# ut-vision/Rot-MVGaze

Measured on AMD Instinct MI355X. Metric: multi-view samples/sec (fwd+bwd), BxVx3x224x224, higher is better.
Workload: dtype f32; 1 GPU; C3: ResNet-50, V=4, B=128 per GPU, 3x224x224, fwd+loss+bwd; backbone=ResNet-50, views=4, batch_per_gpu=128, global_batch=128, image=3x224x224, parallelism=dp1, weights=random init, seed 0 (kaiming-normal convs, default Linear), rccl_ranks=1, step_launch=eager: every kernel queued from Python

## Files before the change

### include/rotmvgaze.h

```cpp
#ifndef ROTMVGAZE_H
#define ROTMVGAZE_H

#include <stddef.h>
#include <stdint.h>

#ifdef __cplusplus
extern "C" {
#endif

#define MVG_ABI_VERSION 11

int mvg_abi_version(void);
const char *mvg_last_error(void);
int mvg_device_cus(void);
int mvg_set_scratch(void *ptr, size_t bytes, void *stream);
size_t mvg_scratch_bytes(void);
void *mvg_stream_create_low_priority(void);
int mvg_set_reserved_cus(int n);

enum {
  MVG_K_CONV_FPROP = 0, MVG_K_CONV_DGRAD = 1, MVG_K_CONV_WGRAD = 2, MVG_K_WGRAD_REDUCE = 3,
  MVG_K_BN_FINALIZE = 4, MVG_K_BN_APPLY = 5, MVG_K_BN_BWD_REDUCE = 6, MVG_K_BN_BWD_APPLY = 7,
  MVG_K_POOL = 8, MVG_K_LAYOUT = 9, MVG_K_LINEAR_FPROP = 10, MVG_K_LINEAR_DGRAD = 11,
  MVG_K_LINEAR_WGRAD = 12, MVG_K_ROTCAT = 13, MVG_K_COLSUM = 14, MVG_K_LOSS = 15,
// ... 38 lines not shown
                    int nvec, int fout, int img_rows, int feat_rows, float *workspace, size_t ws_floats, void *stream);
int mvg_fuser_wgrad(const float *img_feat, const float *feat, const float *rel, const int32_t *row_img,
                    const int32_t *row_src, const float *dy, float *dw, float *db, int rows, int cf, int nvec, int fout,
                    int img_rows, int feat_rows, float *workspace, int splits, int accumulate, void *stream);

int mvg_linear_wgrad(const float *x, const float *dy, float *dw, float *db, int rows, int fin, int fout,
                     float *workspace, int splits, int accumulate, void *stream);

size_t mvg_linear_workspace_floats(int rows, int fin, int fout);
int mvg_linear_fprop(const float *x, const float *w, const float *bias, int relu, float *y, int rows,
                     int fin, int fout, float *workspace, size_t ws_floats, void *stream);
int mvg_linear_dgrad(const float *dy, const float *w, const float *mask, const float *addend, float *dx,
                     int rows, int fin, int fout, float *workspace, size_t ws_floats, void *stream);


int mvg_bn_finalize(const float *stats, int groups, int partials, int rows_per_partial,
                    int64_t rows_per_group, int c, const float *gamma, const float *beta,
                    float *running_mean, float *running_var, float momentum, float eps,
                    float *mean, float *invstd, float *scale, float *shift, void *stream);
int mvg_bn_eval_affine(int groups, int c, const float *gamma, const float *beta,
                       const float *running_mean, const float *running_var, float eps,
                       float *scale, float *shift, void *stream);
int mvg_bn_eval_affine_batch(const void *items_dev, int n, int max_c, float eps, void *stream);
int mvg_bn_apply(const float *y, const float *scale, const float *shift, const float *residual,
                 const float *res_scale, const float *res_shift, int relu, float *out, int groups,
                 int64_t rows_per_group, int c, void *stream);
int mvg_bn_apply_bits(const float *y, const float *scale, const float *shift, const float *residual,
                      const float *res_scale, const float *res_shift, float *out, uint8_t *relu_bits, int groups,
                      int64_t rows_per_group, int c, void *stream);
int mvg_bn_bwd_reduce_bits(const float *g, const uint8_t *relu_bits, const float *y, const float *mean,
                           const float *invstd, int groups, int64_t rows_per_group, int c, float *s1, float *s2,
                           float *dgamma, float *dbeta, int accumulate, float *workspace, float *dz_out, void *stream);
int mvg_bn_apply_bits_bf16(const uint16_t *y, const float *scale, const float *shift, const uint16_t *residual,
                           const float *res_scale, const float *res_shift, uint16_t *out, uint8_t *relu_bits,
                           int groups, int64_t rows_per_group, int c, void *stream);
int mvg_bn_bwd_reduce_bits_bf16(const uint16_t *g, const uint8_t *relu_bits, const uint16_t *y, const float *mean,
                                const float *invstd, int groups, int64_t rows_per_group, int c, float *s1,
                                float *s2, float *dgamma, float *dbeta, int accumulate, float *workspace,
                                uint16_t *dz_out, void *stream);
int mvg_bn_bwd_reduce(const float *g, const float *act, const float *y, const float *mean,
                      const float *invstd, const float *relu_scale, const float *relu_shift,
                      int groups, int64_t rows_per_group, int c, float *s1, float *s2, float *dgamma,
                      float *dbeta, int accumulate, float *workspace, float *dz_out, void *stream);
size_t mvg_bn_bwd_workspace_floats(int groups, int64_t rows_per_group, int c);
int mvg_bn_bwd_apply(const float *g, const float *act, const float *y, const float *mean,
                     const float *invstd, const float *gamma, const float *s1, const float *s2,
                     const float *relu_scale, const float *relu_shift, int groups,
                     int64_t rows_per_group, int c, float *dy, float *dz_out, void *stream);
int mvg_bn_eval_bwd(const float *g, const float *act, const uint8_t *relu_bits, const float *y, const float *relu_scale,
                    const float *relu_shift, const float *gamma, const float *running_mean, const float *running_var,
                    float eps, int groups, int64_t rows_per_group, int c, float *dy, float *dz_out, float *dgamma,
                    float *dbeta, int accumulate, float *workspace, void *stream);
size_t mvg_bn_eval_bwd_workspace_floats(int groups, int64_t rows_per_group, int c);

int mvg_maxpool3x3s2_fwd(const float *x, float *y, uint8_t *argmax, int n, int h, int w, int c,
                         int ho, int wo, void *stream);
int mvg_maxpool3x3s2_bwd(const float *dy, const uint8_t *argmax, float *dx, int n, int h, int w,
                         int c, int ho, int wo, void *stream);
int mvg_bn_relu_maxpool_fwd(const float *y, const float *scale, const float *shift, float *pooled,
                            uint8_t *argmax, int groups, int n_per_group, int h, int w, int c,
                            int ho, int wo, void *stream);
int mvg_bn_relu_maxpool_bwd_reduce(const float *g_pooled, const uint8_t *argmax, const float *y,
                                   const float *mean, const float *invstd, const float *scale,
                                   const float *shift, int groups, int n_per_group, int h, int w,
                                   int c, int ho, int wo, float *s1, float *s2, float *dgamma,
                                   float *dbeta, int accumulate, float *workspace, void *stream);
int mvg_bn_relu_maxpool_bwd_apply(const float *g_pooled, const uint8_t *argmax, const float *y,
                                  const float *mean, const float *invstd, const float *gamma,
                                  const float *scale, const float *shift, const float *s1,
                                  const float *s2, int groups, int n_per_group, int h, int w, int c,
                                  int ho, int wo, float *dy, void *stream);
int mvg_bn_relu_maxpool_eval_bwd(const float *g_pooled, const uint8_t *argmax, const float *y, const float *scale,
                                 const float *shift, const float *gamma, const float *running_mean,
                                 const float *running_var, float eps, int groups, int n_per_group, int h, int w,
                                 int c, int ho, int wo, float *dy, float *dgamma, float *dbeta, int accumulate,
                                 float *workspace, void *stream);
int mvg_avgpool_fwd(const float *x, float *y, int n, int hw, int c, void *stream);
int mvg_avgpool_bwd(const float *dy, float *dx, int n, int hw, int c, void *stream);
int mvg_nchw_to_nhwc4(const float *src, float *dst, int n, int c, int h, int w, void *stream);
int mvg_nhwc4_to_nchw(const float *src, float *dst, int n, int c, int h, int w, void *stream);
int mvg_preprocess_u8hwc(const uint8_t *src, float *dst, int n, int h, int w, float mean0, float mean1,
                         float mean2, float std0, float std1, float std2, int swap_rb, void *stream);
int mvg_preprocess_u8hwc_resize(const uint8_t *src, float *dst, int n, int h, int w, int oh, int ow, float mean0,
                                float mean1, float mean2, float std0, float std1, float std2, int swap_rb,
                                void *stream);
int mvg_multi_erase_nchw(float *img, const float *masks, const int32_t *grid, int gmax, int n, int c,
                         int h, int w, void *stream);

int mvg_rotation_matrix_2d(const float *pitch_yaw , float *rot , int n,
                           int inverse, void *stream);
int mvg_relative_rotation(const float *rot, const int32_t *vi, const int32_t *vj, float *rel,
                          int batch, int views, int dirs, void *stream);

int mvg_rotcat_fwd(const float *img_feat , const float *feat ,
                   const float *rel , const int32_t *view_of,
                   const int32_t *src_of, float *x , int batch, int dirs,
                   int cf, int nvec, void *stream);
int mvg_rotcat_bwd(const float *dx, const float *rel, const int32_t *src_of, float *dfeat, int batch,
                   int dirs, int cf, int nvec, void *stream);
int mvg_rotcat_ext_fwd(const float *img_feat, const float *feat, const float *rel_apply,
                       const float *rel_append, const int32_t *view_of, const int32_t *src_of,
                       float *x, int ld, int batch, int dirs, int cf, int nvec, void *stream);
int mvg_rotcat_ext_bwd(const float *dx, int ld, const float *rel, const int32_t *src_of, float *dfeat,
                       int batch, int dirs, int cf, int nvec, void *stream);
int mvg_ibn_scales(const float *a , const float *feat ,
                   const int32_t *view_of, const int32_t *src_of, float *running_mean, int training,
                   float momentum, float eps, float *scales, int batch, int dirs, int nvec,
                   void *stream);
int mvg_paircat_fwd(const float *a, const float *feat, const float *rel, const float *scales,
                    const int32_t *view_of, const int32_t *src_of, float *x, int batch, int dirs,
                    int nvec, void *stream);
int mvg_paircat_bwd(const float *dx, const float *rel, const float *scales, const int32_t *src_of,
                    float *da_dir, float *dfeat, int batch, int dirs, int nvec, void *stream);
int mvg_segment_sum(const float *x, int64_t row_stride, int width, const int32_t *seg_of, float *out,
                    int batch, int dirs, int segments, int accumulate, void *stream);

int mvg_axpby(const float *x, float *y, float a, float b, int64_t n, void *stream);
int mvg_scale_by(const float *x, const float *scale, float *out, int64_t n, void *stream);

int mvg_linear_skinny_fwd(const float *x, const float *w, const float *bias, float *y, int rows, int k,
                          int nout, void *stream);
int mvg_linear_skinny_bwd(const float *dy, const float *x, const float *w, const float *mask, float *dx,
                          float *dw, float *db, int rows, int k, int nout, int accumulate, float *dx_absmax, void *stream);

int mvg_adam_step(float *param, const float *grad, float *exp_avg, float *exp_avg_sq, int64_t n, float lr,
                  float beta1, float beta2, float eps, float weight_decay, int step, void *stream);
int mvg_adam_step_dev(float *param, const float *grad, float *exp_avg, float *exp_avg_sq, int64_t n, const float *lr_dev,
                      float *state3, float beta1, float beta2, float eps, float weight_decay, void *stream);

int mvg_gaze_angular_loss(const float *pred, const float *gt, int n, float row_weight,
                          float *loss, int accumulate, float *dpred, float *theta_out, void *stream);

int mvg_gaze_lp_loss(const float *pred, const float *label, int n, int p, float *loss, float *dpred, void *stream);
int mvg_gaze_angular_loss_multi(const float *pred, const float *gt, int iters, int dirs, int batch, const float *host_weights,
                                float *loss, float *dpred, void *stream);

int mvg_mt19937_seed(uint32_t *host_state , uint64_t seed);
int64_t mvg_pair_index_build(uint32_t *host_state, const int64_t *host_file_rows, int n_files,
                             int camera_tag, int64_t *host_out , int64_t capacity);


int mvg_cast_weights_bf16(const mvg_conv_desc *d, const float *w, int cin_src, void *w_krsc, void *w_crsk,
                          void *stream);
int mvg_conv_fprop_bf16(const mvg_conv_desc *d, const void *x, const void *wgt, void *y, const float *bias,
                        int relu, float *stats, void *stream);
int mvg_conv_stats_partials_bf16(const mvg_conv_desc *d, int32_t *out_rows_per_partial);
int mvg_conv_fprop_bf16_affine(const mvg_conv_desc *d, const void *x, const void *wgt, void *out, const float *scale,
                               const float *shift, const void *residual, int relu, void *stream);
int mvg_conv_dgrad_bf16(const mvg_conv_desc *d, const void *dy, const void *wgt_crsk, void *dx,
                        const void *mask, const void *addend, void *stream);
int mvg_conv_dgrad_bn_partials_bf16(const mvg_conv_desc *d);
int mvg_conv_dgrad_bf16_bnreduce(const mvg_conv_desc *d, const void *dy, const void *wgt_crsk, void *dx, const void *addend,
                                 const void *bn_y, const uint8_t *bn_bits, const float *bn_mean, const float *bn_invstd,
                                 const float *relu_scale, const float *relu_shift, float *partials, float *s1, float *s2,
                                 float *dgamma, float *dbeta, int accumulate, void *stream);
int mvg_stem_rowwindow_bf16(const float *x_nchw, void *xw, int64_t images, int h, int w, void *stream);
int mvg_stem_fprop_bf16(const mvg_conv_desc *d, const void *xw, const void *w_fold, void *y, float *stats, void *stream);
int mvg_stem_wgrad_splits_bf16(const mvg_conv_desc *d);
int mvg_stem_wgrad_bf16(const mvg_conv_desc *d, const void *xw, const void *dy, float *dw_fold, float *workspace, int splits,
                        int accumulate, void *stream);
int mvg_conv_wgrad_bf16(const mvg_conv_desc *d, const void *x, const void *dy, float *dw, float *workspace,
                        int splits, int accumulate, void *stream);
int mvg_conv_wgrad_splits_bf16(const mvg_conv_desc *d);
int mvg_conv_wgrad_bf16_slabs(const mvg_conv_desc *d, const void *x, const void *dy, float *workspace, int splits, void *stream);
int mvg_linear_fprop_mixed(const float *x, const void *w_bf16, const float *bias, int relu, float *y, int rows, int fin,
                           int fout, void *stream);
int mvg_linear_dgrad_mixed(const float *dy, const void *wt_bf16, const float *mask, const float *addend, float *dx,
                           int rows, int fin, int fout, void *stream);
int mvg_linear_wgrad_mixed(const float *x, const float *dy, float *dw, float *db, int rows, int fin, int fout,
                           float *workspace, int splits, int accumulate, void *stream);
int mvg_bn_apply_bf16(const uint16_t *y, const float *scale, const float *shift, const uint16_t *residual,
                      const float *res_scale, const float *res_shift, int relu, uint16_t *out, int groups,
                      int64_t rows_per_group, int c, void *stream);
int mvg_bn_bwd_reduce_bf16(const uint16_t *g, const uint16_t *act, const uint16_t *y, const float *mean,
                           const float *invstd, const float *relu_scale, const float *relu_shift, int groups,
                           int64_t rows_per_group, int c, float *s1, float *s2, float *dgamma, float *dbeta,
                           int accumulate, float *workspace, uint16_t *dz_out, void *stream);
int mvg_bn_bwd_apply_bf16(const uint16_t *g, const uint16_t *act, const uint16_t *y, const float *mean,
                          const float *invstd, const float *gamma, const float *s1, const float *s2,
                          const float *relu_scale, const float *relu_shift, int groups, int64_t rows_per_group,
                          int c, uint16_t *dy, uint16_t *dz_out, void *stream);
int mvg_bn_relu_maxpool_fwd_bf16(const uint16_t *y, const float *scale, const float *shift, uint16_t *pooled,
                                 uint8_t *argmax, int groups, int n_per_group, int h, int w, int c, int ho,
                                 int wo, void *stream);
int mvg_bn_relu_maxpool_bwd_reduce_bf16(const uint16_t *g_pooled, const uint8_t *argmax, const uint16_t *y,
                                        const float *mean, const float *invstd, const float *scale,
                                        const float *shift, int groups, int n_per_group, int h, int w, int c,
                                        int ho, int wo, float *s1, float *s2, float *dgamma, float *dbeta,
                                        int accumulate, float *workspace, void *stream);
int mvg_bn_relu_maxpool_bwd_apply_bf16(const uint16_t *g_pooled, const uint8_t *argmax, const uint16_t *y,
                                       const float *mean, const float *invstd, const float *gamma,
                                       const float *scale, const float *shift, const float *s1,
                                       const float *s2, int groups, int n_per_group, int h, int w, int c,
                                       int ho, int wo, uint16_t *dy, void *stream);
int mvg_avgpool_fwd_bf16(const uint16_t *x, float *y, int n, int hw, int c, void *stream);
int mvg_avgpool_bwd_bf16(const float *dy, uint16_t *dx, int n, int hw, int c, void *stream);
int mvg_nchw_to_nhwc8_bf16(const float *src, uint16_t *dst, int n, int c, int h, int w, void *stream);
int mvg_preprocess_u8hwc_resize_bf16(const uint8_t *src, uint16_t *dst, int n, int h, int w, int oh, int ow, float mean0,
                                     float mean1, float mean2, float std0, float std1, float std2, int swap_rb,
                                     void *stream);

int mvg_split_f32(const float *x, void *out_sp, int64_t n, float scale, void *stream);
int mvg_merge_sp(const void *x_sp, float *out, int64_t n, float inv_scale, void *stream);
int mvg_split_weights(const mvg_conv_desc *d, const float *w, void *w_krsc_sp, void *w_crsk_sp, float *stat2, void *items_dev,
                      void *stream);
int mvg_weights_prep_batch(const void *items_dev, int n, int mode, int blocks_per_item , void *stream);
int mvg_conv_stats_partials_split(const mvg_conv_desc *d, int32_t *rows_per_partial);
int mvg_conv_fprop_split(const mvg_conv_desc *d, const void *x_sp, const float *x_sinv, const void *w_sp, const float *w_sinv,
                         float *y, float *stats, void *stream);
int mvg_conv_fprop_split_affine(const mvg_conv_desc *d, const void *x_sp, const float *x_sinv, const void *w_sp, const float *w_sinv,
                                void *out, int out_sp, const float *scale, const float *shift, const void *residual,
                                int residual_sp, int relu, void *stream);
int mvg_conv_fprop_split_affine_ranged(const mvg_conv_desc *d, const void *x_sp, const float *x_sinv, const void *w_sp,
                                       const float *w_sinv, void *out, int out_sp, const float *scale, const float *shift,
                                       const void *residual, int residual_sp, int relu, uint32_t *range_word, void *stream);
int mvg_split_f32_ranged(const float *x, void *out_sp, int64_t n, float scale, uint32_t *range_word, void *stream);
int mvg_conv_dgrad_split(const mvg_conv_desc *d, const void *dy_sp, const float *dy_sinv, const void *w_crsk_sp,
                         const float *w_sinv, float *dx, const float *addend, const void *relu_mask_sp, void *stream);
int mvg_bn_apply_split(const float *y, const float *scale, const float *shift, const void *residual, int residual_sp,
                       const float *res_scale, const float *res_shift, int relu, void *out_sp, uint8_t *relu_bits,
                       int groups, int64_t rows_per_group, int c, void *stream);
int mvg_bn_bwd_reduce_split(const float *g, const uint8_t *relu_bits, const float *y, const float *mean, const float *invstd,
                            const float *relu_scale, const float *relu_shift, int groups, int64_t rows_per_group, int c,
                            float *s1, float *s2, float *dgamma, float *dbeta, int accumulate, float *workspace,
                            float *dz_out, float *mx, const float *gamma, float *dy_sinv, void *stream);
int mvg_bn_bwd_apply_split(const float *g, const float *y, const float *mean, const float *invstd, const float *gamma,
                           const float *s1, const float *s2, const float *relu_scale, const float *relu_shift,
                           int groups, int64_t rows_per_group, int c, void *dy_sp, const float *mx, float *dy_sinv,
                           int dy_sinv_ready, void *stream);
int mvg_bn_relu_maxpool_fwd_split(const float *y, const float *scale, const float *shift, void *pooled_sp,
                                  uint8_t *argmax, int groups, int n_per_group, int h, int w, int c, int ho, int wo,
                                  void *stream);
int mvg_avgpool_fwd_split(const void *x_sp, float *y, int n, int hw, int c, void *stream);
int mvg_act_scales(const void *items_dev, int n, float *slots, int n_slots, void *stream);
int mvg_bn_apply_split_scaled(const float *y, const float *scale, const float *shift, const void *residual, int residual_sp,
                              const float *res_scale, const float *res_shift, const float *res_sinv, int relu, void *out_sp,
                              const float *out_sinv, uint8_t *relu_bits, int groups, int64_t rows_per_group, int c,
                              void *stream);
int mvg_bn_relu_maxpool_fwd_split_scaled(const float *y, const float *scale, const float *shift, void *pooled_sp,
                                         const float *pooled_sinv, uint8_t *argmax, int groups, int n_per_group, int h, int w,
                                         int c, int ho, int wo, void *stream);
int mvg_avgpool_fwd_split_scaled(const void *x_sp, const float *x_sinv, float *y, int n, int hw, int c, void *stream);
int mvg_conv_dgrad_bn_partials_split(const mvg_conv_desc *d);
int mvg_conv_dgrad_split_bnreduce(const mvg_conv_desc *d, const void *dy_sp, const float *dy_sinv, const void *w_crsk_sp,
                                  const float *w_sinv, float *dx, const float *addend, const float *bn_y, const uint8_t *bn_bits,
                                  const float *bn_mean, const float *bn_invstd, const float *relu_scale, const float *relu_shift,
                                  float *partials, float *s1, float *s2, float *dgamma, float *dbeta, int accumulate,
                                  float *mx, const float *bn_gamma, float *dx_dy_sinv, void *stream);
int mvg_conv_dgrad_split_bnapply_bnreduce(const mvg_conv_desc *d, void *dy_sp, const float *dy_sinv, const float *dz, const float *y,
                                          const float *mean, const float *invstd, const float *gamma, const float *un_s1,
                                          const float *un_s2, int64_t rows_per_group, const void *w_crsk_sp, const float *w_sinv,
                                          float *dx, const float *addend, const float *bn_y, const uint8_t *bn_bits,
                                          const float *bn_mean, const float *bn_invstd, const float *relu_scale,
                                          const float *relu_shift, float *partials, float *s1, float *s2, float *dgamma, float *dbeta,
                                          int accumulate, float *mx, const float *bn_gamma, float *dx_dy_sinv, void *stream);
int mvg_conv_fprop_split_stages(const mvg_conv_desc *d);
int mvg_conv_dgrad_split_stages(const mvg_conv_desc *d, int fused_reduce);
int mvg_conv_fprop_split_bnapply(const mvg_conv_desc *d, void *out_sp, const float *out_sinv, const float *bn_y, const float *scale,
                                 const float *shift, const void *residual, int residual_sp, const float *res_scale,
                                 const float *res_shift, const float *res_sinv, uint8_t *relu_bits, const void *w_sp,
                                 const float *w_sinv, float *y, float *stats, void *stream);
int mvg_stem_rowwindow_split(const float *x_nhwc4, void *xw_sp, int64_t images, int h, int w, void *stream);
int mvg_stem_rowwindow_split_nchw(const float *x_nchw, void *xw_sp, int64_t images, int h, int w, void *stream);
int mvg_stem_fprop_split(const mvg_conv_desc *d, const void *xw_sp, const void *w_sp, const float *w_sinv, float *y, float *stats,
                         void *stream);
int mvg_stem_wgrad_splits_split(const mvg_conv_desc *d);
int mvg_stem_wgrad_split(const mvg_conv_desc *d, const void *xw_sp, const void *dy_sp, const float *dy_sinv, float *dw_rw,
                         float *workspace, int splits, int accumulate, void *stream);
int mvg_bn_relu_maxpool_bwd_reduce_split(const float *g_pooled, const uint8_t *argmax, const float *y, const float *mean,
                                         const float *invstd, const float *scale, const float *shift, int groups,
                                         int n_per_group, int h, int w, int c, int ho, int wo, float *s1, float *s2,
                                         float *dgamma, float *dbeta, int accumulate, float *workspace, float *mx, const float *gamma,
                                         float *dy_sinv, void *stream);
int mvg_bn_relu_maxpool_bwd_apply_split(const float *g_pooled, const uint8_t *argmax, const float *y, const float *mean,
                                        const float *invstd, const float *gamma, const float *scale, const float *shift,
                                        const float *s1, const float *s2, int groups, int n_per_group, int h, int w, int c,
                                        int ho, int wo, void *dy_sp, const float *mx, float *dy_sinv, int dy_sinv_ready, void *stream);
int mvg_conv_wgrad_splits_split(const mvg_conv_desc *d);
int mvg_conv_wgrad_split_tile(const mvg_conv_desc *d, int32_t *bm, int32_t *bn, int32_t *incremental);
int mvg_conv_wgrad_split(const mvg_conv_desc *d, const void *x_sp, const void *dy_sp, const float *dy_sinv, float *dw,
                         float *workspace, int splits, int accumulate, void *stream);
int mvg_conv_wgrad_split_slabs(const mvg_conv_desc *d, const void *x_sp, const void *dy_sp, const float *dy_sinv, float *workspace,
                               int splits, void *stream);
int mvg_conv_wgrad_split_xs(const mvg_conv_desc *d, const void *x_sp, const float *x_sinv, const void *dy_sp, const float *dy_sinv,
                            float *dw, float *workspace, int splits, int accumulate, void *stream);
int mvg_conv_wgrad_split_slabs_xs(const mvg_conv_desc *d, const void *x_sp, const float *x_sinv, const void *dy_sp,
                                  const float *dy_sinv, float *workspace, int splits, void *stream);
int mvg_wgrad_reduce_batch(const float *const *host_slabs, float *const *host_dw, const int64_t *host_n, const int32_t *host_splits,
                           const int32_t *host_accumulate, int n, void *stream);

int mvg_absmax_multi(const float *const *host_ptrs, const int64_t *host_counts, float *const *host_out_slots, int n, void *stream);
int mvg_fuse_build_split(const float *img_feat, const float *feat, const float *rel, const int32_t *row_img, const int32_t *row_src_f,
                         const int32_t *row_src_h, void *xf_sp, void *xh_sp, const float *am_img, const float *am_feat,
                         float *xf_sinv, float *xh_sinv, int rows, int cf, int nvec, void *stream);
int mvg_fuse_unbuild(const float *dxh, const float *dxn, const float *rel, const int32_t *seg, const int32_t *vi, float *dfeat, float *da,
                     int da_accumulate, int segments, int views, int dirs, int batch, int cf, int nvec, float *absmax, void *stream);
int mvg_linear_fprop_split(int rows, int fin, int fout, const void *x_sp, const float *x_sinv, const void *w_sp, const float *w_sinv,
                           const float *bias, int relu, void *out, int out_sp, float *out_sinv, const float *bias_absmax,
                           float *out_absmax, void *stream);
int mvg_linear_dgrad_split(int rows, int fin, int fout, const void *dy_sp, const float *dy_sinv, const void *wt_sp, const float *w_sinv,
                           float *dx, const float *addend, const void *relu_mask_sp, float *out_absmax, void *stream);
int mvg_linear_wgrad_split(int rows, int fin, int fout, const void *x_sp, const float *x_sinv, const void *dy_sp, const float *dy_sinv,
                           float *dw, float *workspace, int splits, int accumulate, void *stream);
int mvg_split_colsum(const float *g, int rows, int cols, const float *absmax, void *out_sp, float *out_sinv, float *db, int accumulate,
                     void *stream);

typedef struct mvg_session mvg_session;
typedef struct {
  int32_t depth;
  int32_t num_iter;
  int32_t views, batch;
  int32_t height, width;
  int32_t share_weights, ignore_rotmat;
  int32_t split;
  int32_t raw_u8;
  int32_t in_h, in_w, input_bgr;
} mvg_session_cfg;

int mvg_session_create(const mvg_session_cfg *cfg, mvg_session **out);
#define MVG_SESSION_FP32 0
#define MVG_SESSION_BF16 1
int mvg_session_create_ex(const mvg_session_cfg *cfg, int32_t compute, mvg_session **out);
int mvg_session_compute(const mvg_session *s);
void mvg_session_destroy(mvg_session *s);
int mvg_session_num_tensors(const mvg_session *s);
const char *mvg_session_tensor_name(const mvg_session *s, int i);
int64_t mvg_session_tensor_numel(const mvg_session *s, int i);
size_t mvg_session_workspace_bytes(const mvg_session *s);
int mvg_session_launches(const mvg_session *s);
int mvg_session_num_steps(const mvg_session *s);
const char *mvg_session_step_name(const mvg_session *s, int i);
int mvg_session_bind(mvg_session *s, const void *const *host_tensor_ptrs, void *workspace, size_t bytes, void *stream);
int mvg_session_forward(mvg_session *s, const void *const *host_view_ptrs, const float *rot, float *img_feat, float *lifted,
                        float *feats, float *preds, void *stream);
int mvg_session_num_range_units(const mvg_session *s);
const char *mvg_session_range_unit_name(const mvg_session *s, int i);
int mvg_session_set_range_record(mvg_session *s, uint32_t *record_dev);

#ifdef __cplusplus
}
#endif
#endif
```

### rot-mvgaze_amd/_lib.py

```python
from __future__ import annotations

import ctypes as C
import os

_HERE = os.path.dirname(os.path.abspath(__file__))
LIB_PATH = os.path.join(_HERE, "csrc", "librotmvgaze_hip.so")

K_FAMILIES = 18
ABI_VERSION = 11
SESSION_FP32, SESSION_BF16 = 0, 1


class ConvDesc(C.Structure):
    _fields_ = [(n, C.c_int32) for n in
                ("groups", "n", "h", "w", "cin", "cout", "r", "s", "stride", "pad", "ho", "wo")]

    @classmethod
    def make(cls, groups, n, h, w, cin, cout, k, stride, pad):
        ho = (h + 2 * pad - k) // stride + 1
        wo = (w + 2 * pad - k) // stride + 1
        return cls(groups, n, h, w, cin, cout, k, k, stride, pad, ho, wo)

    @classmethod
    def linear(cls, rows, fin, fout):
        return cls(1, rows, 1, 1, fin, fout, 1, 1, 1, 0, 1, 1)


class ProfEntry(C.Structure):
    _fields_ = [("launches", C.c_int64), ("ms", C.c_double), ("flops", C.c_double), ("bytes", C.c_double)]


class SessionCfg(C.Structure):
    _fields_ = [(n, C.c_int32) for n in
                ("depth", "num_iter", "views", "batch", "height", "width", "share_weights", "ignore_rotmat", "split", "raw_u8",
                 "in_h", "in_w", "input_bgr")]


_P = C.c_void_p
_I = C.c_int
_I64 = C.c_int64
_F = C.c_float
_D = C.POINTER(ConvDesc)

SIGNATURES = {
    "mvg_abi_version": (_I, []),
    "mvg_last_error": (C.c_char_p, []),
    "mvg_device_cus": (_I, []),
    "mvg_set_scratch": (_I, [_P, C.c_size_t, _P]),
    "mvg_scratch_bytes": (C.c_size_t, []),
    "mvg_set_reserved_cus": (_I, [_I]),
    "mvg_stream_create_low_priority": (_P, []),
    "mvg_prof_enable": (_I, [_I]),
    "mvg_prof_reset": (_I, []),
    "mvg_prof_collect": (_I, [C.POINTER(ProfEntry)]),
    "mvg_prof_family_name": (C.c_char_p, [_I]),
    "mvg_conv_fprop": (_I, [_D, _P, _P, _P, _P, _I, _P, _P]),
    "mvg_conv_fprop_affine": (_I, [_D, _P, _P, _P, _P, _P, _P, _I, _P]),
    "mvg_conv_stats_partials": (_I, [_D, C.POINTER(C.c_int32)]),
    "mvg_conv_dgrad": (_I, [_D, _P, _P, _P, _P, _P, _P]),
    "mvg_conv_wgrad": (_I, [_D, _P, _P, _P, _P, _I, _I, _P]),
    "mvg_conv_wgrad_splits": (_I, [_D]),
    "mvg_linear_wgrad": (_I, [_P, _P, _P, _P, _I, _I, _I, _P, _I, _I, _P]),
    "mvg_fuser_fprop": (_I, [_P, _P, _P, _P, _P, _P, _P, _I, _P, _I, _I, _I, _I, _I, _I, _P, C.c_size_t, _P]),
    "mvg_fuser_wgrad": (_I, [_P, _P, _P, _P, _P, _P, _P, _P, _I, _I, _I, _I, _I, _I, _P, _I, _I, _P]),
    "mvg_linear_workspace_floats": (C.c_size_t, [_I, _I, _I]),
    "mvg_linear_fprop": (_I, [_P, _P, _P, _I, _P, _I, _I, _I, _P, C.c_size_t, _P]),
    "mvg_linear_dgrad": (_I, [_P, _P, _P, _P, _P, _I, _I, _I, _P, C.c_size_t, _P]),
    "mvg_bn_finalize": (_I, [_P, _I, _I, _I, _I64, _I, _P, _P, _P, _P, _F, _F, _P, _P, _P, _P, _P]),
    "mvg_bn_eval_affine": (_I, [_I, _I, _P, _P, _P, _P, _F, _P, _P, _P]),
    "mvg_bn_eval_affine_batch": (_I, [_P, _I, _I, _F, _P]),
    "mvg_bn_apply": (_I, [_P, _P, _P, _P, _P, _P, _I, _P, _I, _I64, _I, _P]),
    "mvg_bn_bwd_reduce": (_I, [_P, _P, _P, _P, _P, _P, _P, _I, _I64, _I, _P, _P, _P, _P, _I, _P, _P, _P]),
    "mvg_split_f32": (_I, [_P, _P, _I64, _F, _P]),
    "mvg_merge_sp": (_I, [_P, _P, _I64, _F, _P]),
    "mvg_split_weights": (_I, [_D, _P, _P, _P, _P, _P, _P]),
    "mvg_weights_prep_batch": (_I, [_P, _I, _I, _I, _P]),
    "mvg_conv_stats_partials_split": (_I, [_D, C.POINTER(C.c_int32)]),
    "mvg_conv_fprop_split": (_I, [_D, _P, _P, _P, _P, _P, _P, _P]),
    "mvg_conv_fprop_split_affine": (_I, [_D, _P, _P, _P, _P, _P, _I, _P, _P, _P, _I, _I, _P]),
    "mvg_conv_dgrad_split": (_I, [_D, _P, _P, _P, _P, _P, _P, _P, _P]),
    "mvg_bn_apply_split": (_I, [_P, _P, _P, _P, _I, _P, _P, _I, _P, _P, _I, _I64, _I, _P]),
    "mvg_bn_bwd_apply_split": (_I, [_P, _P, _P, _P, _P, _P, _P, _P, _P, _I, _I64, _I, _P, _P, _P, _I, _P]),
    "mvg_bn_bwd_reduce_split": (_I, [_P, _P, _P, _P, _P, _P, _P, _I, _I64, _I, _P, _P, _P, _P, _I, _P, _P, _P, _P, _P, _P]),
    "mvg_bn_relu_maxpool_fwd_split": (_I, [_P, _P, _P, _P, _P, _I, _I, _I, _I, _I, _I, _I, _P]),
    "mvg_avgpool_fwd_split": (_I, [_P, _P, _I, _I, _I, _P]),
    "mvg_act_scales": (_I, [_P, _I, _P, _I, _P]),
    "mvg_bn_apply_split_scaled": (_I, [_P, _P, _P, _P, _I, _P, _P, _P, _I, _P, _P, _P, _I, _I64, _I, _P]),
    "mvg_bn_relu_maxpool_fwd_split_scaled": (_I, [_P, _P, _P, _P, _P, _P, _I, _I, _I, _I, _I, _I, _I, _P]),
    "mvg_avgpool_fwd_split_scaled": (_I, [_P, _P, _P, _I, _I, _I, _P]),
    "mvg_conv_wgrad_split_xs": (_I, [_D, _P, _P, _P, _P, _P, _P, _I, _I, _P]),
    "mvg_conv_wgrad_split_slabs_xs": (_I, [_D, _P, _P, _P, _P, _P, _I, _P]),
    "mvg_stem_rowwindow_split": (_I, [_P, _P, _I64, _I, _I, _P]),
    "mvg_stem_rowwindow_split_nchw": (_I, [_P, _P, _I64, _I, _I, _P]),
    "mvg_stem_fprop_split": (_I, [_D, _P, _P, _P, _P, _P, _P]),
    "mvg_stem_wgrad_splits_split": (_I, [_D]),
    "mvg_stem_wgrad_split": (_I, [_D, _P, _P, _P, _P, _P, _I, _I, _P]),
    "mvg_bn_relu_maxpool_bwd_reduce_split": (_I, [_P, _P, _P, _P, _P, _P, _P, _I, _I, _I, _I, _I, _I, _I, _P, _P, _P, _P, _I, _P, _P, _P, _P, _P]),
    "mvg_bn_relu_maxpool_bwd_apply_split": (_I, [_P, _P, _P, _P, _P, _P, _P, _P, _P, _P, _I, _I, _I, _I, _I, _I, _I, _P, _P, _P, _I, _P]),
    "mvg_conv_dgrad_bn_partials_split": (_I, [_D]),
    "mvg_conv_dgrad_split_bnreduce": (_I, [_D, _P, _P, _P, _P, _P, _P, _P, _P, _P, _P, _P, _P, _P, _P, _P, _P, _P, _I, _P, _P, _P, _P]),
    "mvg_conv_dgrad_split_bnapply_bnreduce": (_I, [_D] + [_P] * 9 + [_I64] + [_P] * 15 + [_I, _P, _P, _P, _P]),
    "mvg_conv_fprop_split_stages": (_I, [_D]),
    "mvg_conv_dgrad_split_stages": (_I, [_D, _I]),
    "mvg_conv_fprop_split_bnapply": (_I, [_D] + [_P] * 6 + [_I] + [_P] * 9),
    "mvg_conv_wgrad_splits_split": (_I, [_D]),
    "mvg_conv_wgrad_split_tile": (_I, [_D, C.POINTER(C.c_int32), C.POINTER(C.c_int32), C.POINTER(C.c_int32)]),
    "mvg_conv_wgrad_split": (_I, [_D, _P, _P, _P, _P, _P, _I, _I, _P]),
    "mvg_conv_wgrad_split_slabs": (_I, [_D, _P, _P, _P, _P, _I, _P]),
    "mvg_wgrad_reduce_batch": (_I, [C.POINTER(C.c_void_p), C.POINTER(C.c_void_p), C.POINTER(C.c_int64), C.POINTER(C.c_int32),
                                    C.POINTER(C.c_int32), _I, _P]),
    "mvg_bn_apply_bits": (_I, [_P, _P, _P, _P, _P, _P, _P, _P, _I, _I64, _I, _P]),
    "mvg_bn_bwd_reduce_bits": (_I, [_P, _P, _P, _P, _P, _I, _I64, _I, _P, _P, _P, _P, _I, _P, _P, _P]),
    "mvg_bn_apply_bits_bf16": (_I, [_P, _P, _P, _P, _P, _P, _P, _P, _I, _I64, _I, _P]),
    "mvg_bn_bwd_reduce_bits_bf16": (_I, [_P, _P, _P, _P, _P, _I, _I64, _I, _P, _P, _P, _P, _I, _P, _P, _P]),
    "mvg_bn_bwd_workspace_floats": (C.c_size_t, [_I, _I64, _I]),
    "mvg_bn_bwd_apply": (_I, [_P, _P, _P, _P, _P, _P, _P, _P, _P, _P, _I, _I64, _I, _P, _P, _P]),
    "mvg_maxpool3x3s2_fwd": (_I, [_P, _P, _P, _I, _I, _I, _I, _I, _I, _P]),
    "mvg_maxpool3x3s2_bwd": (_I, [_P, _P, _P, _I, _I, _I, _I, _I, _I, _P]),
    "mvg_bn_relu_maxpool_fwd": (_I, [_P, _P, _P, _P, _P, _I, _I, _I, _I, _I, _I, _I, _P]),
    "mvg_bn_relu_maxpool_bwd_reduce": (_I, [_P, _P, _P, _P, _P, _P, _P, _I, _I, _I, _I, _I, _I, _I, _P, _P, _P, _P, _I, _P,
                                            _P]),
    "mvg_bn_relu_maxpool_bwd_apply": (_I, [_P, _P, _P, _P, _P, _P, _P, _P, _P, _P, _I, _I, _I, _I, _I, _I, _I, _P, _P]),
    "mvg_bn_eval_bwd": (_I, [_P, _P, _P, _P, _P, _P, _P, _P, _P, _F, _I, _I64, _I, _P, _P, _P, _P, _I, _P, _P]),
    "mvg_bn_eval_bwd_workspace_floats": (C.c_size_t, [_I, _I64, _I]),
    "mvg_bn_relu_maxpool_eval_bwd": (_I, [_P, _P, _P, _P, _P, _P, _P, _P, _F, _I, _I, _I, _I, _I, _I, _I, _P, _P, _P, _I, _P,
                                          _P]),
    "mvg_avgpool_fwd": (_I, [_P, _P, _I, _I, _I, _P]),
    "mvg_avgpool_bwd": (_I, [_P, _P, _I, _I, _I, _P]),
    "mvg_nchw_to_nhwc4": (_I, [_P, _P, _I, _I, _I, _I, _P]),
    "mvg_nhwc4_to_nchw": (_I, [_P, _P, _I, _I, _I, _I, _P]),
    "mvg_preprocess_u8hwc": (_I, [_P, _P, _I, _I, _I, _F, _F, _F, _F, _F, _F, _I, _P]),
    "mvg_gaze_lp_loss": (_I, [_P, _P, _I, _I, _P, _P, _P]),
    "mvg_preprocess_u8hwc_resize": (_I, [_P, _P, _I, _I, _I, _I, _I, _F, _F, _F, _F, _F, _F, _I, _P]),
    "mvg_multi_erase_nchw": (_I, [_P, _P, _P, _I, _I, _I, _I, _I, _P]),
    "mvg_rotation_matrix_2d": (_I, [_P, _P, _I, _I, _P]),
    "mvg_relative_rotation": (_I, [_P, _P, _P, _P, _I, _I, _I, _P]),
    "mvg_rotcat_fwd": (_I, [_P, _P, _P, _P, _P, _P, _I, _I, _I, _I, _P]),
    "mvg_rotcat_bwd": (_I, [_P, _P, _P, _P, _I, _I, _I, _I, _P]),
    "mvg_rotcat_ext_fwd": (_I, [_P, _P, _P, _P, _P, _P, _P, _I, _I, _I, _I, _I, _P]),
    "mvg_rotcat_ext_bwd": (_I, [_P, _I, _P, _P, _P, _I, _I, _I, _I, _P]),
    "mvg_ibn_scales": (_I, [_P, _P, _P, _P, _P, _I, _F, _F, _P, _I, _I, _I, _P]),
    "mvg_paircat_fwd": (_I, [_P, _P, _P, _P, _P, _P, _P, _I, _I, _I, _P]),
    "mvg_paircat_bwd": (_I, [_P, _P, _P, _P, _P, _P, _I, _I, _I, _P]),
    "mvg_segment_sum": (_I, [_P, _I64, _I, _P, _P, _I, _I, _I, _I, _P]),
    "mvg_axpby": (_I, [_P, _P, _F, _F, _I64, _P]),
    "mvg_scale_by": (_I, [_P, _P, _P, _I64, _P]),
    "mvg_linear_skinny_fwd": (_I, [_P, _P, _P, _P, _I, _I, _I, _P]),
    "mvg_linear_skinny_bwd": (_I, [_P, _P, _P, _P, _P, _P, _P, _I, _I, _I, _I, _P, _P]),
    "mvg_adam_step": (_I, [_P, _P, _P, _P, _I64, _F, _F, _F, _F, _F, _I, _P]),
    "mvg_gaze_angular_loss": (_I, [_P, _P, _I, _F, _P, _I, _P, _P, _P]),
    "mvg_gaze_angular_loss_multi": (_I, [_P, _P, _I, _I, _I, C.POINTER(C.c_float), _P, _P, _P]),
    "mvg_adam_step_dev": (_I, [_P, _P, _P, _P, _I64, _P, _P, _F, _F, _F, _F, _P]),
    "mvg_absmax_multi": (_I, [C.POINTER(C.c_void_p), C.POINTER(C.c_int64), C.POINTER(C.c_void_p), _I, _P]),
    "mvg_fuse_build_split": (_I, [_P, _P, _P, _P, _P, _P, _P, _P, _P, _P, _P, _P, _I, _I, _I, _P]),
    "mvg_fuse_unbuild": (_I, [_P, _P, _P, _P, _P, _P, _P, _I, _I, _I, _I, _I, _I, _I, _P, _P]),
    "mvg_linear_fprop_split": (_I, [_I, _I, _I, _P, _P, _P, _P, _P, _I, _P, _I, _P, _P, _P, _P]),
    "mvg_linear_dgrad_split": (_I, [_I, _I, _I, _P, _P, _P, _P, _P, _P, _P, _P, _P]),
    "mvg_linear_wgrad_split": (_I, [_I, _I, _I, _P, _P, _P, _P, _P, _P, _I, _I, _P]),
    "mvg_split_colsum": (_I, [_P, _I, _I, _P, _P, _P, _P, _I, _P]),
    "mvg_cast_weights_bf16": (_I, [_D, _P, _I, _P, _P, _P]),
    "mvg_conv_fprop_bf16": (_I, [_D, _P, _P, _P, _P, _I, _P, _P]),
    "mvg_conv_stats_partials_bf16": (_I, [_D, C.POINTER(C.c_int32)]),
    "mvg_conv_fprop_bf16_affine": (_I, [_D, _P, _P, _P, _P, _P, _P, _I, _P]),
    "mvg_conv_dgrad_bf16": (_I, [_D, _P, _P, _P, _P, _P, _P]),
    "mvg_conv_dgrad_bn_partials_bf16": (_I, [_D]),
    "mvg_conv_dgrad_bf16_bnreduce": (_I, [_D, _P, _P, _P, _P, _P, _P, _P, _P, _P, _P, _P, _P, _P, _P, _P, _I, _P]),
    "mvg_conv_wgrad_bf16": (_I, [_D, _P, _P, _P, _P, _I, _I, _P]),
    "mvg_stem_rowwindow_bf16": (_I, [_P, _P, _I64, _I, _I, _P]),
    "mvg_stem_fprop_bf16": (_I, [_D, _P, _P, _P, _P, _P]),
    "mvg_stem_wgrad_splits_bf16": (_I, [_D]),
    "mvg_stem_wgrad_bf16": (_I, [_D, _P, _P, _P, _P, _I, _I, _P]),
    "mvg_conv_wgrad_splits_bf16": (_I, [_D]),
    "mvg_conv_wgrad_bf16_slabs": (_I, [_D, _P, _P, _P, _I, _P]),
    "mvg_linear_fprop_mixed": (_I, [_P, _P, _P, _I, _P, _I, _I, _I, _P]),
    "mvg_linear_dgrad_mixed": (_I, [_P, _P, _P, _P, _P, _I, _I, _I, _P]),
    "mvg_linear_wgrad_mixed": (_I, [_P, _P, _P, _P, _I, _I, _I, _P, _I, _I, _P]),
    "mvg_bn_apply_bf16": (_I, [_P, _P, _P, _P, _P, _P, _I, _P, _I, _I64, _I, _P]),
    "mvg_bn_bwd_reduce_bf16": (_I, [_P, _P, _P, _P, _P, _P, _P, _I, _I64, _I, _P, _P, _P, _P, _I, _P, _P, _P]),
    "mvg_bn_bwd_apply_bf16": (_I, [_P, _P, _P, _P, _P, _P, _P, _P, _P, _P, _I, _I64, _I, _P, _P, _P]),
    "mvg_bn_relu_maxpool_fwd_bf16": (_I, [_P, _P, _P, _P, _P, _I, _I, _I, _I, _I, _I, _I, _P]),
    "mvg_bn_relu_maxpool_bwd_reduce_bf16": (_I, [_P, _P, _P, _P, _P, _P, _P, _I, _I, _I, _I, _I, _I, _I, _P, _P, _P, _P, _I,
                                                 _P, _P]),
    "mvg_bn_relu_maxpool_bwd_apply_bf16": (_I, [_P, _P, _P, _P, _P, _P, _P, _P, _P, _P, _I, _I, _I, _I, _I, _I, _I, _P, _P]),
    "mvg_avgpool_fwd_bf16": (_I, [_P, _P, _I, _I, _I, _P]),
    "mvg_avgpool_bwd_bf16": (_I, [_P, _P, _I, _I, _I, _P]),
    "mvg_nchw_to_nhwc8_bf16": (_I, [_P, _P, _I, _I, _I, _I, _P]),
    "mvg_preprocess_u8hwc_resize_bf16": (_I, [_P, _P, _I, _I, _I, _I, _I, _F, _F, _F, _F, _F, _F, _I, _P]),
    "mvg_mt19937_seed": (_I, [_P, C.c_uint64]),
    "mvg_pair_index_build": (_I64, [_P, _P, _I, _I, _P, _I64]),
    "mvg_session_create": (_I, [C.POINTER(SessionCfg), C.POINTER(_P)]),
    "mvg_session_destroy": (None, [_P]),
    "mvg_session_num_tensors": (_I, [_P]),
    "mvg_session_tensor_name": (C.c_char_p, [_P, _I]),
    "mvg_session_tensor_numel": (_I64, [_P, _I]),
    "mvg_session_workspace_bytes": (C.c_size_t, [_P]),
    "mvg_session_launches": (_I, [_P]),
    "mvg_session_bind": (_I, [_P, C.POINTER(_P), _P, C.c_size_t, _P]),
    "mvg_session_forward": (_I, [_P, C.POINTER(_P), _P, _P, _P, _P, _P, _P]),
    "mvg_conv_fprop_split_affine_ranged": (_I, [_D, _P, _P, _P, _P, _P, _I, _P, _P, _P, _I, _I, _P, _P]),
    "mvg_split_f32_ranged": (_I, [_P, _P, _I64, _F, _P, _P]),
    "mvg_session_num_range_units": (_I, [_P]),
    "mvg_session_range_unit_name": (C.c_char_p, [_P, _I]),
    "mvg_session_set_range_record": (_I, [_P, _P]),
    "mvg_session_create_ex": (_I, [C.POINTER(SessionCfg), C.c_int32, C.POINTER(_P)]),
    "mvg_session_compute": (_I, [_P]),
    "mvg_session_num_steps": (_I, [_P]),
    "mvg_session_step_name": (C.c_char_p, [_P, _I]),
}

_lib = None


def lib() -> C.CDLL:
    global _lib
    if _lib is not None:
        return _lib
    if not os.path.exists(LIB_PATH):
        raise RuntimeError(
            f"{LIB_PATH} not found: the HIP extension is required (python rot-mvgaze_amd/csrc/build.py); "
            "this package has no CPU fallback")
    try:
        l = C.CDLL(LIB_PATH, mode=C.RTLD_GLOBAL)
    except OSError as e:
        raise RuntimeError(f"failed to load {LIB_PATH}: {e}") from e
    for name, (res, args) in SIGNATURES.items():
        fn = getattr(l, name)
        fn.restype = res
        fn.argtypes = args
    if l.mvg_abi_version() != ABI_VERSION:
        raise RuntimeError(f"librotmvgaze_hip.so ABI {l.mvg_abi_version()} != binding ABI {ABI_VERSION}")
    _lib = l
    return l


def check(rc: int, what: str = "") -> None:
    if rc != 0:
        msg = lib().mvg_last_error()
        raise RuntimeError(f"librotmvgaze_hip {what} failed (rc={rc}): {msg.decode() if msg else '?'}")
```

### rot-mvgaze_amd/csrc/conv_split.hip

```cpp
#include "bf16_tile.h"
#include "elem.h"

namespace mvg {

typedef _Float16 f16x8 __attribute__((ext_vector_type(8)));

#define SPLIT_ONE(PA, PB, av, bv, acc)                                                                         \
  _Pragma("unroll") for (int i = 0; i < TM; ++i) _Pragma("unroll") for (int j = 0; j < TN; ++j)                \
      acc[i][j] = __builtin_amdgcn_mfma_f32_32x32x16_f16(av[PA][i], bv[PB][j], acc[i][j], 0, 0, 0);
#define SPLIT_PRODUCTS(av, bv, acc) SPLIT_ONE(0, 1, av, bv, acc) SPLIT_ONE(1, 0, av, bv, acc) SPLIT_ONE(0, 0, av, bv, acc)

constexpr int SP_BM = 128, SP_BK = 32;

__global__ __launch_bounds__(256) void split_f32_kernel(const float4 *__restrict__ x, uint4 *__restrict__ out, long long n8, float scale) {
  const long long stride = (long long)gridDim.x * 256;
  for (long long i = (long long)blockIdx.x * 256 + threadIdx.x; i < n8; i += stride) {
    const float4 lo = x[2 * i], hi = x[2 * i + 1];
    const float v[8] = {lo.x * scale, lo.y * scale, lo.z * scale, lo.w * scale, hi.x * scale, hi.y * scale, hi.z * scale, hi.w * scale};
    uint4 q1, q2;
    split2_chunk(v, q1, q2);
    out[2 * i] = q1;
    out[2 * i + 1] = q2;
  }
}
// ... 27 lines not shown
}

__global__ __launch_bounds__(256) void split_colsum_kernel(const float *__restrict__ g, int rows, int cols, const unsigned *__restrict__ absmax,
                                                           uint4 *__restrict__ out, float *__restrict__ out_sinv, float *__restrict__ db,
                                                           int accumulate) {
  __shared__ float sh[64][33];
  const float scale = sp_scale_for(__uint_as_float(*absmax));
  if (blockIdx.x == 0 && threadIdx.x == 0) *out_sinv = 1.f / scale;
  const int cl = threadIdx.x & 3, rl = threadIdx.x >> 2;
  const int c8 = blockIdx.x * 4 + cl, c8n = cols >> 3;
  float sum[8] = {0.f, 0.f, 0.f, 0.f, 0.f, 0.f, 0.f, 0.f};
  for (int r = rl; r < rows; r += 64) {
    const float4 *src = reinterpret_cast<const float4 *>(g + (long long)r * cols + c8 * 8);
    const float4 lo = src[0], hi = src[1];
    const float v[8] = {lo.x, lo.y, lo.z, lo.w, hi.x, hi.y, hi.z, hi.w};
    float w[8];
#pragma unroll
    for (int k = 0; k < 8; ++k) {
      sum[k] += v[k];
      w[k] = v[k] * scale;
    }
    uint4 q1, q2;
    split2_chunk(w, q1, q2);
    uint4 *dst = out + SP_NP * ((long long)r * c8n + c8);
    dst[0] = q1;
    dst[1] = q2;
  }
  if (db == nullptr) return;
#pragma unroll
  for (int k = 0; k < 8; ++k) sh[rl][cl * 8 + k] = sum[k];
  __syncthreads();
  if (threadIdx.x < 32) {
    const int col = blockIdx.x * 32 + threadIdx.x;
    float t = accumulate ? db[col] : 0.f;
    for (int r = 0; r < 64; ++r) t += sh[r][threadIdx.x];
    db[col] = t;
  }
}

struct WPrepItem {
  const float *w;
  void *wk, *wt;
  int cout, rs, cin, cin_pad;
  float *stat;
};

__global__ void wprep_stage_item_kernel(WPrepItem it, WPrepItem *__restrict__ dst) {
  if (threadIdx.x == 0) *dst = it;
  if (threadIdx.x < 2) it.stat[threadIdx.x] = 0.f;
}

__global__ __launch_bounds__(256) void weights_absmax_kernel(const WPrepItem *__restrict__ items) {
  const WPrepItem it = items[blockIdx.y];
  const long long n4 = (long long)it.cout * it.rs * it.cin / 4;
  float m = 0.f;
  for (long long i = (long long)blockIdx.x * 256 + threadIdx.x; i < n4; i += (long long)gridDim.x * 256) {
    const float4 v = reinterpret_cast<const float4 *>(it.w)[i];
    m = fmaxf(fmaxf(m, fmaxf(fabsf(v.x), fabsf(v.y))), fmaxf(fabsf(v.z), fabsf(v.w)));
  }
#pragma unroll
  for (int o = 32; o > 0; o >>= 1) m = fmaxf(m, __shfl_xor(m, o, 64));
  if ((threadIdx.x & 63) == 0 && m > 0.f) atomicMax(reinterpret_cast<unsigned *>(it.stat), __float_as_uint(m));
}

__global__ __launch_bounds__(256) void weights_prep_batch_kernel(const WPrepItem *__restrict__ items, int mode) {
  __shared__ float tile[64][65];
  const WPrepItem it = items[blockIdx.y];
  const float *__restrict__ w = it.w;
  const int cout = it.cout, rs = it.rs, cin = it.cin;
  if (mode == 1) {
    const float scale = sp_scale_for(__uint_as_float(*reinterpret_cast<const unsigned *>(it.stat)));
    if (blockIdx.x == 0 && threadIdx.x == 0) it.stat[1] = 1.f / scale;
    uint4 *wk = reinterpret_cast<uint4 *>(it.wk), *wt = reinterpret_cast<uint4 *>(it.wt);
    const int c8n = cin / 8, o8n = cout / 8;
    const bool tiled = wt != nullptr && rs == 1 && (cin % 64) == 0 && (cout % 64) == 0;
    const long long nk = (long long)cout * rs * c8n, nt = (wt && !tiled) ? (long long)cin * rs * o8n : 0;
    for (long long i = (long long)blockIdx.x * 256 + threadIdx.x; i < nk + nt; i += (long long)gridDim.x * 256) {
      float v[8];
      uint4 *dst;
      if (i < nk) {
        const float4 *src = reinterpret_cast<const float4 *>(w + i * 8);
        const float4 lo = src[0], hi = src[1];
        v[0] = lo.x; v[1] = lo.y; v[2] = lo.z; v[3] = lo.w; v[4] = hi.x; v[5] = hi.y; v[6] = hi.z; v[7] = hi.w;
        dst = wk + SP_NP * i;
      } else {
        const long long j = i - nk;
        const int o8 = (int)(j % o8n);
        const long long t = j / o8n;
        const int tap = (int)(t % rs), c = (int)(t / rs);
#pragma unroll
        for (int k = 0; k < 8; ++k) v[k] = w[((long long)(o8 * 8 + k) * rs + tap) * cin + c];
        dst = wt + SP_NP * j;
      }
#pragma unroll
      for (int k = 0; k < 8; ++k) v[k] *= scale;
      uint4 q1, q2;
      split2_chunk(v, q1, q2);
      dst[0] = q1;
      dst[1] = q2;
    }
    if (tiled) {
      const int tc = cin / 64, ntiles = (cout / 64) * tc;
      for (int t = blockIdx.x; t < ntiles; t += gridDim.x) {
        const int o0 = (t / tc) * 64, c0 = (t % tc) * 64;
        __syncthreads();
#pragma unroll
        for (int ps = 0; ps < 4; ++ps) {
          const int r = (threadIdx.x >> 4) + 16 * ps, cq = threadIdx.x & 15;
          const float4 x = *reinterpret_cast<const float4 *>(w + (long long)(o0 + r) * cin + c0 + 4 * cq);
          tile[r][4 * cq] = x.x;
          tile[r][4 * cq + 1] = x.y;
          tile[r][4 * cq + 2] = x.z;
          tile[r][4 * cq + 3] = x.w;
        }
        __syncthreads();
#pragma unroll
        for (int q = 0; q < 2; ++q) {
          const int idx = threadIdx.x + 256 * q, cl = idx >> 3, o8 = idx & 7;
          float v[8];
#pragma unroll
          for (int k = 0; k < 8; ++k) v[k] = tile[o8 * 8 + k][cl] * scale;
          uint4 q1, q2;
          split2_chunk(v, q1, q2);
          uint4 *dst = wt + SP_NP * ((long long)(c0 + cl) * o8n + (o0 >> 3) + o8);
          dst[0] = q1;
          dst[1] = q2;
        }
      }
    }
    return;
  }
  unsigned short *wk = reinterpret_cast<unsigned short *>(it.wk), *wt = reinterpret_cast<unsigned short *>(it.wt);
  const int cin_pad = it.cin_pad;
  const long long total = (long long)cout * rs * cin_pad;
  if (rs == 1 && cin == cin_pad && (cin % 64) == 0 && (cout % 64) == 0) {
    uint4 *wk4 = reinterpret_cast<uint4 *>(wk);
    for (long long i = (long long)blockIdx.x * 256 + threadIdx.x; i < total / 8; i += (long long)gridDim.x * 256) {
      const float4 lo = reinterpret_cast<const float4 *>(w + i * 8)[0], hi = reinterpret_cast<const float4 *>(w + i * 8)[1];
      wk4[i] = make_uint4(bf16_pack2(lo.x, lo.y), bf16_pack2(lo.z, lo.w), bf16_pack2(hi.x, hi.y), bf16_pack2(hi.z, hi.w));
    }
    if (wt) {
      const int tc = cin / 64, ntiles = (cout / 64) * tc;
      for (int t = blockIdx.x; t < ntiles; t += gridDim.x) {
        const int o0 = (t / tc) * 64, c0 = (t % tc) * 64;
        __syncthreads();
#pragma unroll
        for (int ps = 0; ps < 4; ++ps) {
          const int r = (threadIdx.x >> 4) + 16 * ps, cq = threadIdx.x & 15;
          const float4 x = *reinterpret_cast<const float4 *>(w + (long long)(o0 + r) * cin + c0 + 4 * cq);
          tile[r][4 * cq] = x.x;
          tile[r][4 * cq + 1] = x.y;
          tile[r][4 * cq + 2] = x.z;
          tile[r][4 * cq + 3] = x.w;
        }
        __syncthreads();
#pragma unroll
        for (int q = 0; q < 2; ++q) {
          const int idx = threadIdx.x + 256 * q, cl = idx >> 3, o8 = idx & 7;
          float v[8];
#pragma unroll
          for (int k = 0; k < 8; ++k) v[k] = tile[o8 * 8 + k][cl];
          *reinterpret_cast<uint4 *>(wt + (long long)(c0 + cl) * cout + o0 + o8 * 8) =
              make_uint4(bf16_pack2(v[0], v[1]), bf16_pack2(v[2], v[3]), bf16_pack2(v[4], v[5]), bf16_pack2(v[6], v[7]));
        }
      }
    }
    return;
  }
  for (long long i = (long long)blockIdx.x * 256 + threadIdx.x; i < total; i += (long long)gridDim.x * 256) {
    const int c = (int)(i % cin_pad);
    const long long t = i / cin_pad;
    const int tap = (int)(t % rs), o = (int)(t / rs);
    const float v = c < cin ? w[((long long)o * rs + tap) * cin + c] : 0.f;
    const __bf16 b = (__bf16)v;
    const unsigned short u = __builtin_bit_cast(unsigned short, b);
    wk[i] = u;
    if (wt) wt[((long long)c * rs + tap) * cout + o] = u;
  }
}

typedef float f32x4 __attribute__((ext_vector_type(4)));

#define SPLIT16_ONE(PA, PB)                                                                       \
  _Pragma("unroll") for (int i = 0; i < TM; ++i) _Pragma("unroll") for (int j = 0; j < TN; ++j)   \
      acc[i][j] = __builtin_amdgcn_mfma_f32_16x16x32_f16(av[PA][i], bv[PB][j], acc[i][j], 0, 0, 0);

__device__ __forceinline__ int sp_row_swz(int R) { return ((R >> 1) & 1) | (((R >> 2) & 1) << 2); }

enum AForm : int { A_DMA = 0, A_DY = 1, A_OUT_SP = 2, A_OUT_AFFINE = 3 };
constexpr int BNA_MAX_C = 512;

__device__ __forceinline__ void unpack8(const float4 (&v)[2], float (&o)[8]) {
  o[0] = v[0].x; o[1] = v[0].y; o[2] = v[0].z; o[3] = v[0].w; o[4] = v[1].x; o[5] = v[1].y; o[6] = v[1].z; o[7] = v[1].w;
}

struct DyFormer {
  static constexpr int TABLES = 5;
  __amdgpu_buffer_rsrc_t rs_dz, rs_y;
  float inv_rows, dsc;
  float4 dzv[2][2], yv[2][2];
  float mu[8], is[8], ga[8], sa[8], sb[8];
  static __device__ __forceinline__ void stage(float *t, const IgemmParams &p, int g, int C, int tid) {
    for (int i = tid; i < C; i += 256) {
      const long long gc = (long long)g * C + i;
      t[i] = p.bna_mean[gc];
      t[C + i] = p.bna_invstd[gc];
      t[2 * C + i] = p.bna_gamma[i];
      t[3 * C + i] = p.bna_s1[gc];
      t[4 * C + i] = p.bna_s2[gc];
    }
  }
  __device__ __forceinline__ DyFormer(const IgemmParams &p, long long grow0, long long rows_per_group, int C)
      : rs_dz(make_rsrc(p.bna_dz + grow0 * C, 4ll * rows_per_group * C)), rs_y(make_rsrc(p.bna_y + grow0 * C, 4ll * rows_per_group * C)),
        inv_rows(p.bna_inv_rows), dsc(1.f / *p.a_sinv) {}
  __device__ __forceinline__ void load(int i, unsigned off) {
    dzv[i][0] = buf_ld16(rs_dz, off);
    dzv[i][1] = buf_ld16(rs_dz, off + 16u);
    yv[i][0] = buf_ld16(rs_y, off);
    yv[i][1] = buf_ld16(rs_y, off + 16u);
  }
  __device__ __forceinline__ void consts(const float *kc, int C) {
    ld8(kc, mu);
    ld8(kc + C, is);
    ld8(kc + 2 * C, ga);
    ld8(kc + 3 * C, sa);
    ld8(kc + 4 * C, sb);
  }
  __device__ __forceinline__ void form(int i, bool ok, float (&o)[8]) {
    float d[8], v[8];
    unpack8(dzv[i], d);
    unpack8(yv[i], v);
    bn_dy_chunk(d, v, mu, is, ga, sa, sb, inv_rows, dsc, o, false, mu, mu);
#pragma unroll
    for (int k = 0; k < 8; ++k) o[k] = ok ? o[k] : 0.f;
  }
  __device__ __forceinline__ void store_extra(int, unsigned) {}
};

template <bool AFFINE>
struct OutFormer {
  static constexpr int TABLES = AFFINE ? 4 : 2;
  __amdgpu_buffer_rsrc_t rs_y, rs_r;
  float osc, rsi;
  unsigned short *bits_out;
  float4 yv[2][2], rv[2][2];
  float sc[8], sh[8], rs[8], rh[8];
  unsigned mb[2];
  static __device__ __forceinline__ void stage(float *t, const IgemmParams &p, int g, int C, int tid) {
    for (int i = tid; i < C; i += 256) {
      const long long gc = (long long)g * C + i;
      t[i] = p.fap_scale[gc];
      t[C + i] = p.fap_shift[gc];
      if constexpr (AFFINE) {
        t[2 * C + i] = p.fap_res_scale[gc];
        t[3 * C + i] = p.fap_res_shift[gc];
      }
    }
  }
  __device__ __forceinline__ OutFormer(const IgemmParams &p, long long grow0, long long rows_per_group, int C)
      : rs_y(make_rsrc(p.fap_y + grow0 * C, 4ll * rows_per_group * C)),
        rs_r(make_rsrc(reinterpret_cast<const float *>(p.fap_res) + grow0 * C, 4ll * rows_per_group * C)),
        osc(__uint_as_float(__builtin_amdgcn_readfirstlane(__float_as_uint(p.a_sinv ? 1.f / *p.a_sinv : 1.f)))),
        rsi(__uint_as_float(__builtin_amdgcn_readfirstlane(__float_as_uint((!AFFINE && p.fap_res_sinv) ? *p.fap_res_sinv : 1.f)))),
        bits_out(p.fap_bits ? p.fap_bits + grow0 * (C >> 3) : nullptr) {}
  __device__ __forceinline__ void load(int i, unsigned off) {
    yv[i][0] = buf_ld16(rs_y, off);
    yv[i][1] = buf_ld16(rs_y, off + 16u);
    rv[i][0] = buf_ld16(rs_r, off);
    rv[i][1] = buf_ld16(rs_r, off + 16u);
  }
  __device__ __forceinline__ void consts(const float *kc, int C) {
    ld8(kc, sc);
    ld8(kc + C, sh);
    if constexpr (AFFINE) {
      ld8(kc + 2 * C, rs);
      ld8(kc + 3 * C, rh);
    }
  }
  __device__ __forceinline__ void form(int i, bool ok, float (&o)[8]) {
    float v[8], r[8];
    unpack8(yv[i], v);
    if constexpr (AFFINE) {
      unpack8(rv[i], r);
    } else {
      const uint4 r1 = make_uint4(__float_as_uint(rv[i][0].x), __float_as_uint(rv[i][0].y), __float_as_uint(rv[i][0].z), __float_as_uint(rv[i][0].w));
      const uint4 r2 = make_uint4(__float_as_uint(rv[i][1].x), __float_as_uint(rv[i][1].y), __float_as_uint(rv[i][1].z), __float_as_uint(rv[i][1].w));
      merge2_chunk(r1, r2, r);
    }
    mb[i] = bn_apply_chunk(v, sc, sh, true, r, AFFINE, rs, rh, !AFFINE, rsi, true, osc, o);
#pragma unroll
    for (int k = 0; k < 8; ++k) o[k] = ok ? o[k] : 0.f;
  }
  __device__ __forceinline__ void store_extra(int i, unsigned off) {
    if (bits_out) bits_out[off >> 5] = (unsigned short)mb[i];
  }
};

#define MVG_SPLIT_RNG 0
#include "conv_split_igemm.inc"
#undef MVG_SPLIT_RNG
#define MVG_SPLIT_RNG 1
#include "conv_split_igemm.inc"
#undef MVG_SPLIT_RNG

template <int BM, int BN, bool INCR>
__global__ __launch_bounds__(256, BN >= 256 ? 2 : 3) void wgrad_split_kernel(WgradParams p) {
  constexpr int BK = 16, WGM = 2, WGN = 2;
  constexpr int WTM = BM / WGM, WTN = BN / WGN;
  constexpr int TM = WTM / 32, TN = WTN / 32;
  constexpr int LDA = BM + 32, LDB = BN + 32;
  constexpr int MV = BM / 8, NVB = BN / 8;
  constexpr int A_TPR = 256 / BK;
  constexpr int A_CPT = MV / A_TPR > 0 ? MV / A_TPR : 1;
  constexpr int B_CPT = (NVB + A_TPR - 1) / A_TPR;
  constexpr int A_ELEMS = BK * LDA, B_ELEMS = BK * LDB;
  constexpr int STAGE = SP_NP * (A_ELEMS + B_ELEMS);
  __shared__ __attribute__((aligned(16))) unsigned short smem[2 * STAGE];

  const int tid = threadIdx.x;
  const int lane = tid & 63, wave = tid >> 6;
  const int wm = wave / WGN, wn = wave % WGN;
  const int li = lane & 31, lh = lane >> 5;
  const int tiles = p.mtiles * p.ntiles;
  const int logical = xcd_remap(blockIdx.x, gridDim.x);
  const int split = logical / tiles;
  const int tile = logical - split * tiles;
  const int ntile = tile % p.ntiles, mtile = tile / p.ntiles;
  const long long m_begin = (long long)split * p.pixels_per_split;
  long long m_end = m_begin + p.pixels_per_split;
  if (m_end > p.pixels) m_end = p.pixels;
  const int m_count = m_end > m_begin ? (int)(m_end - m_begin) : 0;
  const int ohw = p.ho * p.wo;
  const long long img0 = m_begin / ohw;
  const unsigned rem0 = (unsigned)(m_begin - img0 * ohw);

  const char *dy = reinterpret_cast<const char *>(p.dy);
  const char *x = reinterpret_cast<const char *>(p.x);
  const __amdgpu_buffer_rsrc_t rs_a = make_rsrc(dy + m_begin * p.cout * SP_BYTES, (long long)SP_BYTES * m_count * p.cout);
  const long long x_img_elems = (long long)p.h * p.w * p.cin;
  const __amdgpu_buffer_rsrc_t rs_b = make_rsrc(x + img0 * x_img_elems * SP_BYTES, p.x_bytes - (long long)SP_BYTES * img0 * x_img_elems);
  const int i_row = tid / A_TPR, i_v0 = tid % A_TPR;
  unsigned a_off[A_CPT];
  bool a_on[A_CPT];
#pragma unroll
  for (int j = 0; j < A_CPT; ++j) {
    const int cv = i_v0 + j * A_TPR;
    const int col = mtile * BM + cv * 8;
    a_on[j] = cv < MV;
    a_off[j] = (a_on[j] && col < p.cout) ? (unsigned)(i_row * p.cout + col) * (unsigned)SP_BYTES : 0x80000000u;
  }
  int i_dy[B_CPT], i_dx[B_CPT];
  unsigned i_tconst[B_CPT];
  bool i_cok[B_CPT], b_on[B_CPT];
#pragma unroll
  for (int j = 0; j < B_CPT; ++j) {
    const int cv = i_v0 + j * A_TPR;
    const int col = ntile * BN + cv * 8;
    b_on[j] = cv < NVB;
    i_cok[j] = b_on[j] && col < p.ncols;
    const int tap = (int)fdiv((unsigned)(i_cok[j] ? col : 0), p.cin_div);
    const int cc = (i_cok[j] ? col : 0) - tap * p.cin;
    const int fr = (int)fdiv((unsigned)tap, p.s_div), fs = tap - fr * p.s;
    i_dy[j] = fr - p.pad;
    i_dx[j] = fs - p.pad_w;
    i_tconst[j] = (unsigned)((i_dy[j] * p.w + i_dx[j]) * p.cin + cc) * (unsigned)SP_BYTES;
  }
  const unsigned row_bytes = (unsigned)(p.stride * p.w * p.cin) * (unsigned)SP_BYTES, col_bytes = (unsigned)(p.stride_w * p.cin) * (unsigned)SP_BYTES;
  const unsigned img_bytes = (unsigned)x_img_elems * (unsigned)SP_BYTES;
  int s_oy = 0, s_ox = 0;
  unsigned s_imgoff = 0;
  if (INCR) {
    const unsigned pix = rem0 + (unsigned)i_row;
    const unsigned img = fdiv(pix, p.ohw_div);
    const unsigned rem = pix - img * (unsigned)ohw;
    const unsigned oy = fdiv(rem, p.wo_div);
    s_oy = (int)oy;
    s_ox = (int)(rem - oy * (unsigned)p.wo);
    s_imgoff = img * img_bytes;
  }
  u32x4 a_reg[A_CPT][SP_NP], b_reg[B_CPT][SP_NP];
  auto load_tiles = [&](int kt) {
#pragma unroll
    for (int j = 0; j < A_CPT; ++j) {
#pragma unroll
      for (int pc = 0; pc < SP_NP; ++pc)
        a_reg[j][pc] = __builtin_amdgcn_raw_buffer_load_b128(rs_a, a_off[j] + 16u * pc, 0, 0);
      a_off[j] += (unsigned)(BK * p.cout) * (unsigned)SP_BYTES;
    }
    const bool mok = kt * BK + i_row < m_count;
    int oy, ox;
    unsigned imgoff;
    if constexpr (INCR) {
      oy = s_oy;
      ox = s_ox;
      imgoff = s_imgoff;
    } else {
      const unsigned pix = rem0 + (unsigned)(kt * BK + i_row);
      const unsigned img = fdiv(pix, p.ohw_div);
      const unsigned rem = pix - img * (unsigned)ohw;
      const unsigned uy = fdiv(rem, p.wo_div);
      oy = (int)uy;
      ox = (int)(rem - uy * (unsigned)p.wo);
      imgoff = img * img_bytes;
    }
    const int iy0 = oy * p.stride, ix0 = ox * p.stride_w;
    const unsigned pixoff = imgoff + (unsigned)oy * row_bytes + (unsigned)ox * col_bytes;
#pragma unroll
    for (int j = 0; j < B_CPT; ++j) {
      const bool ok = mok & i_cok[j] & ((unsigned)(iy0 + i_dy[j]) < (unsigned)p.h) & ((unsigned)(ix0 + i_dx[j]) < (unsigned)p.w);
#pragma unroll
      for (int pc = 0; pc < SP_NP; ++pc)
        b_reg[j][pc] = __builtin_amdgcn_raw_buffer_load_b128(rs_b, pred_off(pixoff + i_tconst[j] + 16u * pc, ok), 0, 0);
    }
    if constexpr (INCR) {
      unsigned nx = (unsigned)s_ox + BK;
      const unsigned q = fdiv(nx, p.wo_div);
      nx -= q * (unsigned)p.wo;
      s_ox = (int)nx;
      const int noy = s_oy + (int)q;
      const bool wrap = noy >= p.ho;
      s_oy = wrap ? noy - p.ho : noy;
      s_imgoff += wrap ? img_bytes : 0u;
    }
  };
  auto store_tiles = [&](int buf) {
    unsigned short *As = smem + buf * STAGE;
    unsigned short *Bs = As + SP_NP * A_ELEMS;
#pragma unroll
    for (int j = 0; j < A_CPT; ++j)
      if (a_on[j]) {
#pragma unroll
        for (int pc = 0; pc < SP_NP; ++pc)
          *reinterpret_cast<u32x4 *>(As + pc * A_ELEMS + i_row * LDA + (i_v0 + j * A_TPR) * 8) = a_reg[j][pc];
      }
#pragma unroll
    for (int j = 0; j < B_CPT; ++j)
      if (b_on[j]) {
#pragma unroll
        for (int pc = 0; pc < SP_NP; ++pc)
          *reinterpret_cast<u32x4 *>(Bs + pc * B_ELEMS + i_row * LDB + (i_v0 + j * A_TPR) * 8) = b_reg[j][pc];
      }
  };

  f32x16 acc[TM][TN];
#pragma unroll
  for (int i = 0; i < TM; ++i)
#pragma unroll
    for (int j = 0; j < TN; ++j)
#pragma unroll
      for (int e = 0; e < 16; ++e) acc[i][j][e] = 0.f;

  const int KT = (m_count + BK - 1) / BK;
  load_tiles(0);
  store_tiles(0);
  load_tiles(1);
  __syncthreads();
  for (int kt = 0; kt < KT; ++kt) {
    const int cur = kt & 1;
    store_tiles(cur ^ 1);
    load_tiles(kt + 2);
    const unsigned short *As = smem + cur * STAGE;
    const unsigned short *Bs = As + SP_NP * A_ELEMS;
    f16x8 av[SP_NP][TM], bv[SP_NP][TN];
#pragma unroll
    for (int pc = 0; pc < SP_NP; ++pc) {
#pragma unroll
      for (int i = 0; i < TM; ++i) av[pc][i] = __builtin_bit_cast(f16x8, tr_frag(As + pc * A_ELEMS, LDA, 0, wm * WTM + i * 32, lane));
#pragma unroll
      for (int j = 0; j < TN; ++j) bv[pc][j] = __builtin_bit_cast(f16x8, tr_frag(Bs + pc * B_ELEMS, LDB, 0, wn * WTN + j * 32, lane));
    }
    SPLIT_PRODUCTS(av, bv, acc)
    __syncthreads();
  }

  float *out = p.out + (long long)split * p.cout * p.ncols;
  const float osc = (p.dy_sinv ? *p.dy_sinv : 1.f) * (p.x_sinv ? *p.x_sinv : 1.f);
#pragma unroll
  for (int i = 0; i < TM; ++i)
#pragma unroll
    for (int j = 0; j < TN; ++j) {
      const int col = ntile * BN + wn * WTN + j * 32 + li;
#pragma unroll
      for (int e = 0; e < 16; ++e) {
        const int row = mtile * BM + wm * WTM + i * 32 + (e & 3) + 8 * (e >> 2) + 4 * lh;
        if (row < p.cout && col < p.ncols) {
          const long long off = (long long)row * p.ncols + col;
          float v = acc[i][j][e] * osc;
          if (p.accumulate) v += out[off];
          out[off] = v;
        }
      }
    }
}

struct ReduceItem {
  const float *slabs;
  float *dw;
  long long n4;
  int splits, accumulate, lanes, block0;
};
struct ReduceBatch {
  ReduceItem it[8];
  int n;
};
__global__ __launch_bounds__(256) void wgrad_reduce_batch_kernel(ReduceBatch b) {
  __shared__ float4 sh[256];
  int k = 0;
  for (int i = 1; i < b.n; ++i) k += (int)blockIdx.x >= b.it[i].block0;
  const ReduceItem &r = b.it[k];
  const int cols = 256 / r.lanes;
  const int c = threadIdx.x % cols, l = threadIdx.x / cols;
  const long long i = (long long)(blockIdx.x - r.block0) * cols + c;
  float4 s = make_float4(0.f, 0.f, 0.f, 0.f);
  if (i < r.n4)
    for (int q = l; q < r.splits; q += r.lanes) {
      const float4 v = reinterpret_cast<const float4 *>(r.slabs)[(long long)q * r.n4 + i];
      s.x += v.x;
      s.y += v.y;
      s.z += v.z;
      s.w += v.w;
    }
  sh[threadIdx.x] = s;
  __syncthreads();
  if (l == 0 && i < r.n4) {
    float4 t = r.accumulate ? reinterpret_cast<const float4 *>(r.dw)[i] : make_float4(0.f, 0.f, 0.f, 0.f);
    for (int q = 0; q < r.lanes; ++q) {
      const float4 v = sh[q * cols + c];
      t.x += v.x;
      t.y += v.y;
      t.z += v.z;
      t.w += v.w;
    }
    reinterpret_cast<float4 *>(r.dw)[i] = t;
  }
}

__global__ __launch_bounds__(256) void stem_rowwindow_kernel(const float4 *__restrict__ x, uint4 *__restrict__ xw, long long n, int h, int w) {
  const int wo = w >> 1;
  for (long long i = (long long)blockIdx.x * 256 + threadIdx.x; i < n; i += (long long)gridDim.x * 256) {
    const int q = (int)(i & 3);
    const long long t = i >> 2;
    const int ox = (int)(t % wo);
    const long long row = t / wo;
    const int c0 = 2 * ox - 4 + 2 * q;
    float v[8] = {0.f, 0.f, 0.f, 0.f, 0.f, 0.f, 0.f, 0.f};
    if (c0 >= 0 && c0 < w) {
      const float4 a = x[row * w + c0], b = x[row * w + c0 + 1];
      v[0] = a.x; v[1] = a.y; v[2] = a.z; v[3] = a.w; v[4] = b.x; v[5] = b.y; v[6] = b.z; v[7] = b.w;
    }
    uint4 q1, q2;
    split2_chunk(v, q1, q2);
    xw[SP_NP * i] = q1;
    xw[SP_NP * i + 1] = q2;
  }
}

__global__ __launch_bounds__(256) void stem_rowwindow_nchw_kernel(const float *__restrict__ x, uint4 *__restrict__ xw, long long n, int h, int w) {
  const int wo = w >> 1;
  const long long plane = (long long)h * w;
  for (long long i = (long long)blockIdx.x * 256 + threadIdx.x; i < n; i += (long long)gridDim.x * 256) {
    const int q = (int)(i & 3);
    const long long t = i >> 2;
    const int ox = (int)(t % wo);
    const long long row = t / wo;
    const long long img = row / h;
    const int yy = (int)(row - img * h);
    const int c0 = 2 * ox - 4 + 2 * q;
    float v[8] = {0.f, 0.f, 0.f, 0.f, 0.f, 0.f, 0.f, 0.f};
    if (c0 >= 0 && c0 < w) {
      const float *src = x + img * 3 * plane + (long long)yy * w + c0;
      const float2 r = *reinterpret_cast<const float2 *>(src), g = *reinterpret_cast<const float2 *>(src + plane),
                   b = *reinterpret_cast<const float2 *>(src + 2 * plane);
      v[0] = r.x; v[1] = g.x; v[2] = b.x; v[4] = r.y; v[5] = g.y; v[6] = b.y;
    }
    uint4 q1, q2;
    split2_chunk(v, q1, q2);
    xw[SP_NP * i] = q1;
    xw[SP_NP * i + 1] = q2;
  }
}

static int validate_split(const mvg_conv_desc *d) {
  if (validate(d)) return 2;
  MVG_REQUIRE(d->cin % 32 == 0 && d->cout % 32 == 0, "split conv: cin and cout must be multiples of 32 (got %d, %d)", d->cin,
              d->cout);
  MVG_REQUIRE(d->r * d->s <= 32, "split conv: at most 32 filter taps");
  return 0;
}

static int split_tile_rows(int ncols, int taps, long long rows) { return (ncols < 128 && taps > 1 && rows >= 65536) ? 256 : SP_BM; }

struct SplitPlan { int bm, bn, kt_max; long long tiles; bool pipelined; };
static int split_conv_stages(const SplitPlan &pl) { return (pl.pipelined && pl.bn == 128 && pl.bm == SP_BM) ? 2 : 1; }
static SplitPlan split_plan(int ncols, int taps, long long rows, int groups, bool lin, IgemmClass *cls, int ncls) {
  SplitPlan pl;
  pl.bm = lin ? SP_BM : split_tile_rows(ncols, taps, rows);
  pl.bn = ncols >= 128 ? 128 : 64;
  if (lin && pl.bn == 128 && ncls == 1) {
    const long long t128 = (long long)groups * ceil_div(cls[0].rows_per_group, pl.bm) * ceil_div(ncols, 128);
    if (2 * t128 <= compute_cus()) pl.bn = 64;
  }
  pl.tiles = 0, pl.kt_max = 0;
  for (int i = 0; i < ncls; ++i) {
    IgemmClass &c = cls[i];
    c.mtiles_per_group = ceil_div(c.rows_per_group, pl.bm);
    c.KT = ceil_div(c.ktotal, SP_BK);
    c.tile0 = (int)pl.tiles;
    pl.tiles += (long long)groups * c.mtiles_per_group * ceil_div(ncols, pl.bn);
    pl.kt_max = c.KT > pl.kt_max ? c.KT : pl.kt_max;
  }
  pl.pipelined = pl.tiles <= 2LL * compute_cus() || (pl.tiles <= 4LL * compute_cus() && pl.kt_max >= 48);
  return pl;
}

template <bool DGRAD>
static int launch_igemm_split(IgemmParams &p, hipStream_t st, bool lin, int taps, long long rows, AForm af = A_DMA, bool ranged = false) {
  const SplitPlan pl = split_plan(p.ncols, taps, rows, p.groups, lin, p.cls, p.ncls);
  const int bm = pl.bm, bn = pl.bn;
  const bool pipelined = pl.pipelined;
  p.ntiles = ceil_div(p.ncols, bn);
  p.splits = 1;
  p.sk_tiles = 0;
  p.bn_parts = 0;
  for (int i = 0; i < p.ncls; ++i) {
    IgemmClass &c = p.cls[i];
    c.korder = c.ntaps > 1 ? 1 : 0;
    c.per_div = make_fastdiv((unsigned)(c.ntaps > 0 ? c.ntaps : 1));
    c.unit0 = 0;
    c.part0 = p.bn_parts;
    p.bn_parts += c.mtiles_per_group;
    MVG_REQUIRE((c.ntaps >= 1 || (DGRAD && p.bn_part)) && c.ntaps <= 32 && c.ktotal % SP_BK == 0, "split conv: class shape not covered");
  }
  MVG_REQUIRE(pl.tiles < (1LL << 31), "split conv: grid too large");
  if (pl.tiles <= 0) return 0;
  p.nt_out = (!lin && !(DGRAD && p.cls_step == 2)) ? 1 : 0;
  dim3 grid((unsigned)pl.tiles), block(256);
  if (af != A_DMA) {
    MVG_REQUIRE(!lin && bm == SP_BM && p.ntiles == 1 && p.ncls == 1 && DGRAD == (af == A_DY), "split conv: the operand-forming loaders take one column tile");
    if constexpr (DGRAD) {
      if (bn == 128) hipLaunchKernelGGL((igemm_split16_kernel<128, true, false, 2, 1, A_DY>), grid, block, 0, st, p);
      else hipLaunchKernelGGL((igemm_split16_kernel<64, true, false, 2, 1, A_DY>), grid, block, 0, st, p);
      return check_launch("conv_dgrad_split_bnapply");
    } else {
      if (bn == 128 && af == A_OUT_AFFINE) hipLaunchKernelGGL((igemm_split16_kernel<128, false, false, 2, 1, A_OUT_AFFINE>), grid, block, 0, st, p);
      else if (bn == 128) hipLaunchKernelGGL((igemm_split16_kernel<128, false, false, 2, 1, A_OUT_SP>), grid, block, 0, st, p);
      else if (af == A_OUT_AFFINE) hipLaunchKernelGGL((igemm_split16_kernel<64, false, false, 2, 1, A_OUT_AFFINE>), grid, block, 0, st, p);
      else hipLaunchKernelGGL((igemm_split16_kernel<64, false, false, 2, 1, A_OUT_SP>), grid, block, 0, st, p);
      return check_launch("conv_fprop_split_bnapply");
    }
  }
  if (ranged) {
    MVG_REQUIRE(!DGRAD && !lin && p.out_sp && p.out_absmax, "split conv: the range record goes with a forward that stores sp");
    if constexpr (!DGRAD) {
      if (bm == 256) hipLaunchKernelGGL((igemm_split16_ranged_kernel<64, 4>), grid, block, 0, st, p);
      else if (split_conv_stages(pl) == 2) hipLaunchKernelGGL((igemm_split16_ranged_kernel<128, 2, 2>), grid, block, 0, st, p);
      else if (bn == 128) hipLaunchKernelGGL((igemm_split16_ranged_kernel<128>), grid, block, 0, st, p);
      else hipLaunchKernelGGL((igemm_split16_ranged_kernel<64>), grid, block, 0, st, p);
    }
    return check_launch("conv_fprop_split_ranged");
  }
  if (lin) {
    if (bn == 128 && pipelined) hipLaunchKernelGGL((igemm_split16_kernel<128, DGRAD, true, 2, 2>), grid, block, 0, st, p);
    else if (bn == 128) hipLaunchKernelGGL((igemm_split16_kernel<128, DGRAD, true>), grid, block, 0, st, p);
    else if (pipelined) hipLaunchKernelGGL((igemm_split16_kernel<64, DGRAD, true, 2, 2>), grid, block, 0, st, p);
    else hipLaunchKernelGGL((igemm_split16_kernel<64, DGRAD, true>), grid, block, 0, st, p);
  } else if (bm == 256) hipLaunchKernelGGL((igemm_split16_kernel<64, DGRAD, false, 4>), grid, block, 0, st, p);
  else if (split_conv_stages(pl) == 2) hipLaunchKernelGGL((igemm_split16_kernel<128, DGRAD, false, 2, 2>), grid, block, 0, st, p);
  else if (bn == 128) hipLaunchKernelGGL((igemm_split16_kernel<128, DGRAD>), grid, block, 0, st, p);
  else hipLaunchKernelGGL((igemm_split16_kernel<64, DGRAD>), grid, block, 0, st, p);
  return check_launch(DGRAD ? "conv_dgrad_split" : "conv_fprop_split");
}

}

using namespace mvg;

extern "C" {

int mvg_split_f32(const float *x, void *out_sp, int64_t n, float scale, void *stream) {
  MVG_REQUIRE(x && out_sp && n >= 0 && n % 8 == 0, "split_f32: null argument or n %% 8 != 0");
  MVG_REQUIRE(scale > 0.f, "split_f32: scale must be positive (a power of two keeps the round trip exact)");
  if (n == 0) return 0;
  hipStream_t st = (hipStream_t)stream;
  ProfScope ps(MVG_K_LAYOUT, st, 0.0, (4.0 + SP_BYTES) * (double)n);
  long long blocks = (n / 8 + 255) / 256;
  if (blocks > 8192) blocks = 8192;
  hipLaunchKernelGGL(split_f32_kernel, dim3((unsigned)blocks), dim3(256), 0, st, (const float4 *)x, (uint4 *)out_sp, (long long)(n / 8), scale);
  return check_launch("split_f32");
}

int mvg_split_f32_ranged(const float *x, void *out_sp, int64_t n, float scale, uint32_t *range_word, void *stream) {
  MVG_REQUIRE(x && out_sp && range_word && n >= 0 && n % 8 == 0, "split_f32_ranged: null argument or n %% 8 != 0");
  MVG_REQUIRE(scale > 0.f, "split_f32_ranged: scale must be positive (a power of two keeps the round trip exact)");
  if (n == 0) return 0;
  hipStream_t st = (hipStream_t)stream;
  ProfScope ps(MVG_K_LAYOUT, st, 0.0, (4.0 + SP_BYTES) * (double)n);
  long long blocks = (n / 8 + 255) / 256;
  if (blocks > 8192) blocks = 8192;
  hipLaunchKernelGGL(split_f32_ranged_kernel, dim3((unsigned)blocks), dim3(256), 0, st, (const float4 *)x, (uint4 *)out_sp, (long long)(n / 8), scale,
                     (unsigned *)range_word);
  return check_launch("split_f32_ranged");
}

int mvg_merge_sp(const void *x_sp, float *out, int64_t n, float inv_scale, void *stream) {
  MVG_REQUIRE(x_sp && out && n >= 0 && n % 8 == 0, "merge_sp: null argument or n %% 8 != 0");
  if (n == 0) return 0;
  hipStream_t st = (hipStream_t)stream;
  ProfScope ps(MVG_K_LAYOUT, st, 0.0, (4.0 + SP_BYTES) * (double)n);
  long long blocks = (n / 8 + 255) / 256;
  if (blocks > 8192) blocks = 8192;
  hipLaunchKernelGGL(merge_sp_kernel, dim3((unsigned)blocks), dim3(256), 0, st, (const uint4 *)x_sp, (float4 *)out, (long long)(n / 8), inv_scale);
  return check_launch("merge_sp");
}

int mvg_split_weights(const mvg_conv_desc *d, const float *w, void *w_krsc_sp, void *w_crsk_sp, float *stat2, void *items_dev,
                      void *stream) {
  MVG_REQUIRE(d && w && w_krsc_sp && stat2 && items_dev, "split_weights: null argument");
  if (validate_split(d)) return 2;
  hipStream_t st = (hipStream_t)stream;
  WPrepItem it;
  memset(&it, 0, sizeof(it));
  it.w = w;
  it.wk = w_krsc_sp;
  it.wt = w_crsk_sp;
  it.cout = d->cout;
  it.rs = d->r * d->s;
  it.cin = d->cin;
  it.cin_pad = d->cin;
  it.stat = stat2;
  static_assert(sizeof(WPrepItem) <= 64, "WPrepItem grew: update the callers' table record size");
  hipLaunchKernelGGL(wprep_stage_item_kernel, dim3(1), dim3(64), 0, st, it, (WPrepItem *)items_dev);
  if (check_launch("split_weights: staging the table record")) return 1;
  const long long n8 = (long long)d->cout * it.rs * d->cin / 8;
  long long blocks = (n8 + 256 * 8 - 1) / (256 * 8);
  return mvg_weights_prep_batch(items_dev, 1, 1, (int)(blocks < 16 ? 16 : (blocks > 2048 ? 2048 : blocks)), stream);
}

int mvg_weights_prep_batch(const void *items_dev, int n, int mode, int blocks_per_item, void *stream) {
  MVG_REQUIRE(items_dev != nullptr && n > 0 && (mode == 0 || mode == 1) && blocks_per_item >= 0 && blocks_per_item <= 4096,
              "weights_prep_batch: bad arguments");
  hipStream_t st = (hipStream_t)stream;
  ProfScope ps(MVG_K_LAYOUT, st, 0.0, 0.0);
  const unsigned bx = blocks_per_item > 0 ? (unsigned)blocks_per_item : 64u;
  if (mode == 1) {
    hipLaunchKernelGGL(weights_absmax_kernel, dim3(bx > 64 ? bx / 2 : 16, (unsigned)n), dim3(256), 0, st, (const WPrepItem *)items_dev);
    if (check_launch("weights_absmax")) return 1;
  }
  hipLaunchKernelGGL(weights_prep_batch_kernel, dim3(bx, (unsigned)n), dim3(256), 0, st, (const WPrepItem *)items_dev, mode);
  return check_launch("weights_prep_batch");
}

int mvg_conv_stats_partials_split(const mvg_conv_desc *d, int32_t *rows_per_partial) {
  if (validate_split(d)) return -1;
  const long long rows = (long long)d->n * d->ho * d->wo;
  if (rows_per_partial) *rows_per_partial = 64;
  return ceil_div(rows, SP_BM) * 2;
}

struct SplitAffine {
  const float *scale, *shift;
  const void *residual;
  int residual_sp, relu, out_sp;
  int lin;
  float *out_absmax, *out_sinv;
  const float *bias_absmax;
  uint32_t *range_word;
};

struct SplitFwdApply {
  const float *y, *scale, *shift, *res_scale, *res_shift, *res_sinv;
  const void *res;
  uint8_t *bits;
};

static int fprop_split_impl(const mvg_conv_desc *d, const void *x_sp, const float *x_sinv, const void *w_sp, const float *w_sinv,
                            void *y, float *stats, void *stream, const SplitAffine *aff, int stride_w = -1, int pad_w = -1,
                            const SplitFwdApply *fap = nullptr) {
  if (stride_w < 0 && validate_split(d)) return 2;
  IgemmParams p;
  memset(&p, 0, sizeof(p));
  p.a = (const float *)x_sp;
  p.b = (const float *)w_sp;
  p.a_sinv = x_sinv;
  p.b_sinv = w_sinv;
  p.out = (float *)y;
  p.stats = stats;
  if (aff) {
    p.scale = aff->scale;
    p.bias = aff->shift;
    p.addend = (const float *)aff->residual;
    p.addend_sp = aff->residual_sp;
    p.relu = aff->relu;
    p.out_sp = aff->out_sp;
    p.out_absmax = aff->range_word ? (unsigned *)aff->range_word : (unsigned *)aff->out_absmax;
    p.out_sinv = aff->out_sinv;
    p.bias_absmax = aff->bias_absmax;
  }
  if (fap) {
    p.fap_y = fap->y;
    p.fap_scale = fap->scale;
    p.fap_shift = fap->shift;
    p.fap_res = fap->res;
    p.fap_res_scale = fap->res_scale;
    p.fap_res_shift = fap->res_shift;
    p.fap_res_sinv = fap->res_sinv;
    p.fap_bits = (unsigned short *)fap->bits;
  }
  if (fprop_geometry(p, d, SP_BYTES, SP_BYTES, "split conv", stride_w, pad_w)) return 2;
  MVG_REQUIRE(p.rows_per_group * (long long)d->cout < (1ll << 31), "split conv: a group of the output exceeds 2^31 elements");
  const double flops = 2.0 * d->groups * (double)p.rows_per_group * d->cout * d->r * d->s * d->cin * (stride_w >= 0 ? 147.0 / 224.0 : 1.0);
  const double bytes = (double)SP_BYTES * (d->groups * (double)d->n * d->h * d->w * d->cin + (double)d->cout * d->r * d->s * d->cin) +
                       4.0 * d->groups * (double)p.rows_per_group * d->cout +
                       (fap ? 8.0 + 1.0 / 4.0 : 0.0) * d->groups * (double)d->n * d->h * d->w * d->cin;
  const bool lin = d->r == 1 && d->s == 1 && d->h == 1 && d->w == 1;
  ProfScope ps(lin ? MVG_K_LINEAR_FPROP : MVG_K_CONV_FPROP, (hipStream_t)stream, flops, bytes);
  p.stats_partials = ceil_div(p.rows_per_group, SP_BM) * 2;
  return launch_igemm_split<false>(p, (hipStream_t)stream, aff && aff->lin, d->r * d->s, p.rows_per_group,
                                   fap ? (fap->res_scale ? A_OUT_AFFINE : A_OUT_SP) : A_DMA, aff && aff->range_word);
}

int mvg_conv_fprop_split(const mvg_conv_desc *d, const void *x_sp, const float *x_sinv, const void *w_sp, const float *w_sinv, float *y,
                         float *stats, void *stream) {
  return fprop_split_impl(d, x_sp, x_sinv, w_sp, w_sinv, y, stats, stream, nullptr);
}

int mvg_conv_fprop_split_stages(const mvg_conv_desc *d) {
  if (validate_split(d)) return -1;
  IgemmClass c;
  memset(&c, 0, sizeof(c));
  c.rows_per_group = (long long)d->n * d->ho * d->wo;
  c.ktotal = d->r * d->s * d->cin;
  const SplitPlan pl = split_plan(d->cout, d->r * d->s, c.rows_per_group, d->groups, false, &c, 1);
  return split_conv_stages(pl);
}

int mvg_conv_fprop_split_bnapply(const mvg_conv_desc *d, void *out_sp, const float *out_sinv, const float *bn_y, const float *scale,
                                 const float *shift, const void *residual, int residual_sp, const float *res_scale,
                                 const float *res_shift, const float *res_sinv, uint8_t *relu_bits, const void *w_sp,
                                 const float *w_sinv, float *y, float *stats, void *stream) {
  MVG_REQUIRE(d && out_sp && bn_y && scale && shift && residual && w_sp && y, "fprop_split_bnapply: null argument");
  MVG_REQUIRE(d->r == 1 && d->s == 1 && d->stride == 1 && d->pad == 0, "fprop_split_bnapply: 1x1, stride 1, pad 0 only");
  MVG_REQUIRE(d->cout == 64 || d->cout == 128, "fprop_split_bnapply: cout must be 64 or 128 (one column tile; got %d)", d->cout);
  MVG_REQUIRE(d->cin % 32 == 0 && d->cin <= BNA_MAX_C, "fprop_split_bnapply: cin must be a multiple of 32, at most %d (got %d)", BNA_MAX_C,
              d->cin);
  MVG_REQUIRE(residual_sp ? (!res_scale && !res_shift) : (res_scale && res_shift && !res_sinv),
              "fprop_split_bnapply: the residual is an sp identity (no res_scale / res_shift) or fp32 with res_scale and res_shift");
  MVG_REQUIRE((long long)d->n * d->h * d->w * d->cin < (1ll << 29), "fprop_split_bnapply: a group of the input exceeds 2 GiB");
  const SplitFwdApply a = {bn_y, scale, shift, res_scale, res_shift, res_sinv, residual, relu_bits};
  return fprop_split_impl(d, out_sp, out_sinv, w_sp, w_sinv, y, stats, stream, nullptr, -1, -1, &a);
}

int mvg_conv_fprop_split_affine(const mvg_conv_desc *d, const void *x_sp, const float *x_sinv, const void *w_sp, const float *w_sinv,
                                void *out, int out_sp, const float *scale, const float *shift, const void *residual, int residual_sp,
                                int relu, void *stream) {
  MVG_REQUIRE(scale && shift && out, "fprop_split_affine: scale, shift and out are required");
  const SplitAffine a = {scale, shift, residual, residual_sp, relu, out_sp, 0, nullptr, nullptr, nullptr, nullptr};
  return fprop_split_impl(d, x_sp, x_sinv, w_sp, w_sinv, out, nullptr, stream, &a);
}

int mvg_conv_fprop_split_affine_ranged(const mvg_conv_desc *d, const void *x_sp, const float *x_sinv, const void *w_sp, const float *w_sinv,
                                       void *out, int out_sp, const float *scale, const float *shift, const void *residual,
                                       int residual_sp, int relu, uint32_t *range_word, void *stream) {
  MVG_REQUIRE(scale && shift && out, "fprop_split_affine_ranged: scale, shift and out are required");
  MVG_REQUIRE(range_word && out_sp, "fprop_split_affine_ranged: range_word is required and the output must be sp (out_sp != 0)");
  const SplitAffine a = {scale, shift, residual, residual_sp, relu, out_sp, 0, nullptr, nullptr, nullptr, range_word};
  return fprop_split_impl(d, x_sp, x_sinv, w_sp, w_sinv, out, nullptr, stream, &a);
}

struct SplitBnFuse {
  const float *y;
  const uint8_t *bits;
  const float *mean, *invstd, *rscale, *rshift;
  float *part;
  int part_rows;
};

struct SplitBnApply {
  const float *dz, *y, *mean, *invstd, *gamma, *s1, *s2;
  long long rows_per_group;
};

static int dgrad_split_impl(const mvg_conv_desc *d, const void *dy_sp, const float *dy_sinv, const void *w_crsk_sp, const float *w_sinv,
                            float *dx, const float *addend, void *stream, const SplitBnFuse *bnf, const void *relu_mask_sp = nullptr,
                            bool lin_kernel = false, float *out_absmax = nullptr, const SplitBnApply *bna = nullptr) {
  if (validate_split(d)) return 2;
  IgemmParams p;
  memset(&p, 0, sizeof(p));
  p.a = (const float *)dy_sp;
  p.b = (const float *)w_crsk_sp;
  p.a_sinv = dy_sinv;
  p.b_sinv = w_sinv;
  p.out = dx;
  p.addend = addend;
  p.mask = (const float *)relu_mask_sp;
  p.mask_sp = relu_mask_sp != nullptr;
  p.out_absmax = (unsigned *)out_absmax;
  if (bnf) {
    p.bn_y = bnf->y;
    p.bn_bits = bnf->bits;
    p.bn_mean = bnf->mean;
    p.bn_invstd = bnf->invstd;
    p.bn_rscale = bnf->rscale;
    p.bn_rshift = bnf->rshift;
    p.bn_part = bnf->part;
    p.bn_part_rows = bnf->part_rows;
  }
  if (bna) {
    p.bna_dz = bna->dz;
    p.bna_y = bna->y;
    p.bna_mean = bna->mean;
    p.bna_invstd = bna->invstd;
    p.bna_gamma = bna->gamma;
    p.bna_s1 = bna->s1;
    p.bna_s2 = bna->s2;
    p.bna_inv_rows = 1.0f / (float)bna->rows_per_group;
  }
  if (dgrad_geometry(p, d, SP_BYTES, SP_BYTES, "split conv")) return 2;
  MVG_REQUIRE((long long)d->n * d->h * d->w * d->cin < (1ll << 31), "split conv: a group of dx exceeds 2^31 elements");
  const double flops = 2.0 * d->groups * (double)d->n * d->ho * d->wo * d->cout * d->r * d->s * d->cin;
  const double bytes = (double)SP_BYTES * (d->groups * (double)d->n * d->ho * d->wo * d->cout + (double)d->cout * d->r * d->s * d->cin) +
                       (bnf ? 8.25 : 4.0) * d->groups * (double)d->n * d->h * d->w * d->cin +
                       (bna ? 8.0 : 0.0) * d->groups * (double)d->n * d->ho * d->wo * d->cout;
  const bool lin = d->r == 1 && d->s == 1 && d->h == 1 && d->w == 1;
  ProfScope ps(lin ? MVG_K_LINEAR_DGRAD : MVG_K_CONV_DGRAD, (hipStream_t)stream, flops, bytes);
  if (int e = dgrad_classes(p, d, bnf != nullptr, 4, dx, addend, (hipStream_t)stream)) return e;
  if (p.ncls == 0) return 0;
  return launch_igemm_split<true>(p, (hipStream_t)stream, lin_kernel, d->r * d->s, (long long)d->n * d->h * d->w, bna ? A_DY : A_DMA);
}

int mvg_conv_dgrad_split(const mvg_conv_desc *d, const void *dy_sp, const float *dy_sinv, const void *w_crsk_sp, const float *w_sinv,
                         float *dx, const float *addend, const void *relu_mask_sp, void *stream) {
  MVG_REQUIRE(!relu_mask_sp || d->stride == 1, "dgrad_split: the sp ReLU mask is for stride-1 launches (Linear layers)");
  return dgrad_split_impl(d, dy_sp, dy_sinv, w_crsk_sp, w_sinv, dx, addend, stream, nullptr, relu_mask_sp);
}

int mvg_conv_dgrad_split_stages(const mvg_conv_desc *d, int fused_reduce) {
  if (validate_split(d)) return -1;
  IgemmParams p;
  memset(&p, 0, sizeof(p));
  if (dgrad_geometry(p, d, SP_BYTES, SP_BYTES, "split conv")) return -1;
  DgradDropped dropped;
  dgrad_plan_classes(p, d, fused_reduce != 0, dropped);
  return split_conv_stages(split_plan(p.ncols, d->r * d->s, (long long)d->n * d->h * d->w, p.groups, false, p.cls, p.ncls));
}

int mvg_conv_dgrad_bn_partials_split(const mvg_conv_desc *d) {
  if (validate_split(d)) return -1;
  return dgrad_bn_partials(d, split_tile_rows(d->cin, d->r * d->s, (long long)d->n * d->h * d->w));
}

static int dgrad_split_bnreduce_impl(const char *who, const mvg_conv_desc *d, const void *dy_sp, const float *dy_sinv, const void *w_crsk_sp,
                                     const float *w_sinv, float *dx, const float *addend, const float *bn_y, const uint8_t *bn_bits,
                                     const float *bn_mean, const float *bn_invstd, const float *relu_scale, const float *relu_shift,
                                     float *partials, float *s1, float *s2, float *dgamma, float *dbeta, int accumulate, float *mx,
                                     const float *bn_gamma, float *dx_dy_sinv, void *stream, const SplitBnApply *bna) {
  MVG_REQUIRE(bn_y && bn_mean && bn_invstd && partials && s1 && s2, "%s: null argument", who);
  MVG_REQUIRE((bn_gamma == nullptr) == (dx_dy_sinv == nullptr) && (!dx_dy_sinv || mx), "%s: bn_gamma, dx_dy_sinv (and mx) go together", who);
  MVG_REQUIRE(!(bn_bits && relu_scale) && ((relu_scale == nullptr) == (relu_shift == nullptr)),
              "%s: give the ReLU mask either as bits or as (relu_scale, relu_shift)", who);
  const int P = mvg_conv_dgrad_bn_partials_split(d);
  MVG_REQUIRE(P > 0, "%s: bad descriptor", who);
  const SplitBnFuse f = {bn_y, bn_bits, bn_mean, bn_invstd, relu_scale, relu_shift, partials, mx ? 3 : 2};
  if (dgrad_split_impl(d, dy_sp, dy_sinv, w_crsk_sp, w_sinv, dx, addend, stream, &f, nullptr, false, nullptr, bna)) return 1;
  ProfScope ps(MVG_K_BN_BWD_REDUCE, (hipStream_t)stream, 0.0, 8.0 * d->groups * (double)P * d->cin);
  return bn_bwd_finalize_launch(partials, d->groups, P, d->cin, s1, s2, dgamma, dbeta, accumulate, (hipStream_t)stream, mx, nullptr, nullptr,
                                bn_gamma, bn_invstd, (long long)d->n * d->h * d->w, dx_dy_sinv);
}

int mvg_conv_dgrad_split_bnreduce(const mvg_conv_desc *d, const void *dy_sp, const float *dy_sinv, const void *w_crsk_sp,
                                  const float *w_sinv, float *dx, const float *addend, const float *bn_y, const uint8_t *bn_bits,
                                  const float *bn_mean, const float *bn_invstd, const float *relu_scale, const float *relu_shift,
                                  float *partials, float *s1, float *s2, float *dgamma, float *dbeta, int accumulate,
                                  float *mx, const float *bn_gamma, float *dx_dy_sinv, void *stream) {
  return dgrad_split_bnreduce_impl("dgrad_split_bnreduce", d, dy_sp, dy_sinv, w_crsk_sp, w_sinv, dx, addend, bn_y, bn_bits, bn_mean, bn_invstd,
                                   relu_scale, relu_shift, partials, s1, s2, dgamma, dbeta, accumulate, mx, bn_gamma, dx_dy_sinv, stream, nullptr);
}

int mvg_conv_dgrad_split_bnapply_bnreduce(const mvg_conv_desc *d, void *dy_sp, const float *dy_sinv, const float *dz, const float *y,
                                          const float *mean, const float *invstd, const float *gamma, const float *un_s1,
                                          const float *un_s2, int64_t rows_per_group, const void *w_crsk_sp, const float *w_sinv,
                                          float *dx, const float *addend, const float *bn_y, const uint8_t *bn_bits,
                                          const float *bn_mean, const float *bn_invstd, const float *relu_scale,
                                          const float *relu_shift, float *partials, float *s1, float *s2, float *dgamma, float *dbeta,
                                          int accumulate, float *mx, const float *bn_gamma, float *dx_dy_sinv, void *stream) {
  MVG_REQUIRE(d && dy_sp && dz && y && mean && invstd && gamma && un_s1 && un_s2 && w_crsk_sp && dx,
              "dgrad_split_bnapply_bnreduce: null argument");
  MVG_REQUIRE(dy_sinv, "dgrad_split_bnapply_bnreduce: dy_sinv (the 2^-k the reduce pass left for this unit's dy) is required");
  MVG_REQUIRE(d->r == 1 && d->s == 1 && d->stride == 1 && d->pad == 0, "dgrad_split_bnapply_bnreduce: 1x1, stride 1, pad 0 only");
  MVG_REQUIRE(d->cin == 64 || d->cin == 128, "dgrad_split_bnapply_bnreduce: cin must be 64 or 128 (one column tile; got %d)", d->cin);
  MVG_REQUIRE(d->cout % 32 == 0 && d->cout <= BNA_MAX_C, "dgrad_split_bnapply_bnreduce: cout must be a multiple of 32, at most %d (got %d)",
              BNA_MAX_C, d->cout);
  MVG_REQUIRE(rows_per_group == (int64_t)d->n * d->ho * d->wo, "dgrad_split_bnapply_bnreduce: rows_per_group is not n * ho * wo");
  const SplitBnApply a = {dz, y, mean, invstd, gamma, un_s1, un_s2, (long long)rows_per_group};
  return dgrad_split_bnreduce_impl("dgrad_split_bnapply_bnreduce", d, dy_sp, dy_sinv, w_crsk_sp, w_sinv, dx, addend, bn_y, bn_bits, bn_mean,
                                   bn_invstd, relu_scale, relu_shift, partials, s1, s2, dgamma, dbeta, accumulate, mx, bn_gamma, dx_dy_sinv, stream, &a);
}

static void wgrad_split_tile(const mvg_conv_desc *d, int &bm, int &bn, bool &incr) {
  incr = (long long)d->ho * d->wo >= 32;
  const int ncols = d->r * d->s * d->cin;
  bm = d->cout >= 128 ? 128 : 64;
  bn = ncols >= 128 ? 128 : 64;
  if (bm == 128 && ncols >= 256 && ncols % 256 == 0) bn = 256;
  else if (ncols % 192 == 0) bn = 192;
}

int mvg_conv_wgrad_splits_split(const mvg_conv_desc *d) {
  if (validate_split(d)) return -1;
  int bm, bn;
  bool incr;
  wgrad_split_tile(d, bm, bn, incr);
  const long long tiles = (long long)ceil_div(d->cout, bm) * ceil_div(d->r * d->s * d->cin, bn);
  return wgrad_split_count(tiles, (long long)d->groups * d->n * d->ho * d->wo, bn == 256 ? 2 : 3, 256);
}

int mvg_conv_wgrad_split_tile(const mvg_conv_desc *d, int32_t *bm, int32_t *bn, int32_t *incremental) {
  if (validate_split(d)) return -1;
  int tm, tn;
  bool incr;
  wgrad_split_tile(d, tm, tn, incr);
  if (bm) *bm = tm;
  if (bn) *bn = tn;
  if (incremental) *incremental = incr ? 1 : 0;
  return 0;
}

static int wgrad_split_impl(const mvg_conv_desc *d, const void *x_sp, const void *dy_sp, const float *dy_sinv, float *dw, float *workspace,
                            int splits, int accumulate, void *stream, int stride_w = -1, int pad_w = -1, const float *x_sinv = nullptr,
                            bool slabs_only = false) {
  if (stride_w < 0 && validate_split(d)) return 2;
  WgradParams p;
  memset(&p, 0, sizeof(p));
  p.x = (const float *)x_sp;
  p.dy = (const float *)dy_sp;
  p.dy_sinv = dy_sinv;
  p.x_sinv = x_sinv;
  if (wgrad_geometry(p, d, SP_BYTES, 16, dw, nullptr, workspace, splits, accumulate, "wgrad_split", stride_w, pad_w)) return 2;
  int bm, bn;
  bool incr;
  wgrad_split_tile(d, bm, bn, incr);
  p.mtiles = ceil_div(d->cout, bm);
  p.ntiles = ceil_div(p.ncols, bn);
  hipStream_t st = (hipStream_t)stream;
  const bool lin = d->r == 1 && d->s == 1 && d->h == 1 && d->w == 1;
  {
    const double flops = 2.0 * (double)p.pixels * d->cout * d->r * d->s * d->cin * (stride_w >= 0 ? 147.0 / 224.0 : 1.0);
    const double bytes = (double)SP_BYTES * ((double)d->groups * d->n * d->h * d->w * d->cin + (double)p.pixels * d->cout) +
                         4.0 * (double)d->cout * d->r * d->s * d->cin;
    ProfScope ps(lin ? MVG_K_LINEAR_WGRAD : MVG_K_CONV_WGRAD, st, flops, bytes);
    MVG_REQUIRE((long long)p.mtiles * p.ntiles * splits < (1LL << 31), "wgrad_split: grid too large");
    dim3 grid(p.mtiles * p.ntiles * splits), block(256);
#define MVG_WGRAD_SPLIT(BM_, BN_)                                                                  \
  do {                                                                                             \
    if (incr) hipLaunchKernelGGL((wgrad_split_kernel<BM_, BN_, true>), grid, block, 0, st, p);     \
    else hipLaunchKernelGGL((wgrad_split_kernel<BM_, BN_, false>), grid, block, 0, st, p);         \
  } while (0)
    if (bm == 128 && bn == 256) MVG_WGRAD_SPLIT(128, 256);
    else if (bm == 128 && bn == 192) MVG_WGRAD_SPLIT(128, 192);
    else if (bm == 64 && bn == 192) MVG_WGRAD_SPLIT(64, 192);
    else if (bm == 128 && bn == 128) MVG_WGRAD_SPLIT(128, 128);
    else if (bm == 64 && bn == 128) MVG_WGRAD_SPLIT(64, 128);
    else if (bm == 128 && bn == 64) MVG_WGRAD_SPLIT(128, 64);
    else MVG_WGRAD_SPLIT(64, 64);
#undef MVG_WGRAD_SPLIT
    if (check_launch("conv_wgrad_split")) return 1;
  }
  return splits > 1 && !slabs_only ? wgrad_reduce_slabs(p, workspace, dw, nullptr, splits, accumulate, st, "wgrad_split") : 0;
}

int mvg_conv_wgrad_split_xs(const mvg_conv_desc *d, const void *x_sp, const float *x_sinv, const void *dy_sp, const float *dy_sinv,
                            float *dw, float *workspace, int splits, int accumulate, void *stream) {
  MVG_REQUIRE(d && x_sp && dy_sp && dw, "wgrad_split: d, x_sp, dy_sp and dw are required");
  return wgrad_split_impl(d, x_sp, dy_sp, dy_sinv, dw, workspace, splits, accumulate, stream, -1, -1, x_sinv);
}

int mvg_conv_wgrad_split(const mvg_conv_desc *d, const void *x_sp, const void *dy_sp, const float *dy_sinv, float *dw, float *workspace,
                         int splits, int accumulate, void *stream) {
  return wgrad_split_impl(d, x_sp, dy_sp, dy_sinv, dw, workspace, splits, accumulate, stream);
}

int mvg_conv_wgrad_split_slabs_xs(const mvg_conv_desc *d, const void *x_sp, const float *x_sinv, const void *dy_sp, const float *dy_sinv,
                                  float *workspace, int splits, void *stream) {
  MVG_REQUIRE(d && x_sp && dy_sp, "wgrad_split_slabs: d, x_sp and dy_sp are required");
  MVG_REQUIRE(splits > 1 && workspace, "wgrad_split_slabs: splits > 1 and a workspace (the slabs ARE the result)");
  return wgrad_split_impl(d, x_sp, dy_sp, dy_sinv, workspace, workspace, splits, 0, stream, -1, -1, x_sinv, true);
}

int mvg_conv_wgrad_split_slabs(const mvg_conv_desc *d, const void *x_sp, const void *dy_sp, const float *dy_sinv, float *workspace, int splits,
                               void *stream) {
  MVG_REQUIRE(splits > 1 && workspace, "wgrad_split_slabs: splits > 1 and a workspace (the slabs ARE the result)");
  return wgrad_split_impl(d, x_sp, dy_sp, dy_sinv, workspace, workspace, splits, 0, stream, -1, -1, nullptr, true);
}

int mvg_wgrad_reduce_batch(const float *const *host_slabs, float *const *host_dw, const int64_t *host_n, const int32_t *host_splits,
                           const int32_t *host_accumulate, int n, void *stream) {
  MVG_REQUIRE(host_slabs && host_dw && host_n && host_splits && host_accumulate && n >= 1 && n <= 8, "wgrad_reduce_batch: 1..8 items");
  ReduceBatch b;
  memset(&b, 0, sizeof(b));
  b.n = n;
  long long blocks = 0;
  double bytes = 0.0;
  for (int i = 0; i < n; ++i) {
    MVG_REQUIRE(host_slabs[i] && host_dw[i] && host_n[i] > 0 && host_n[i] % 4 == 0 && host_splits[i] > 1, "wgrad_reduce_batch: bad item");
    ReduceItem &r = b.it[i];
    r.slabs = host_slabs[i];
    r.dw = host_dw[i];
    r.n4 = host_n[i] / 4;
    r.splits = host_splits[i];
    r.accumulate = host_accumulate[i];
    r.lanes = r.splits >= 32 ? 16 : (r.splits >= 8 ? 4 : 1);
    r.block0 = (int)blocks;
    blocks += (r.n4 + 256 / r.lanes - 1) / (256 / r.lanes);
    bytes += 4.0 * host_n[i] * (r.splits + 1);
  }
  MVG_REQUIRE(blocks < (1LL << 31), "wgrad_reduce_batch: grid too large");
  hipStream_t st = (hipStream_t)stream;
  ProfScope ps(MVG_K_WGRAD_REDUCE, st, 0.0, bytes);
  hipLaunchKernelGGL(wgrad_reduce_batch_kernel, dim3((unsigned)blocks), dim3(256), 0, st, b);
  return check_launch("wgrad_reduce_batch");
}

static mvg_conv_desc linear_desc(int rows, int fin, int fout) {
  mvg_conv_desc d;
  memset(&d, 0, sizeof(d));
  d.groups = 1; d.n = rows; d.h = d.w = d.ho = d.wo = 1; d.cin = fin; d.cout = fout; d.r = d.s = 1; d.stride = 1; d.pad = 0;
  return d;
}

int mvg_split_colsum(const float *g, int rows, int cols, const float *absmax, void *out_sp, float *out_sinv, float *db, int accumulate,
                     void *stream) {
  MVG_REQUIRE(g && absmax && out_sp && out_sinv && rows > 0 && cols > 0 && cols % 32 == 0, "split_colsum: null argument or cols %% 32 != 0");
  hipStream_t st = (hipStream_t)stream;
  ProfScope ps(MVG_K_COLSUM, st, 0.0, (4.0 + SP_BYTES) * (double)rows * cols);
  hipLaunchKernelGGL(split_colsum_kernel, dim3(cols / 32), dim3(256), 0, st, g, rows, cols, (const unsigned *)absmax, (uint4 *)out_sp, out_sinv,
                     db, accumulate);
  return check_launch("split_colsum");
}

int mvg_linear_fprop_split(int rows, int fin, int fout, const void *x_sp, const float *x_sinv, const void *w_sp, const float *w_sinv,
                           const float *bias, int relu, void *out, int out_sp, float *out_sinv, const float *bias_absmax,
                           float *out_absmax, void *stream) {
  MVG_REQUIRE(bias != nullptr && out != nullptr, "linear_fprop_split: bias and out are required");
  MVG_REQUIRE(!out_sp || out_sinv, "linear_fprop_split: an sp result needs out_sinv (it is stored scaled)");
  MVG_REQUIRE(!(out_sp && out_absmax), "linear_fprop_split: out_absmax is for fp32 results");
  const mvg_conv_desc d = linear_desc(rows, fin, fout);
  const SplitAffine a = {nullptr, bias, nullptr, 0, relu, out_sp, 1, out_absmax, out_sinv, bias_absmax, nullptr};
  return fprop_split_impl(&d, x_sp, x_sinv, w_sp, w_sinv, out, nullptr, stream, &a);
}

int mvg_linear_dgrad_split(int rows, int fin, int fout, const void *dy_sp, const float *dy_sinv, const void *wt_sp, const float *w_sinv,
                           float *dx, const float *addend, const void *relu_mask_sp, float *out_absmax, void *stream) {
  const mvg_conv_desc d = linear_desc(rows, fin, fout);
  return dgrad_split_impl(&d, dy_sp, dy_sinv, wt_sp, w_sinv, dx, addend, stream, nullptr, relu_mask_sp, true, out_absmax);
}

int mvg_linear_wgrad_split(int rows, int fin, int fout, const void *x_sp, const float *x_sinv, const void *dy_sp, const float *dy_sinv,
                           float *dw, float *workspace, int splits, int accumulate, void *stream) {
  const mvg_conv_desc d = linear_desc(rows, fin, fout);
  return wgrad_split_impl(&d, x_sp, dy_sp, dy_sinv, dw, workspace, splits, accumulate, stream, -1, -1, x_sinv);
}

static int stem_desc(const mvg_conv_desc *d, mvg_conv_desc *rw) {
  MVG_REQUIRE(d != nullptr, "stem (row-window): null descriptor");
  MVG_REQUIRE(d->r == 7 && d->s == 7 && d->stride == 2 && d->pad == 3 && d->cin == 4, "stem (row-window): 7x7 stride 2 pad 3, 4 stored channels");
  MVG_REQUIRE(d->w % 2 == 0 && d->ho == (d->h - 1) / 2 + 1 && d->wo == d->w / 2, "stem (row-window): even width; ho, wo inconsistent");
  MVG_REQUIRE(d->cout % 32 == 0 && d->groups > 0 && d->n > 0, "stem (row-window): cout must be a multiple of 32");
  *rw = *d;
  rw->w = d->wo;
  rw->cin = 32;
  rw->s = 1;
  return 0;
}

int mvg_stem_rowwindow_split(const float *x_nhwc4, void *xw_sp, int64_t images, int h, int w, void *stream) {
  MVG_REQUIRE(x_nhwc4 && xw_sp && images > 0 && h > 0 && w > 0 && w % 2 == 0, "stem_rowwindow: bad arguments (even width)");
  hipStream_t st = (hipStream_t)stream;
  const long long n = images * h * (w / 2) * 4;
  ProfScope ps(MVG_K_LAYOUT, st, 0.0, 16.0 * (double)images * h * w + 32.0 * (double)n);
  long long blocks = (n + 255) / 256;
  if (blocks > 16384) blocks = 16384;
  hipLaunchKernelGGL(stem_rowwindow_kernel, dim3((unsigned)blocks), dim3(256), 0, st, (const float4 *)x_nhwc4, (uint4 *)xw_sp, n, h, w);
  return check_launch("stem_rowwindow");
}

int mvg_stem_rowwindow_split_nchw(const float *x_nchw, void *xw_sp, int64_t images, int h, int w, void *stream) {
  MVG_REQUIRE(x_nchw && xw_sp && images > 0 && h > 0 && w > 0 && w % 2 == 0, "stem_rowwindow (NCHW): bad arguments (even width)");
  hipStream_t st = (hipStream_t)stream;
  const long long n = images * h * (w / 2) * 4;
  ProfScope ps(MVG_K_LAYOUT, st, 0.0, 12.0 * (double)images * h * w + 32.0 * (double)n);
  long long blocks = (n + 255) / 256;
  if (blocks > 16384) blocks = 16384;
  hipLaunchKernelGGL(stem_rowwindow_nchw_kernel, dim3((unsigned)blocks), dim3(256), 0, st, x_nchw, (uint4 *)xw_sp, n, h, w);
  return check_launch("stem_rowwindow_nchw");
}

int mvg_stem_fprop_split(const mvg_conv_desc *d, const void *xw_sp, const void *w_sp, const float *w_sinv, float *y, float *stats,
                         void *stream) {
  mvg_conv_desc rw;
  if (stem_desc(d, &rw)) return 2;
  return fprop_split_impl(&rw, xw_sp, nullptr, w_sp, w_sinv, y, stats, stream, nullptr, 1, 0);
}

int mvg_stem_wgrad_splits_split(const mvg_conv_desc *d) {
  mvg_conv_desc rw;
  if (stem_desc(d, &rw)) return -1;
  const long long tiles = (long long)ceil_div(rw.cout, rw.cout >= 128 ? 128 : 64) * ceil_div(7 * 32, 128);
  return wgrad_split_count(tiles, (long long)rw.groups * rw.n * rw.ho * rw.wo, 3, 256);
}

int mvg_stem_wgrad_split(const mvg_conv_desc *d, const void *xw_sp, const void *dy_sp, const float *dy_sinv, float *dw_rw, float *workspace,
                         int splits, int accumulate, void *stream) {
  mvg_conv_desc rw;
  if (stem_desc(d, &rw)) return 2;
  return wgrad_split_impl(&rw, xw_sp, dy_sp, dy_sinv, dw_rw, workspace, splits, accumulate, stream, 1, 0);
}

}
```

### rot-mvgaze_amd/csrc/conv_split_igemm.inc

```
#ifndef MVG_SPLIT_RNG
#error "conv_split_igemm.inc: define MVG_SPLIT_RNG (0 or 1) before including"
#endif

#if MVG_SPLIT_RNG
template <int BN, int WGM = 2, int STAGES = 1>
__global__ __launch_bounds__(256, STAGES == 2 ? 2 : WGM == 4 ? 3 : 4) void igemm_split16_ranged_kernel(IgemmParams p) {
  constexpr bool DGRAD = false, LIN = false;
  constexpr AForm AF = A_DMA;
#else
template <int BN, bool DGRAD, bool LIN = false, int WGM = 2, int STAGES = 1, AForm AF = A_DMA>
__global__ __launch_bounds__(256, STAGES == 2 ? 2 : (DGRAD || WGM == 4 || AF != A_DMA) ? 3 : 4) void igemm_split16_kernel(IgemmParams p) {
#endif
  constexpr int BM = 64 * WGM, WGN = 4 / WGM, NW = 4;
  static_assert(WGM == 2 || (WGM == 4 && BN == 64), "tiles: 128 x BN (2 x 2 waves) or 256 x 64 (4 x 1)");
  static_assert(STAGES == 1 || STAGES == 2, "one LDS stage, or the two-stage pipeline");
  static_assert(AF == A_DMA || (DGRAD == (AF == A_DY) && !LIN && WGM == 2 && STAGES == 1),
                "operand-forming loaders: dy in backward-data, the block output in forward; 128-row tiles, one stage");
  using Former = std::conditional_t<AF == A_DY, DyFormer, OutFormer<AF == A_OUT_AFFINE>>;
  constexpr int WTM = BM / WGM, WTN = BN / WGN;
  constexpr int TM = WTM / 16, TN = WTN / 16;
  constexpr int SLOTS = 4 * SP_NP;
  constexpr int ROWB = 16 * SLOTS, ROWS = BM + BN, STAGE_B = ROWS * ROWB;
  constexpr int NQ = ROWS * SLOTS / 64;
  constexpr int QA = BM * SLOTS / 64;
  constexpr int A_PER = QA / NW, B_PER = (NQ - QA) / NW;
  static_assert(QA % NW == 0 && (NQ - QA) % NW == 0, "whole instructions per wave");
  constexpr int EPI_B = bf16_epilogue_bytes<BM, BN, WGM, DGRAD>();
  constexpr int INFO_OFF = STAGES * STAGE_B > EPI_B ? STAGES * STAGE_B : EPI_B;
  constexpr int BNK_OFF = INFO_OFF + BM * 8;
  constexpr int SMEM_B = BNK_OFF + (AF != A_DMA ? Former::TABLES : 0) * BNA_MAX_C * 4;
  __shared__ __attribute__((aligned(16))) unsigned char smem[SMEM_B];

  const int tid = threadIdx.x;
  const int lane = tid & 63, wave = __builtin_amdgcn_readfirstlane(tid >> 6);
  const int wm = wave / WGN, wn = wave % WGN;
  const int nwg = gridDim.x;
  const int wg_all = p.no_remap ? (int)blockIdx.x : xcd_remap(blockIdx.x, nwg);
  int ci = 0;
  for (int i = 1; i < p.ncls; ++i) ci += wg_all >= p.cls[i].tile0;
  const IgemmClass &c = p.cls[ci];
  const int wg = wg_all - c.tile0;
  const int ntile = wg % p.ntiles;
  const int mt_all = wg / p.ntiles;
  const int g = mt_all / c.mtiles_per_group;
  const int mtile = mt_all - g * c.mtiles_per_group;
  const int KT = c.KT;
  const int ohw = c.out_h * c.out_w;

  uint2 *rowinfo = reinterpret_cast<uint2 *>(smem + INFO_OFF);
  if (tid < BM) {
    const long long m = (long long)mtile * BM + tid;
    const bool ok = m < c.rows_per_group;
    const int mm = ok ? (int)m : 0;
    const int img = (int)fdiv((unsigned)mm, c.ohw_div);
    const int rem = mm - img * ohw;
    const int oy = (int)fdiv((unsigned)rem, c.ow_div), ox = rem - oy * c.out_w;
    const int y0 = DGRAD ? oy + c.cls_cy : oy * p.stride - p.pad;
    const int x0 = DGRAD ? ox + c.cls_cx : ox * p.stride_w - p.pad_w;
    const unsigned base = (unsigned)(img * p.src_img_stride * SP_BYTES) + (unsigned)((y0 * p.src_w + x0) * p.src_c) * (unsigned)SP_BYTES;
    unsigned msk = 0;
    for (int t = 0; t < c.ntaps; ++t) {
      const int fr = (int)fdiv((unsigned)t, c.tap_ns_div), fs = t - fr * c.tap_ns;
      const int iy = DGRAD ? y0 - fr : y0 + fr;
      const int ix = DGRAD ? x0 - fs : x0 + fs;
      msk |= (unsigned)(((unsigned)iy < (unsigned)p.src_h) & ((unsigned)ix < (unsigned)p.src_w)) << t;
    }
    rowinfo[tid] = make_uint2(base, ok ? msk : 0u);
  }
  if constexpr (AF != A_DMA) Former::stage(reinterpret_cast<float *>(smem + BNK_OFF), p, g, p.src_c, tid);
  __syncthreads();
  unsigned a_base[A_PER], a_vmask[A_PER], b_base[B_PER];
#pragma unroll
  for (int i = 0; i < A_PER; ++i) {
    const int sl = (wave + NW * i) * 64 + lane;
    const int row = sl / SLOTS, j = (sl % SLOTS) ^ sp_row_swz(row);
    const uint2 ri = rowinfo[row];
    a_base[i] = ri.x + 16u * (unsigned)j;
    a_vmask[i] = ri.y;
  }
#pragma unroll
  for (int i = 0; i < B_PER; ++i) {
    const int sl = (wave + NW * (A_PER + i)) * 64 + lane - BM * SLOTS;
    const int row = sl / SLOTS, j = (sl % SLOTS) ^ sp_row_swz(row);
    const int n = ntile * BN + row;
    b_base[i] = pred_off(((unsigned)n * (unsigned)p.b_row_len) * (unsigned)SP_BYTES + 16u * (unsigned)j, n < p.ncols);
  }
  const __amdgpu_buffer_rsrc_t rs_a =
      make_rsrc(reinterpret_cast<const char *>(p.a) + (long long)g * p.imgs_per_group * p.src_img_stride * SP_BYTES, p.a_group_bytes);
  const __amdgpu_buffer_rsrc_t rs_b = make_rsrc(p.b, p.b_bytes);
  typedef __attribute__((address_space(3))) void *lds_vp;

  auto issue = [&](int kt, int stage_off) {
    int kstart = kt * SP_BK;
    if (c.korder) {
      const int cblk = (int)fdiv((unsigned)kt, c.per_div), rem = kt - cblk * c.ntaps;
      kstart = (rem << p.src_c_shift) + cblk * SP_BK;
    }
    const int ks = __builtin_amdgcn_readfirstlane(kstart);
    const int tap_u = c.ntaps > 1 ? (ks >> p.src_c_shift) : 0;
    const int chb = ks - (tap_u << p.src_c_shift);
    const int fru = (int)fdiv((unsigned)tap_u, c.tap_ns_div), fsu = tap_u - fru * c.tap_ns;
    const int disp = (fru * p.src_w + fsu) * p.src_c;
    const unsigned sdelta = (unsigned)(((DGRAD ? -disp : disp) + chb) * SP_BYTES);
    unsigned kb = (unsigned)ks * (unsigned)SP_BYTES;
    if (DGRAD) {
      const int btap = (c.tap_r0 + p.tap_step * fru) * p.s + c.tap_s0 + p.tap_step * fsu;
      kb = (unsigned)(btap * p.src_c + chb) * (unsigned)SP_BYTES;
    }
    if constexpr (AF == A_DMA) {
#pragma unroll
      for (int i = 0; i < A_PER; ++i) {
        const bool ok = ((a_vmask[i] >> tap_u) & 1u) != 0u;
        __builtin_amdgcn_raw_ptr_buffer_load_lds(rs_a, (lds_vp)(smem + stage_off + (wave + NW * i) * 1024), 16, (int)pred_off(a_base[i] + sdelta, ok), 0, 0, 0);
      }
    }
#pragma unroll
    for (int i = 0; i < B_PER; ++i)
      __builtin_amdgcn_raw_ptr_buffer_load_lds(rs_b, (lds_vp)(smem + stage_off + (wave + NW * (A_PER + i)) * 1024), 16, (int)(b_base[i] + kb), 0, 0, 0);
  };

  f32x4 acc[TM][TN];
#pragma unroll
  for (int i = 0; i < TM; ++i)
#pragma unroll
    for (int j = 0; j < TN; ++j)
#pragma unroll
      for (int e = 0; e < 4; ++e) acc[i][j][e] = 0.f;

  const int cc_l = lane >> 4;
  int a_off[TM][SP_NP], b_off[TN][SP_NP];
#pragma unroll
  for (int i = 0; i < TM; ++i) {
    const int R = wm * WTM + i * 16 + (lane & 15);
#pragma unroll
    for (int pc = 0; pc < SP_NP; ++pc) a_off[i][pc] = R * ROWB + (((2 * cc_l + pc) ^ sp_row_swz(R)) << 4);
  }
#pragma unroll
  for (int j = 0; j < TN; ++j) {
    const int R = wn * WTN + j * 16 + (lane & 15);
#pragma unroll
    for (int pc = 0; pc < SP_NP; ++pc) b_off[j][pc] = (BM + R) * ROWB + (((2 * cc_l + pc) ^ sp_row_swz(R)) << 4);
  }

  auto load_frags = [&](const unsigned char *stage, f16x8 (&av)[SP_NP][TM], f16x8 (&bv)[SP_NP][TN]) {
#pragma unroll
    for (int pc = 0; pc < SP_NP; ++pc) {
#pragma unroll
      for (int i = 0; i < TM; ++i) av[pc][i] = *reinterpret_cast<const f16x8 *>(stage + a_off[i][pc]);
#pragma unroll
      for (int j = 0; j < TN; ++j) bv[pc][j] = *reinterpret_cast<const f16x8 *>(stage + b_off[j][pc]);
    }
  };
  auto products = [&](const f16x8 (&av)[SP_NP][TM], const f16x8 (&bv)[SP_NP][TN]) { SPLIT16_ONE(0, 1) SPLIT16_ONE(1, 0) SPLIT16_ONE(0, 0) };
  if constexpr (AF != A_DMA) {
    const int C = p.src_c;
    const int a_cc = tid & 3, a_r0 = tid >> 2;
    const long long grow0 = (long long)g * c.rows_per_group;
    Former f(p, grow0, c.rows_per_group, C);
    uint4 *a_out = reinterpret_cast<uint4 *>(const_cast<float *>(p.a)) + grow0 * C / 4;
    bool a_ok[2];
    unsigned a_goff[2];
#pragma unroll
    for (int i = 0; i < 2; ++i) {
      const long long m = (long long)mtile * BM + a_r0 + 64 * i;
      a_ok[i] = m < c.rows_per_group;
      a_goff[i] = pred_off((unsigned)m * (unsigned)C * 4u + 32u * (unsigned)a_cc, a_ok[i]);
    }
    auto a_load = [&](int kt) {
#pragma unroll
      for (int i = 0; i < 2; ++i) f.load(i, a_goff[i] + 128u * (unsigned)kt);
    };
    constexpr bool PREFETCH = BN == 64;
    if (PREFETCH) a_load(0);
    for (int kt = 0; kt < KT; ++kt) {
      issue(kt, 0);
      if (!PREFETCH) a_load(kt);
      uint4 q[2][SP_NP];
      f.consts(reinterpret_cast<const float *>(smem + BNK_OFF) + kt * SP_BK + a_cc * 8, C);
#pragma unroll
      for (int i = 0; i < 2; ++i) {
        float o[8];
        f.form(i, a_ok[i], o);
        split2_chunk(o, q[i][0], q[i][1]);
        const int R = a_r0 + 64 * i;
#pragma unroll
        for (int pc = 0; pc < SP_NP; ++pc)
          *reinterpret_cast<uint4 *>(smem + R * ROWB + (((2 * a_cc + pc) ^ sp_row_swz(R)) << 4)) = q[i][pc];
      }
      asm volatile("s_waitcnt vmcnt(0)" ::: "memory");
      __syncthreads();
#pragma unroll
      for (int i = 0; i < 2; ++i)
        if (a_ok[i]) {
          const unsigned off = a_goff[i] + 128u * (unsigned)kt;
          uint4 *dst = a_out + (off >> 4);
          dst[0] = q[i][0];
          dst[1] = q[i][1];
          f.store_extra(i, off);
        }
      if (PREFETCH && kt + 1 < KT) a_load(kt + 1);
      {
        f16x8 av[SP_NP][TM], bv[SP_NP][TN];
        load_frags(smem, av, bv);
        products(av, bv);
      }
      __syncthreads();
    }
  } else if constexpr (STAGES == 1) {
    for (int kt = 0; kt < KT; ++kt) {
      issue(kt, 0);
      asm volatile("s_waitcnt vmcnt(0)" ::: "memory");
      __syncthreads();
      {
        f16x8 av[SP_NP][TM], bv[SP_NP][TN];
        load_frags(smem, av, bv);
        products(av, bv);
      }
      __syncthreads();
    }
  } else {
    constexpr int G = A_PER + B_PER;
    if (KT > 0) issue(0, 0);
    if (KT > 1) {
      issue(1, STAGE_B);
      asm volatile("s_waitcnt vmcnt(%0)\n\ts_barrier" ::"n"(G) : "memory");
    } else {
      asm volatile("s_waitcnt vmcnt(0)\n\ts_barrier" ::: "memory");
    }
    f16x8 a0[SP_NP][TM], b0[SP_NP][TN], a1[SP_NP][TM], b1[SP_NP][TN];
    load_frags(smem, a0, b0);
    int cur = 0;
    auto step = [&](int kt, const f16x8 (&ca)[SP_NP][TM], const f16x8 (&cb)[SP_NP][TN], f16x8 (&na)[SP_NP][TM], f16x8 (&nb)[SP_NP][TN]) {
      if (kt + 1 < KT) {
        asm volatile("s_waitcnt vmcnt(0) lgkmcnt(0)\n\ts_barrier" ::: "memory");
        if (kt + 2 < KT) issue(kt + 2, cur);
        cur ^= STAGE_B;
        load_frags(smem + cur, na, nb);
      }
      products(ca, cb);
    };
    for (int kt = 0; kt < KT; kt += 2) {
      step(kt, a0, b0, a1, b1);
      if (kt + 1 < KT) step(kt + 1, a1, b1, a0, b0);
    }
    __syncthreads();
  }
#if MVG_SPLIT_RNG
  bf16_epilogue<BM, BN, WGM, DGRAD, true, WGM, true, DGRAD, LIN, WGN, false, true>(p, c, acc, reinterpret_cast<unsigned short *>(smem), tid, g, mtile,
                                                                                     ntile);
#else
  bf16_epilogue<BM, BN, WGM, DGRAD, true, WGM, true, DGRAD, LIN, WGN>(p, c, acc, reinterpret_cast<unsigned short *>(smem), tid, g, mtile, ntile);
#endif
}
```

### rot-mvgaze_amd/heads.py

```python
from __future__ import annotations

from typing import Dict, List, Optional, Tuple

import torch

from . import ops
from ._lib import ConvDesc
from .arch import DEFAULT_VARIANT, NUM_FEAT_VEC, ROT_DIM, Variant
from .backbone import GradSink

Tensor = torch.Tensor
IBN_MOMENTUM, IBN_EPS = 0.05, 1e-4
SPLIT_MIN_ROWS = 1024


def directed_pairs(views: int) -> Tuple[List[int], List[int]]:
    vi, vj = [], []
    for i in range(views):
        for j in range(i + 1, views):
            vi += [i, j]
            vj += [j, i]
    return vi, vj


# ... 82 lines not shown
            rows, dev = x.shape[0], x.device
            assert x.shape[1] == self.fin_p[0], (x.shape, self.fin_p[0])
        hs: List[Tensor] = []
        cur = x
        for l in range(self.n):
            w, b = self._weights(l)
            last = l == self.n - 1
            y = out if (last and out is not None) else torch.empty(rows, self.fout_p[l], dtype=torch.float32, device=dev)
            if self._use_mixed(l):
                assert gen is None
                if self._wbf[l] is None:
                    self._wbf[l] = ops.cast_weights_bf16(ConvDesc.linear(1, self.fin_p[l], self.fout_p[l]), w, self.fin_p[l], True)
                ops.linear_fprop_mixed(cur, self._wbf[l][0], b, not last, y, rows, self.fin_p[l], self.fout_p[l])
            elif l == 0 and gen is not None:
                ops.fuser_fprop(gen.img, gen.feat, gen.rel, gen.row_img, gen.row_src, w, b, not last, y, rows, gen.cf, gen.nvec,
                                self.fout_p[l])
            elif last and self.fout[l] <= 4:
                ops.linear_skinny_fwd(cur, w, b, y, rows, self.fin_p[l], self.fout[l])
            else:
                ops.linear_fprop(cur, w, b, not last, y, rows, self.fin_p[l], self.fout_p[l])
            if not last:
                hs.append(y)
            cur = y
        return hs, cur

    def backward(self, x: Optional[Tensor], hs: List[Tensor], gy: Tensor, sink: GradSink, wr: _Written,
                 dx_addend: Optional[Tensor] = None, dx_out: Optional[Tensor] = None, gen: Optional["_GenInput"] = None) -> Tensor:
        rows, dev = gy.shape[0], gy.device
        g = gy
        for l in range(self.n - 1, -1, -1):
            inp = x if l == 0 else hs[l - 1]
            w, _ = self._weights(l) if self.padded[l] else (self.w[l].detach(), None)
            last = l == self.n - 1
            fin, fout = self.fin_p[l], self.fout_p[l]
            if self.padded[l]:
                accs = (wr.acc(self.w[l]), wr.acc(self.b[l]))

                def padded_grads(inp=inp, g=g, l=l, fin=fin, fout=fout, accs=accs):
                    dwp = torch.empty(fout, fin, dtype=torch.float32, device=dev)
                    dbp = torch.empty(fout, dtype=torch.float32, device=dev)
                    ops.linear_wgrad(inp, g, dwp, dbp, rows, fin, fout, False)
                    for p, src, a in ((self.w[l], dwp[: self.fout[l], : self.fin[l]], accs[0]),
                                      (self.b[l], dbp[: self.fout[l]], accs[1])):
                        if a:
                            sink.view(p).add_(src)
                        else:
                            sink.view(p).copy_(src)
                wr.off_path(padded_grads, inp, g)
            elif last and self.fout[l] <= 4:
                aw, ab = wr.acc(self.w[l]), wr.acc(self.b[l])
                assert aw == ab
                dh = torch.empty(rows, fin, dtype=torch.float32, device=dev)
                ops.linear_skinny_bwd(g, inp, w, inp, dh, sink.view(self.w[l]), sink.view(self.b[l]), rows, fin, self.fout[l], aw)
                g = dh
                continue
            else:
                aw, ab = wr.acc(self.w[l]), wr.acc(self.b[l])

                assert aw == ab

                def grads(inp=inp, g=g, l=l, fin=fin, fout=fout, aw=aw):
                    if self._use_mixed(l):
                        ops.linear_wgrad_mixed(inp, g, sink.view(self.w[l]), sink.view(self.b[l]), rows, fin, fout, aw)
                    elif l == 0 and gen is not None:
                        ops.fuser_wgrad(gen.img, gen.feat, gen.rel, gen.row_img, gen.row_src, g, sink.view(self.w[l]),
                                        sink.view(self.b[l]), rows, gen.cf, gen.nvec, fout, aw)
                    else:
                        ops.linear_wgrad(inp, g, sink.view(self.w[l]), sink.view(self.b[l]), rows, fin, fout, aw)
                if l == 0 and gen is not None:
                    wr.off_path(grads, gen.img, gen.feat, g, *([gen.rel] if gen.rel is not None else []))
                else:
                    wr.off_path(grads, inp, g)
            mixed = self._use_mixed(l)
            if l == 0:
                dx = dx_out if dx_out is not None else torch.empty(rows, fin, dtype=torch.float32, device=dev)
                if mixed:
                    ops.linear_dgrad_mixed(g, self._wbf[l][1], None, dx_addend, dx, rows, fin, fout)
                else:
                    ops.linear_dgrad(g, w, None, dx_addend, dx, rows, fin, fout)
                return dx
            dh = torch.empty(rows, fin, dtype=torch.float32, device=dev)
            if mixed:
                ops.linear_dgrad_mixed(g, self._wbf[l][1], hs[l - 1], None, dh, rows, fin, fout)
            else:
                ops.linear_dgrad(g, w, hs[l - 1], None, dh, rows, fin, fout)
            g = dh
        raise AssertionError("unreachable")


class FusionHead:
    def __init__(self, params: Dict[str, Tensor], fc_dim: int, num_iter: int, variant: Variant = DEFAULT_VARIANT):
        self.cf, self.I, self.v = fc_dim, num_iter, variant
        self.lifter = _Mlp(params, "_lifter._lifter.", 2)
        three = variant.encode_rotmat or variant.share_feature
        self.fusers = [_Mlp(params, f"_img_fusers.{i}._fuser.", 3 if three else 2) for i in range(num_iter)]
        self.heads = [_Mlp(params, f"_gaze_estimators.{i}.", 2) for i in range(num_iter)]
        if variant.share_weights:
            self.fusers = [self.fusers[0]] * num_iter
            self.heads = [self.heads[0]] * num_iter
        self.ibn = [params[f"_img_fusers.{i}._batchnorm.running_mean"] for i in range(num_iter)] \
            if variant.share_feature else None
        self.fused_input = True
        self.mixed = False
        self.split = True
        self.kin = self.fusers[0].in_width
        self.hin = self.heads[0].in_width
        self._idx_cache: Dict[Tuple[int, str], dict] = {}
        self._wprep_state = None
        self._wsp_versions = None
        self.keep_infer_copies = True
        self._wbf_infer_ok = False

    def invalidate_weight_cache(self):
        self._wbf_infer_ok = False

    def _prepare_split_weights(self, rows: int, dev, mixed: bool = False, reuse: bool = False):
        mods = [m for m in self.unique_modules()]
        if mixed:
            mods = [self.lifter] + mods
            layers = [(m, l) for m in mods for l in range(m.n) if m._use_mixed(l)]
        else:
            layers = [(m, l) for m in mods for l in range(m.n) if m._use_split(l, rows)]
        key = (str(dev), mixed, tuple(m.w[l].data_ptr() for m, l in layers))
        if self._wprep_state is None or self._wprep_state[0] != key:
            wstat = torch.zeros(len(layers), 2, dtype=torch.float32, device=dev)
            rows_t, bufs = [], []
            for i, (m, l) in enumerate(layers):
                fin, fout = m.fin[l], m.fout[l]
                if mixed:
                    wk = torch.empty(fout, 1, 1, fin, dtype=torch.bfloat16, device=dev)
                    wt = torch.empty(fin, 1, 1, fout, dtype=torch.bfloat16, device=dev)
                else:
                    wk, wt = ops.sp_empty(fout, fin, device=dev), ops.sp_empty(fin, fout, device=dev)
                    wk.sinv = wt.sinv = wstat[i, 1:2]
                bufs.append((m, l, wk, wt))
                rows_t.append([m.w[l].data_ptr(), wk.data_ptr(), wt.data_ptr(), fout | (1 << 32), fin | (fin << 32), wstat[i].data_ptr()])
            table = torch.tensor(rows_t, dtype=torch.int64).to(dev) if rows_t else None
            self._wprep_state = (key, bufs, table, wstat)
            self._wbf_infer_ok = False
        _, bufs, table, wstat = self._wprep_state
        for m in mods:
            m._wsp = [None] * m.n
            m._wbf = [None] * m.n
        if table is None:
            return
        if mixed and reuse and self._wbf_infer_ok and self._wsp_versions == tuple(m.w[l]._version for m, l, _, _ in bufs):
            for m, l, wk, wt in bufs:
                m._wbf[l] = (wk, wt)
            return
        self._wbf_infer_ok = mixed and reuse
        if not mixed:
            wstat.zero_()
        ops.weights_prep_batch(table, len(bufs), 0 if mixed else 1, 256)
        for m, l, wk, wt in bufs:
            if mixed:
                m._wbf[l] = (wk, wt)
            else:
                m._wsp[l] = (wk, wt)
        self._wsp_versions = tuple(m.w[l]._version for m, l, _, _ in bufs)

    def unique_modules(self) -> List[_Mlp]:
        out, seen = [], set()
        for it in range(self.I - 1, -1, -1):
            for m in (self.heads[it], self.fusers[it]):
                if id(m) not in seen:
                    seen.add(id(m))
                    out.append(m)
        return out

    def _indices(self, views: int, dev) -> dict:
        key = (views, str(dev))
        if key not in self._idx_cache:
            vi, vj = directed_pairs(views)
            D = len(vi)
            mk = lambda a: torch.tensor(a, dtype=torch.int32, device=dev)
            self._idx_cache[key] = {"vi": mk(vi), "vj": mk(vj), "partner": mk([d ^ 1 for d in range(D)]),
                                    "ident": mk(list(range(D))), "D": D}
        return self._idx_cache[key]

    def _row_tables(self, views: int, batch: int, dev) -> dict:
        key = (views, batch, str(dev), "rows")
        if key not in self._idx_cache:
            vi, vj = directed_pairs(views)
            D = len(vi)
            b = torch.arange(batch, dtype=torch.int32)
            tab = lambda idx: (torch.tensor(idx, dtype=torch.int32)[:, None] * batch + b[None, :]).reshape(-1).contiguous().to(dev)
            self._idx_cache[key] = {"img": tab(vi), "view": tab(vj), "partner": tab([d ^ 1 for d in range(D)]),
                                    "ident": tab(list(range(D)))}
        return self._idx_cache[key]

    def _fuser_input(self, a: Tensor, src: Tensor, rel: Tensor, vi, src_idx, B: int, D: int, scales):
        dev, v = a.device, self.v
        X = torch.empty(D * B, self.kin, dtype=torch.float32, device=dev)
        if v.share_feature:
            ops.paircat_fwd(a, src, rel, scales, vi, src_idx, X, B, D, NUM_FEAT_VEC)
        elif v.encode_rotmat:
            ops.rotcat_ext_fwd(a, src, None, rel, vi, src_idx, X, self.kin, B, D, self.cf, NUM_FEAT_VEC)
        else:
            ops.rotcat_fwd(a, src, None if v.ignore_rotmat else rel, vi, src_idx, X, B, D, self.cf, NUM_FEAT_VEC)
        return X

    def _head_input(self, a: Tensor, feat: Tensor, vi, ident, B: int, D: int):
        Xh = torch.empty(D * B, self.hin, dtype=torch.float32, device=a.device)
        if self.v.share_feature:
            ops.paircat_fwd(a, feat, None, None, vi, ident, Xh, B, D, NUM_FEAT_VEC)
        else:
            ops.rotcat_fwd(a, feat, None, vi, ident, Xh, B, D, self.cf, NUM_FEAT_VEC)
        return Xh

    def forward(self, img_feat: Tensor, rot: Tensor, keep_tape: bool, training: bool = True):
        V, B, cf = img_feat.shape
        dev = img_feat.device
        ix = self._indices(V, dev)
        D, I, NV = ix["D"], self.I, NUM_FEAT_VEC
        split_on = self.split and not self.mixed and not (self.v.share_feature or self.v.encode_rotmat) and D * B >= SPLIT_MIN_ROWS
        for m in [self.lifter] + self.fusers + self.heads:
            m.mixed = self.mixed
            m.split = split_on
            m._wbf = [None] * m.n
        self.lifter.split = False
        if split_on:
            return self._forward_split(img_feat, rot, keep_tape, ix)
        if self.mixed:
            self._prepare_split_weights(D * B, dev, mixed=True, reuse=self.keep_infer_copies and not keep_tape and not training)
        hl, lifted = self.lifter.forward(img_feat.reshape(V * B, cf))
        rel = torch.empty(D, B, 3, 3, dtype=torch.float32, device=dev)
        ops.relative_rotation(rot.detach().to(torch.float32).contiguous(), ix["vi"], ix["vj"], rel, B, V, D)
        feats = torch.empty(I, D * B, ROT_DIM, dtype=torch.float32, device=dev)
        preds = torch.empty(I, D * B, 2, dtype=torch.float32, device=dev)
        a = lifted if self.v.share_feature else img_feat
        saved = []
        src, src_idx = lifted, ix["vj"]
        fused_in = self.fused_input and not (self.v.share_feature or self.v.encode_rotmat) and not self.mixed and not split_on
        rt = self._row_tables(V, B, dev) if fused_in else None
        img2d = img_feat.reshape(V * B, cf)
        for it in range(I):
            scales = None
            if fused_in:
                gen_f = _GenInput(img2d, src.reshape(-1, ROT_DIM), None if self.v.ignore_rotmat else rel, rt["img"],
                                  rt["view"] if it == 0 else rt["partner"], cf, NV)
                Hf, Fn = self.fusers[it].forward(None, feats[it], gen=gen_f)
                gen_h = _GenInput(img2d, Fn, None, rt["img"], rt["ident"], cf, NV)
                Hh, _ = self.heads[it].forward(None, preds[it], gen=gen_h)
                if keep_tape:
                    saved.append((gen_f, Hf, gen_h, Hh, None))
                src, src_idx = Fn, ix["partner"]
                continue
            if self.v.share_feature:
                scales = torch.empty(2 * D, NV, dtype=torch.float32, device=dev)
                ops.ibn_scales(a, src, ix["vi"], src_idx, self.ibn[it], training, IBN_MOMENTUM, IBN_EPS, scales, B, D, NV)
            X = self._fuser_input(a, src, rel, ix["vi"], src_idx, B, D, scales)
            Hf, Fn = self.fusers[it].forward(X, feats[it])
            Xh = self._head_input(a, Fn, ix["vi"], ix["ident"], B, D)
            Hh, _ = self.heads[it].forward(Xh, preds[it])
            if keep_tape:
                saved.append((X, Hf, Xh, Hh, scales))
            src, src_idx = Fn, ix["partner"]
        tape = {"img_feat": img_feat, "lifted": lifted, "hl": hl, "rel": rel, "saved": saved, "V": V, "B": B, "mode": "mixed" if self.mixed else "fp32",
                "wbf": {id(m): list(m._wbf) for m in [self.lifter] + self.fusers + self.heads},
                "wsp_versions": self._wsp_versions if self.mixed else None} if keep_tape else None
        return lifted.view(V, B, 3, NV), feats.view(I, D, B, 3, NV), preds.view(I, D, B, 2), tape

    _SLOTS = 64

    def _forward_split(self, img_feat: Tensor, rot: Tensor, keep_tape: bool, ix: dict):
        V, B, cf = img_feat.shape
        dev = img_feat.device
        D, I, NV = ix["D"], self.I, NUM_FEAT_VEC
        rows, kin = D * B, self.kin
        assert 2 + I <= 8 and 11 * I + 2 <= self._SLOTS
        self._prepare_split_weights(rows, dev)
        st = torch.zeros(self._SLOTS, dtype=torch.float32, device=dev)
        names: Dict[str, int] = {}

        def slot(name: str) -> Tensor:
            i = names.setdefault(name, len(names))
            return st[i:i + 1]

        def sp(r: int, c: int, name: str) -> Tensor:
            t = ops.sp_empty(r, c, device=dev)
            t.sinv = slot(name)
            return t
        for m in [self.lifter] + self.fusers + self.heads:
            m.split = False
        hl, lifted = self.lifter.forward(img_feat.reshape(V * B, cf))
        rel = torch.empty(D, B, 3, 3, dtype=torch.float32, device=dev)
        ops.relative_rotation(rot.detach().to(torch.float32).contiguous(), ix["vi"], ix["vj"], rel, B, V, D)
        rel_fuse = None if self.v.ignore_rotmat else rel
        rt = self._row_tables(V, B, dev)
        img2d = img_feat.reshape(V * B, cf)
        ops.absmax_multi([img2d, lifted] + [self.fusers[it].b[0].detach() for it in range(I)],
                         [slot("am_img"), slot("am_lift")] + [slot(f"bam{it}") for it in range(I)])
        feats = torch.empty(I, rows, ROT_DIM, dtype=torch.float32, device=dev)
        preds = torch.empty(I, rows, 2, dtype=torch.float32, device=dev)
        hh = torch.empty(I, rows, self.heads[0].fout[0], dtype=torch.float32, device=dev)
        xf = sp(rows, kin, "xf0")
        ops.fuse_build_split(img2d, lifted, rel_fuse, rt["img"], rt["view"], None, xf, None, slot("am_img"), slot("am_lift"), rows, cf, NV)
        saved = []
        for it in range(I):
            fu, hd = self.fusers[it], self.heads[it]
            wf0, wf1, wh0 = fu._wsp[0], fu._wsp[1], hd._wsp[0]
            hid, hhid = fu.fout[0], hd.fout[0]
            h = sp(rows, hid, f"h{it}")
            ops.linear_fprop_split(xf, wf0[0], fu.b[0].detach(), True, h, rows, kin, hid, bias_absmax=slot(f"bam{it}"))
            ops.linear_fprop_split(h, wf1[0], fu.b[1].detach(), False, feats[it], rows, hid, ROT_DIM, out_absmax=slot(f"amF{it}"))
            xh = sp(rows, kin, f"xh{it}")
            xf_next = sp(rows, kin, f"xf{it + 1}") if it + 1 < I else None
            ops.fuse_build_split(img2d, feats[it], rel_fuse, rt["img"], rt["partner"], rt["ident"], xf_next, xh, slot("am_img"),
                                 slot(f"amF{it}"), rows, cf, NV)
            ops.linear_fprop_split(xh, wh0[0], hd.b[0].detach(), True, hh[it], rows, kin, hhid)
            ops.linear_skinny_fwd(hh[it], hd.w[1].detach(), hd.b[1].detach(), preds[it], rows, hhid, 2)
            if keep_tape:
                saved.append((xf, h, xh, hh[it], wf0, wf1, wh0))
            xf = xf_next
        tape = {"img_feat": img_feat, "lifted": lifted, "hl": hl, "rel": rel, "saved": saved, "V": V, "B": B, "mode": "split",
                "st": st, "slot": slot, "wsp_versions": self._wsp_versions} if keep_tape else None
        return lifted.view(V, B, 3, NV), feats.view(I, D, B, 3, NV), preds.view(I, D, B, 2), tape

    def _backward_split(self, tape: dict, d_lifted: Optional[Tensor], d_feats: Optional[Tensor], d_preds: Optional[Tensor],
                        sink: GradSink, side=None) -> Tensor:
        V, B, cf, v = tape["V"], tape["B"], self.cf, self.v
        img_feat, rel, st, slot = tape["img_feat"], tape["rel"], tape["st"], tape["slot"]
        dev = img_feat.device
        ix = self._indices(V, dev)
        D, NV, I = ix["D"], NUM_FEAT_VEC, self.I
        rows, kin = D * B, self.kin
        wr = _Written(sink, side)
        rel_fuse = None if v.ignore_rotmat else rel
        da = torch.empty(V, B, cf, dtype=torch.float32, device=dev)
        da_live = False
        dXn: Optional[Tensor] = None

        def sp(r: int, c: int, name: str) -> Tensor:
            t = ops.sp_empty(r, c, device=dev)
            t.sinv = slot(name)
            return t

        def wgrad(x_sp, g_sp, p, fin, fout, acc):
            wr.off_path(lambda: ops.linear_wgrad_split(x_sp, g_sp, sink.view(p), rows, fin, fout, acc), x_sp, g_sp, st)

        for it in range(I - 1, -1, -1):
            xf, h, xh, hh, wf0, wf1, wh0 = tape["saved"][it]
            fu, hd = self.fusers[it], self.heads[it]
            hid, hhid = fu.fout[0], hd.fout[0]
            dXh = None
            if d_preds is not None:
                gp = d_preds[it].reshape(rows, 2).contiguous()
                a1, ab1 = wr.acc(hd.w[1]), wr.acc(hd.b[1])
                assert a1 == ab1
                dhh = torch.empty(rows, hhid, dtype=torch.float32, device=dev)
                ops.linear_skinny_bwd(gp, hh, hd.w[1].detach(), hh, dhh, sink.view(hd.w[1]), sink.view(hd.b[1]), rows, hhid, 2, a1,
                                      dx_absmax=slot(f"am_dhh{it}"))
                a0, ab0 = wr.acc(hd.w[0]), wr.acc(hd.b[0])
                assert a0 == ab0
                g_hh = sp(rows, hhid, f"g_hh{it}")
                ops.split_colsum(dhh, rows, hhid, slot(f"am_dhh{it}"), g_hh, sink.view(hd.b[0]), ab0)
                wgrad(xh, g_hh, hd.w[0], kin, hhid, a0)
                dXh = torch.empty(rows, kin, dtype=torch.float32, device=dev)
                ops.linear_dgrad_split(g_hh, wh0[1], dXh, rows, kin, hhid)
            else:
                self._zero_grads(hd, sink, wr)
            ext = d_feats[it].reshape(rows, ROT_DIM).contiguous() if d_feats is not None else None
            if dXh is None and dXn is None and ext is None:
                self._zero_grads(fu, sink, wr)
                if not v.share_weights:
                    sink.publish(hd.parameters() + fu.parameters())
                continue
            am_dF = slot(f"am_dF{it}")
            if dXh is None and dXn is None:
                dF = ext.clone()
            else:
                dF = torch.empty(rows, ROT_DIM, dtype=torch.float32, device=dev)
                ops.fuse_unbuild(dXh, dXn, rel_fuse, ix["partner"], ix["vi"], dF, da, da_live, D, V, D, B, cf, NV,
                                 absmax=am_dF if ext is None else None)
                da_live = True
                if ext is not None:
                    ops.axpby(ext, dF, 1.0, 1.0)
            if ext is not None:
                ops.absmax_multi([dF], [am_dF])
            a1, ab1 = wr.acc(fu.w[1]), wr.acc(fu.b[1])
            assert a1 == ab1
            g_F = sp(rows, ROT_DIM, f"g_F{it}")
            ops.split_colsum(dF, rows, ROT_DIM, am_dF, g_F, sink.view(fu.b[1]), ab1)
            wgrad(h, g_F, fu.w[1], hid, ROT_DIM, a1)
            dh = torch.empty(rows, hid, dtype=torch.float32, device=dev)
            ops.linear_dgrad_split(g_F, wf1[1], dh, rows, hid, ROT_DIM, relu_mask_sp=h, out_absmax=slot(f"am_dh{it}"))
            a0, ab0 = wr.acc(fu.w[0]), wr.acc(fu.b[0])
            assert a0 == ab0
            g_h = sp(rows, hid, f"g_h{it}")
            ops.split_colsum(dh, rows, hid, slot(f"am_dh{it}"), g_h, sink.view(fu.b[0]), ab0)
            wgrad(xf, g_h, fu.w[0], kin, hid, a0)
            dXn = torch.empty(rows, kin, dtype=torch.float32, device=dev)
            ops.linear_dgrad_split(g_h, wf0[1], dXn, rows, kin, hid)
            if not v.share_weights:
                sink.publish(hd.parameters() + fu.parameters())
        if v.share_weights:
            sink.publish(self.heads[0].parameters() + self.fusers[0].parameters())
        dlift, dlift_live = None, False
        if dXn is not None:
            dlift = torch.empty(V * B, ROT_DIM, dtype=torch.float32, device=dev)
            ops.fuse_unbuild(None, dXn, rel_fuse, ix["vj"], ix["vi"], dlift, da, da_live, V, V, D, B, cf, NV)
            da_live = dlift_live = True
        if d_lifted is not None:
            ext = d_lifted.reshape(V * B, ROT_DIM).contiguous()
            if dlift_live:
                ops.axpby(ext, dlift, 1.0, 1.0)
            else:
                dlift, dlift_live = ext.clone(), True
        dimg = da
        if dlift_live:
            self.lifter.split = self.lifter.mixed = False
            self.lifter.backward(img_feat.reshape(V * B, cf), tape["hl"], dlift, sink, wr,
                                 dx_addend=dimg.view(V * B, cf) if da_live else None, dx_out=dimg.view(V * B, cf))
            da_live = True
        else:
            self._zero_grads(self.lifter, sink, wr)
        sink.publish(self.lifter.parameters())
        if not da_live:
            dimg.zero_()
        return dimg

    def backward(self, tape: dict, d_lifted: Optional[Tensor], d_feats: Optional[Tensor], d_preds: Optional[Tensor],
                 sink: GradSink, side=None) -> Tensor:
        V, B, cf, v = tape["V"], tape["B"], self.cf, self.v
        if tape.get("wsp_versions") is not None and tape["wsp_versions"] != self._wsp_versions:
            raise RuntimeError("backward of a tape whose sp weight copies were overwritten by a later forward with DIFFERENT "
                               "weights (forward, optimizer step, forward, then backward of the first call): run backward "
                               "before the weights change")
        if tape.get("mode") == "split":
            return self._backward_split(tape, d_lifted, d_feats, d_preds, sink, side)
        for m in [self.lifter] + self.fusers + self.heads:
            m.split = False
            m.mixed = tape.get("mode") == "mixed"
            if "wbf" in tape:
                m._wbf = list(tape["wbf"][id(m)])
        img_feat, rel = tape["img_feat"], tape["rel"]
        dev = img_feat.device
        ix = self._indices(V, dev)
        D, NV = ix["D"], NUM_FEAT_VEC
        wr = _Written(sink, side)
        aw = ROT_DIM if v.share_feature else cf
        da = torch.empty(V, B, aw, dtype=torch.float32, device=dev)
        da_live = False
        dF_next: Optional[Tensor] = None
        dlift = torch.empty(V * B, ROT_DIM, dtype=torch.float32, device=dev)
        dlift_live = False
        rel_fuse = None if (v.ignore_rotmat or v.encode_rotmat) else rel

        def split_input_grad(dX: Tensor, ld: int, rel_b, scales, src_idx, dsrc: Tensor):
            nonlocal da_live
            if v.share_feature:
                da_dir = torch.empty(D * B, ROT_DIM, dtype=torch.float32, device=dev)
                ops.paircat_bwd(dX, rel_b, scales, src_idx, da_dir, dsrc, B, D, NV)
                ops.segment_sum(da_dir, ROT_DIM, ROT_DIM, ix["vi"], da, B, D, V, da_live)
            else:
                ops.segment_sum(dX, ld, cf, ix["vi"], da, B, D, V, da_live)
                if ld == cf + ROT_DIM:
                    ops.rotcat_bwd(dX, rel_b, src_idx, dsrc, B, D, cf, NV)
                else:
                    ops.rotcat_ext_bwd(dX, ld, rel_b, src_idx, dsrc, B, D, cf, NV)
            da_live = True

        for it in range(self.I - 1, -1, -1):
            X, Hf, Xh, Hh, scales = tape["saved"][it]
            dF = dF_next
            if d_feats is not None:
                ext = d_feats[it].reshape(D * B, ROT_DIM).contiguous()
                if dF is None:
                    dF = ext.clone()
                else:
                    ops.axpby(ext, dF, 1.0, 1.0)
            gen_f = X if isinstance(X, _GenInput) else None
            gen_h = Xh if isinstance(Xh, _GenInput) else None
            if d_preds is not None:
                gp = d_preds[it].reshape(D * B, 2).contiguous()
                dXh = self.heads[it].backward(None if gen_h else Xh, Hh, gp, sink, wr, gen=gen_h)
                dFh = torch.empty(D * B, ROT_DIM, dtype=torch.float32, device=dev)
                split_input_grad(dXh, self.hin, None, None, ix["ident"], dFh)
                if dF is None:
                    dF = dFh
                else:
                    ops.axpby(dFh, dF, 1.0, 1.0)
            else:
                self._zero_grads(self.heads[it], sink, wr)
            dF_next = None
            if dF is None:
                self._zero_grads(self.fusers[it], sink, wr)
            else:
                dX = self.fusers[it].backward(None if gen_f else X, Hf, dF, sink, wr, gen=gen_f)
                if it > 0:
                    dF_next = torch.empty(D * B, ROT_DIM, dtype=torch.float32, device=dev)
                    split_input_grad(dX, self.kin, rel_fuse, scales, ix["partner"], dF_next)
                else:
                    tmp = torch.empty(D * B, ROT_DIM, dtype=torch.float32, device=dev)
                    split_input_grad(dX, self.kin, rel_fuse, scales, ix["ident"], tmp)
                    ops.segment_sum(tmp, ROT_DIM, ROT_DIM, ix["vj"], dlift, B, D, V, False)
                    dlift_live = True
            if not v.share_weights:
                sink.publish(self.heads[it].parameters() + self.fusers[it].parameters())
        if v.share_weights:
            sink.publish(self.heads[0].parameters() + self.fusers[0].parameters())
        if d_lifted is not None:
            ext = d_lifted.reshape(V * B, ROT_DIM).contiguous()
            if dlift_live:
                ops.axpby(ext, dlift, 1.0, 1.0)
            else:
                dlift, dlift_live = ext.clone(), True
        if v.share_feature and da_live:
            if dlift_live:
                ops.axpby(da.view(V * B, ROT_DIM), dlift, 1.0, 1.0)
            else:
                dlift, dlift_live = da.view(V * B, ROT_DIM), True
        dimg = da if not v.share_feature else torch.empty(V, B, cf, dtype=torch.float32, device=dev)
        dimg_live = da_live and not v.share_feature
        if dlift_live:
            self.lifter.backward(img_feat.reshape(V * B, cf), tape["hl"], dlift, sink, wr,
                                 dx_addend=dimg.view(V * B, cf) if dimg_live else None, dx_out=dimg.view(V * B, cf))
            dimg_live = True
        else:
            self._zero_grads(self.lifter, sink, wr)
        sink.publish(self.lifter.parameters())
        if not dimg_live:
            dimg.zero_()
        return dimg

    @staticmethod
    def _zero_grads(m: _Mlp, sink: GradSink, wr: _Written):
        for p in m.parameters():
            if not wr.acc(p):
                sink.view(p).zero_()
```

### rot-mvgaze_amd/ops.py

```python
from __future__ import annotations

import ctypes as C
from typing import Optional

import torch

from ._lib import ConvDesc, K_FAMILIES, ProfEntry, check, lib

Tensor = torch.Tensor


def _p(t: Optional[Tensor]):
    if t is None:
        return None
    assert t.is_cuda and t.dtype in _PTR_DTYPES, (t.device, t.dtype)
    return t.data_ptr()


_PTR_DTYPES = frozenset((torch.float32, torch.int32, torch.uint8, torch.int16, torch.bfloat16, torch.float16))
_workspaces = {}
_MAX_WORKSPACES = 8
_raw_stream = getattr(torch._C, "_cuda_getCurrentRawStream", None)


# ... 401 lines not shown

def bn_bwd_apply_split(g, y, mean, invstd, gamma, s1, s2, groups, rows_per_group, c, dy_sp, relu_affine=None, mx=None, dy_sinv=None):
    rs, rh = relu_affine if relu_affine is not None else (None, None)
    assert mx is not None and mx.dtype == torch.float32 and mx.numel() == groups * c
    ready = dy_sinv is not None
    dy_sp.sinv = dy_sinv if ready else torch.empty(1, dtype=torch.float32, device=g.device)
    check(lib().mvg_bn_bwd_apply_split(_p(g), _p(y), _p(mean), _p(invstd), _p(gamma), _p(s1), _p(s2), _p(rs), _p(rh), groups,
                                       rows_per_group, c, _p(dy_sp), _p(mx), _p(dy_sp.sinv), int(ready), _s()), "bn_bwd_apply_split")


def bn_relu_maxpool_fwd_split(y, scale, shift, pooled_sp, argmax, groups, n_per_group, h, w, c, ho, wo):
    check(lib().mvg_bn_relu_maxpool_fwd_split_scaled(_p(y), _p(scale), _p(shift), _p(pooled_sp), _sinv(pooled_sp), _p(argmax), groups,
                                                     n_per_group, h, w, c, ho, wo, _s()), "bn_relu_maxpool_fwd_split")


def avgpool_fwd_split(x_sp, y, n, hw, c):
    check(lib().mvg_avgpool_fwd_split_scaled(_p(x_sp), _sinv(x_sp), _p(y), n, hw, c, _s()), "avgpool_fwd_split")


def linear_fprop_mixed(x, w_bf16, bias, relu, y, rows, fin, fout):
    check(lib().mvg_linear_fprop_mixed(_p(x), _p(w_bf16), _p(bias), int(relu), _p(y), rows, fin, fout, _s()), "linear_fprop_mixed")


def linear_dgrad_mixed(dy, wt_bf16, mask, addend, dx, rows, fin, fout):
    check(lib().mvg_linear_dgrad_mixed(_p(dy), _p(wt_bf16), _p(mask), _p(addend), _p(dx), rows, fin, fout, _s()), "linear_dgrad_mixed")


def linear_wgrad_mixed(x, dy, dw, db, rows, fin, fout, accumulate=False):
    d = ConvDesc.linear(rows, fin, fout)
    splits, ws = _wgrad_slabs(lib().mvg_conv_wgrad_splits_bf16, "conv_wgrad_splits_bf16", d, fout * fin + fout, x.device)
    check(lib().mvg_linear_wgrad_mixed(_p(x), _p(dy), _p(dw), _p(db), rows, fin, fout, _p(ws), splits, int(accumulate), _s()),
          "linear_wgrad_mixed")


def _linear_ws(x: Tensor, rows: int, fin: int, fout: int):
    n = lib().mvg_linear_workspace_floats(rows, fin, fout)
    return torch.empty(n, dtype=torch.float32, device=x.device), n


def linear_fprop(x: Tensor, w: Tensor, bias: Optional[Tensor], relu: bool, y: Tensor, rows: int, fin: int, fout: int):
    ws, n = _linear_ws(x, rows, fin, fout)
    check(lib().mvg_linear_fprop(_p(x), _p(w), _p(bias), int(relu), _p(y), rows, fin, fout, _p(ws), n, _s(True)),
          "linear_fprop")


def linear_dgrad(dy: Tensor, w: Tensor, mask: Optional[Tensor], addend: Optional[Tensor], dx: Tensor, rows: int,
                 fin: int, fout: int):
    ws, n = _linear_ws(dy, rows, fin, fout)
    check(lib().mvg_linear_dgrad(_p(dy), _p(w), _p(mask), _p(addend), _p(dx), rows, fin, fout, _p(ws), n, _s(True)),
          "linear_dgrad")


def bn_finalize(stats, groups, partials, rows_per_partial, rows_per_group, c, gamma, beta, running_mean, running_var,
                momentum, eps, mean, invstd, scale, shift):
    check(lib().mvg_bn_finalize(_p(stats), groups, partials, rows_per_partial, rows_per_group, c, _p(gamma), _p(beta),
                                _p(running_mean), _p(running_var), momentum, eps, _p(mean), _p(invstd), _p(scale),
                                _p(shift), _s(True)), "bn_finalize")


def bn_eval_affine(groups, c, gamma, beta, running_mean, running_var, eps, scale, shift):
    check(lib().mvg_bn_eval_affine(groups, c, _p(gamma), _p(beta), _p(running_mean), _p(running_var), eps, _p(scale),
                                   _p(shift), _s()), "bn_eval_affine")


def bn_apply(y, scale, shift, residual, relu, out, groups, rows_per_group, c, residual_affine=None):
    rs, rh = residual_affine if residual_affine is not None else (None, None)
    check(_fn("mvg_bn_apply", y)(_p(y), _p(scale), _p(shift), _p(residual), _p(rs), _p(rh), int(relu), _p(out), groups,
                                 rows_per_group, c, _s()), "bn_apply")


def bn_apply_bits(y, scale, shift, residual, out, groups, rows_per_group, c, residual_affine=None):
    per = 8 if y.dtype == torch.bfloat16 else 4
    bits = torch.empty(groups * rows_per_group * c // per, dtype=torch.uint8, device=y.device)
    rs, rh = residual_affine if residual_affine is not None else (None, None)
    check(_fn("mvg_bn_apply_bits", y)(_p(y), _p(scale), _p(shift), _p(residual), _p(rs), _p(rh), _p(out), _p(bits), groups,
                                      rows_per_group, c, _s()), "bn_apply_bits")
    return bits


def bn_bwd_reduce_bits(g, bits, y, mean, invstd, groups, rows_per_group, c, s1, s2, dgamma, dbeta, accumulate, dz_out=None):
    n = lib().mvg_bn_bwd_workspace_floats(groups, rows_per_group, c)
    ws = torch.empty(n, dtype=torch.float32, device=g.device)
    check(_fn("mvg_bn_bwd_reduce_bits", g)(_p(g), _p(bits), _p(y), _p(mean), _p(invstd), groups, rows_per_group, c, _p(s1), _p(s2),
                                           _p(dgamma), _p(dbeta), int(accumulate), _p(ws), _p(dz_out), _s()), "bn_bwd_reduce_bits")


def bn_bwd_reduce(g, act, y, mean, invstd, groups, rows_per_group, c, s1, s2, dgamma, dbeta, accumulate, relu_affine=None,
                  dz_out=None):
    n = lib().mvg_bn_bwd_workspace_floats(groups, rows_per_group, c)
    ws = torch.empty(n, dtype=torch.float32, device=g.device)
    rs, rh = relu_affine if relu_affine is not None else (None, None)
    check(_fn("mvg_bn_bwd_reduce", g)(_p(g), _p(act), _p(y), _p(mean), _p(invstd), _p(rs), _p(rh), groups, rows_per_group, c,
                                  _p(s1), _p(s2), _p(dgamma), _p(dbeta), int(accumulate), _p(ws), _p(dz_out), _s()), "bn_bwd_reduce")


def bn_bwd_apply(g, act, y, mean, invstd, gamma, s1, s2, groups, rows_per_group, c, dy, dz_out=None, relu_affine=None):
    rs, rh = relu_affine if relu_affine is not None else (None, None)
    check(_fn("mvg_bn_bwd_apply", g)(_p(g), _p(act), _p(y), _p(mean), _p(invstd), _p(gamma), _p(s1), _p(s2), _p(rs), _p(rh),
                                 groups, rows_per_group, c, _p(dy), _p(dz_out), _s()), "bn_bwd_apply")


def bn_eval_bwd(g, y, gamma, running_mean, running_var, eps, groups, rows_per_group, c, dy, dgamma, dbeta, accumulate,
                act=None, relu_bits=None, relu_affine=None, dz_out=None):
    n = lib().mvg_bn_eval_bwd_workspace_floats(groups, rows_per_group, c)
    ws = torch.empty(n, dtype=torch.float32, device=g.device)
    rs, rh = relu_affine if relu_affine is not None else (None, None)
    check(lib().mvg_bn_eval_bwd(_p(_f32c(g)), _p(act), _p(relu_bits), _p(_f32c(y)), _p(rs), _p(rh), _p(gamma), _p(running_mean),
                                _p(running_var), eps, groups, rows_per_group, c, _p(_f32c(dy)), _p(dz_out), _p(dgamma), _p(dbeta),
                                int(accumulate), _p(ws), _s()), "bn_eval_bwd")


def bn_relu_maxpool_eval_bwd(g_pooled, argmax, y, scale, shift, gamma, running_mean, running_var, eps, groups, n_per_group, h, w,
                             c, ho, wo, dy, dgamma, dbeta, accumulate):
    n = lib().mvg_bn_eval_bwd_workspace_floats(groups, n_per_group * h * w, c)
    ws = torch.empty(n, dtype=torch.float32, device=y.device)
    check(lib().mvg_bn_relu_maxpool_eval_bwd(_p(_f32c(g_pooled)), _p(argmax), _p(_f32c(y)), _p(scale), _p(shift), _p(gamma),
                                             _p(running_mean), _p(running_var), eps, groups, n_per_group, h, w, c, ho, wo,
                                             _p(_f32c(dy)), _p(dgamma), _p(dbeta), int(accumulate), _p(ws), _s()),
          "bn_relu_maxpool_eval_bwd")


def maxpool_fwd(x, y, argmax, n, h, w, c, ho, wo):
    check(lib().mvg_maxpool3x3s2_fwd(_p(x), _p(y), _p(argmax), n, h, w, c, ho, wo, _s()), "maxpool_fwd")


def maxpool_bwd(dy, argmax, dx, n, h, w, c, ho, wo):
    check(lib().mvg_maxpool3x3s2_bwd(_p(dy), _p(argmax), _p(dx), n, h, w, c, ho, wo, _s()), "maxpool_bwd")


def bn_relu_maxpool_fwd(y, scale, shift, pooled, argmax, groups, n_per_group, h, w, c, ho, wo):
    check(_fn("mvg_bn_relu_maxpool_fwd", y)(_p(y), _p(scale), _p(shift), _p(pooled), _p(argmax), groups, n_per_group, h, w, c, ho,
                                        wo, _s()), "bn_relu_maxpool_fwd")


def bn_relu_maxpool_bwd_reduce(g_pooled, argmax, y, mean, invstd, scale, shift, groups, n_per_group, h, w, c, ho, wo, s1, s2,
                               dgamma, dbeta, accumulate):
    n = lib().mvg_bn_bwd_workspace_floats(groups, n_per_group * h * w, c)
    ws = torch.empty(n, dtype=torch.float32, device=y.device)
    check(_fn("mvg_bn_relu_maxpool_bwd_reduce", y)(_p(g_pooled), _p(argmax), _p(y), _p(mean), _p(invstd), _p(scale), _p(shift),
                                               groups, n_per_group, h, w, c, ho, wo, _p(s1), _p(s2), _p(dgamma), _p(dbeta),
                                               int(accumulate), _p(ws), _s()), "bn_relu_maxpool_bwd_reduce")


def bn_relu_maxpool_bwd_apply(g_pooled, argmax, y, mean, invstd, gamma, scale, shift, s1, s2, groups, n_per_group, h, w, c,
                              ho, wo, dy):
    check(_fn("mvg_bn_relu_maxpool_bwd_apply", y)(_p(g_pooled), _p(argmax), _p(y), _p(mean), _p(invstd), _p(gamma), _p(scale),
                                              _p(shift), _p(s1), _p(s2), groups, n_per_group, h, w, c, ho, wo, _p(dy), _s()),
          "bn_relu_maxpool_bwd_apply")


def avgpool_fwd(x, y, n, hw, c):
    check(_fn("mvg_avgpool_fwd", x)(_p(x), _p(y), n, hw, c, _s()), "avgpool_fwd")


def avgpool_bwd(dy, dx, n, hw, c):
    check(_fn("mvg_avgpool_bwd", dx)(_p(dy), _p(dx), n, hw, c, _s()), "avgpool_bwd")


def nchw_to_nhwc4(src, dst, n, c, h, w):
    check(lib().mvg_nchw_to_nhwc4(_p(src), _p(dst), n, c, h, w, _s()), "nchw_to_nhwc4")


def nchw_to_nhwc8_bf16(src, dst, n, c, h, w):
    check(lib().mvg_nchw_to_nhwc8_bf16(_p(src), _p(dst), n, c, h, w, _s()), "nchw_to_nhwc8_bf16")


def nhwc4_to_nchw(src, dst, n, c, h, w):
    check(lib().mvg_nhwc4_to_nchw(_p(src), _p(dst), n, c, h, w, _s()), "nhwc4_to_nchw")


def low_priority_stream(device) -> "torch.cuda.Stream":
    with torch.cuda.device(device):
        ptr = lib().mvg_stream_create_low_priority()
    if not ptr:
        check(1, "stream_create_low_priority")
    return torch.cuda.ExternalStream(ptr, device=device)


def set_reserved_cus(n: int):
    check(lib().mvg_set_reserved_cus(int(n)), "set_reserved_cus")


def multi_erase_nchw(img, masks, grid, gmax, n, c, h, w):
    check(lib().mvg_multi_erase_nchw(_p(img), _p(masks), _p(grid), gmax, n, c, h, w, _s()), "multi_erase_nchw")


def preprocess_u8hwc_resize(src, dst, n, h, w, oh, ow, mean, std, swap_rb):
    check(lib().mvg_preprocess_u8hwc_resize(_p(src), _p(dst), n, h, w, oh, ow, mean[0], mean[1], mean[2], std[0], std[1],
                                            std[2], int(swap_rb), _s()), "preprocess_u8hwc_resize")


def preprocess_u8hwc_resize_bf16(src, dst, n, h, w, oh, ow, mean, std, swap_rb):
    assert src.dtype == torch.uint8 and src.is_contiguous() and dst.dtype == torch.bfloat16 and dst.is_contiguous()
    assert src.numel() == n * h * w * 3 and dst.numel() == n * oh * ow * 8
    check(lib().mvg_preprocess_u8hwc_resize_bf16(_p(src), _p(dst), n, h, w, oh, ow, mean[0], mean[1], mean[2], std[0], std[1],
                                                 std[2], int(swap_rb), _s()), "preprocess_u8hwc_resize_bf16")


def preprocess_u8hwc(src, dst, n, h, w, mean, std, swap_rb):
    check(lib().mvg_preprocess_u8hwc(_p(src), _p(dst), n, h, w, mean[0], mean[1], mean[2], std[0], std[1], std[2],
                                     int(swap_rb), _s()), "preprocess_u8hwc")


def rotation_matrix_2d(pitch_yaw: Tensor, rot: Tensor, inverse: bool = False):
    check(lib().mvg_rotation_matrix_2d(_p(pitch_yaw), _p(rot), pitch_yaw.shape[0], int(inverse), _s()), "rotation_matrix_2d")


def relative_rotation(rot, vi, vj, rel, batch, views, dirs):
    check(lib().mvg_relative_rotation(_p(rot), _p(vi), _p(vj), _p(rel), batch, views, dirs, _s()), "relative_rotation")


def rotcat_fwd(img_feat, feat, rel, view_of, src_of, x, batch, dirs, cf, nvec):
    check(lib().mvg_rotcat_fwd(_p(img_feat), _p(feat), _p(rel), _p(view_of), _p(src_of), _p(x), batch, dirs, cf, nvec,
                               _s()), "rotcat_fwd")


def rotcat_bwd(dx, rel, src_of, dfeat, batch, dirs, cf, nvec):
    check(lib().mvg_rotcat_bwd(_p(dx), _p(rel), _p(src_of), _p(dfeat), batch, dirs, cf, nvec, _s()), "rotcat_bwd")


def rotcat_ext_fwd(img_feat, feat, rel_apply, rel_append, view_of, src_of, x, ld, batch, dirs, cf, nvec):
    check(lib().mvg_rotcat_ext_fwd(_p(img_feat), _p(feat), _p(rel_apply), _p(rel_append), _p(view_of), _p(src_of), _p(x), ld,
                                   batch, dirs, cf, nvec, _s()), "rotcat_ext_fwd")


def rotcat_ext_bwd(dx, ld, rel, src_of, dfeat, batch, dirs, cf, nvec):
    check(lib().mvg_rotcat_ext_bwd(_p(dx), ld, _p(rel), _p(src_of), _p(dfeat), batch, dirs, cf, nvec, _s()), "rotcat_ext_bwd")


def ibn_scales(a, feat, view_of, src_of, running_mean, training, momentum, eps, scales, batch, dirs, nvec):
    check(lib().mvg_ibn_scales(_p(a), _p(feat), _p(view_of), _p(src_of), _p(running_mean), int(training), momentum, eps,
                               _p(scales), batch, dirs, nvec, _s()), "ibn_scales")


def paircat_fwd(a, feat, rel, scales, view_of, src_of, x, batch, dirs, nvec):
    check(lib().mvg_paircat_fwd(_p(a), _p(feat), _p(rel), _p(scales), _p(view_of), _p(src_of), _p(x), batch, dirs, nvec, _s()),
          "paircat_fwd")


def paircat_bwd(dx, rel, scales, src_of, da_dir, dfeat, batch, dirs, nvec):
    check(lib().mvg_paircat_bwd(_p(dx), _p(rel), _p(scales), _p(src_of), _p(da_dir), _p(dfeat), batch, dirs, nvec, _s()),
          "paircat_bwd")


def segment_sum(x, row_stride, width, seg_of, out, batch, dirs, segments, accumulate):
    check(lib().mvg_segment_sum(_p(x), row_stride, width, _p(seg_of), _p(out), batch, dirs, segments, int(accumulate),
                                _s()), "segment_sum")


def axpby(x, y, a=1.0, b=1.0):
    check(lib().mvg_axpby(_p(x), _p(y), a, b, x.numel(), _s()), "axpby")


def scale_by(x, scale, out):
    check(lib().mvg_scale_by(_p(x), _p(scale), _p(out), x.numel(), _s()), "scale_by")


def linear_skinny_fwd(x, w, bias, y, rows, k, nout):
    check(lib().mvg_linear_skinny_fwd(_p(x), _p(w), _p(bias), _p(y), rows, k, nout, _s()), "linear_skinny_fwd")


def linear_skinny_bwd(dy, x, w, mask, dx, dw, db, rows, k, nout, accumulate=False, dx_absmax=None):
    check(lib().mvg_linear_skinny_bwd(_p(dy), _p(x), _p(w), _p(mask), _p(dx), _p(dw), _p(db), rows, k, nout,
                                      int(accumulate), _p(dx_absmax), _s()), "linear_skinny_bwd")


def adam_step(param, grad, exp_avg, exp_avg_sq, lr, beta1, beta2, eps, weight_decay, step):
    check(lib().mvg_adam_step(_p(param), _p(grad), _p(exp_avg), _p(exp_avg_sq), param.numel(), lr, beta1, beta2, eps,
                              weight_decay, step, _s()), "adam_step")
    for t in (param, exp_avg, exp_avg_sq):
        torch.autograd.graph.increment_version(t)


def gaze_angular_loss(pred, gt, n, row_weight, loss, accumulate=False, dpred=None, theta=None):
    check(lib().mvg_gaze_angular_loss(_p(pred), _p(gt), n, row_weight, _p(loss), int(accumulate), _p(dpred), _p(theta),
                                      _s()), "gaze_angular_loss")


def gaze_lp_loss(pred, label, n, p, loss, dpred=None):
    check(lib().mvg_gaze_lp_loss(_p(pred), _p(label), n, p, _p(loss), _p(dpred), _s()), "gaze_lp_loss")


def absmax_multi(tensors, slots):
    n = len(tensors)
    assert 1 <= n <= 8 and n == len(slots)
    ptrs = (C.c_void_p * n)(*[t.data_ptr() for t in tensors])
    cnts = (C.c_int64 * n)(*[t.numel() for t in tensors])
    outs = (C.c_void_p * n)(*[t.data_ptr() for t in slots])
    for t in tensors:
        assert t.is_cuda and t.dtype == torch.float32 and t.is_contiguous()
    check(lib().mvg_absmax_multi(ptrs, cnts, outs, n, _s()), "absmax_multi")


def fuse_build_split(img_feat, feat, rel, row_img, row_src_f, row_src_h, xf_sp, xh_sp, am_img, am_feat, rows, cf, nvec):
    check(lib().mvg_fuse_build_split(_p(img_feat), _p(feat), _p(rel), _p(row_img), _p(row_src_f), _p(row_src_h), _p(xf_sp), _p(xh_sp),
                                     _p(am_img), _p(am_feat), _sinv(xf_sp), _sinv(xh_sp), rows, cf, nvec, _s()), "fuse_build_split")


def fuse_unbuild(dxh, dxn, rel, seg, vi, dfeat, da, da_accumulate, segments, views, dirs, batch, cf, nvec, absmax=None):
    check(lib().mvg_fuse_unbuild(_p(dxh), _p(dxn), _p(rel), _p(seg), _p(vi), _p(dfeat), _p(da), int(da_accumulate), segments, views, dirs,
                                 batch, cf, nvec, _p(absmax), _s()), "fuse_unbuild")


def linear_fprop_split(x_sp, w_sp, bias, relu, out, rows, fin, fout, bias_absmax=None, out_absmax=None):
    check(lib().mvg_linear_fprop_split(rows, fin, fout, _p(x_sp), _sinv(x_sp), _p(w_sp), _sinv(w_sp), _p(bias), int(relu), _p(out),
                                       int(is_sp(out)), _sinv(out) if is_sp(out) else None, _p(bias_absmax), _p(out_absmax), _s()),
          "linear_fprop_split")


def linear_dgrad_split(dy_sp, wt_sp, dx, rows, fin, fout, addend=None, relu_mask_sp=None, out_absmax=None):
    check(lib().mvg_linear_dgrad_split(rows, fin, fout, _p(dy_sp), _sinv(dy_sp), _p(wt_sp), _sinv(wt_sp), _p(dx), _p(addend),
                                       _p(relu_mask_sp), _p(out_absmax), _s()), "linear_dgrad_split")


def linear_wgrad_split(x_sp, dy_sp, dw, rows, fin, fout, accumulate=False):
    d = ConvDesc.make(1, rows, 1, 1, fin, fout, 1, 1, 0)
    splits, ws = _wgrad_slabs(lib().mvg_conv_wgrad_splits_split, "conv_wgrad_splits_split", d, dw.numel(), dw.device)
    check(lib().mvg_linear_wgrad_split(rows, fin, fout, _p(x_sp), _sinv(x_sp), _p(dy_sp), _sinv(dy_sp), _p(dw), _p(ws), splits,
                                       int(accumulate), _s()), "linear_wgrad_split")


def split_colsum(g, rows, cols, absmax, out_sp, db=None, accumulate=False):
    assert g.dtype == torch.float32 and g.is_contiguous() and g.numel() == rows * cols and cols % 32 == 0
    check(lib().mvg_split_colsum(_p(g), rows, cols, _p(absmax), _p(out_sp), _sinv(out_sp), _p(db), int(accumulate), _s()), "split_colsum")


def gaze_angular_loss_multi(pred, gt, iters, dirs, batch, weights, loss, dpred=None):
    w = (C.c_float * (iters * dirs))(*[float(x) for x in weights])
    check(lib().mvg_gaze_angular_loss_multi(_p(pred), _p(gt), iters, dirs, batch, w, _p(loss), _p(dpred), _s()), "gaze_angular_loss_multi")


def adam_step_dev(param, grad, exp_avg, exp_avg_sq, lr_dev, state3, beta1, beta2, eps, weight_decay):
    check(lib().mvg_adam_step_dev(_p(param), _p(grad), _p(exp_avg), _p(exp_avg_sq), param.numel(), _p(lr_dev), _p(state3), beta1, beta2, eps,
                                  weight_decay, _s()), "adam_step_dev")
    for t in (param, exp_avg, exp_avg_sq):
        torch.autograd.graph.increment_version(t)


def prof_enable(on: bool):
    lib().mvg_prof_enable(int(on))


def prof_reset():
    lib().mvg_prof_reset()


def prof_collect():
    arr = (ProfEntry * K_FAMILIES)()
    check(lib().mvg_prof_collect(arr), "prof_collect")
    out = {}
    for i in range(K_FAMILIES):
        e = arr[i]
        if e.launches:
            out[lib().mvg_prof_family_name(i).decode()] = {
                "launches": int(e.launches), "ms": e.ms, "flops": e.flops, "bytes": e.bytes}
    return out
```

Before: 1709 samples/s.

## Add stream-K scheduling with fix-up pass for small linear split GEMMs

Adds a stream-K variant of the split-precision linear GEMM. K-iterations of all output tiles are spread evenly across a persistent grid, and partial accumulators are written to scratch slabs. A separate fix-up kernel sums the partials and runs the epilogue. It is used for the head linears' forward (when the tape is kept) and their dgrad, where there are fewer tiles than CUs, so under-filled launches should occupy the whole GPU. The cost is an extra kernel launch, scratch traffic, and a plan heuristic that only engages when the tile count is below the CU count.

Measured after the change: 1701 samples/s. No clear change (-0.5%).

```diff
diff --git a/include/rotmvgaze.h b/include/rotmvgaze.h
--- a/include/rotmvgaze.h
+++ b/include/rotmvgaze.h
@@ -364,6 +364,15 @@
                            float *dx, const float *addend, const void *relu_mask_sp, float *out_absmax, void *stream);
 int mvg_linear_wgrad_split(int rows, int fin, int fout, const void *x_sp, const float *x_sinv, const void *dy_sp, const float *dy_sinv,
                            float *dw, float *workspace, int splits, int accumulate, void *stream);
+int mvg_linear_fprop_split_streamk(int rows, int fin, int fout, const void *x_sp, const float *x_sinv, const void *w_sp, const float *w_sinv,
+                                   const float *bias, int relu, void *out, int out_sp, float *out_sinv, const float *bias_absmax,
+                                   float *out_absmax, void *stream);
+int mvg_linear_dgrad_split_streamk(int rows, int fin, int fout, const void *dy_sp, const float *dy_sinv, const void *wt_sp,
+                                   const float *w_sinv, float *dx, const float *addend, const void *relu_mask_sp, float *out_absmax,
+                                   void *stream);
+int mvg_linear_split_streamk_plan(int rows, int fin, int fout, int dgrad, int32_t *bn, int32_t *grid);
+int mvg_set_linear_streamk(int mode);
+int mvg_set_linear_streamk_grid(int per_cu);
 int mvg_split_colsum(const float *g, int rows, int cols, const float *absmax, void *out_sp, float *out_sinv, float *db, int accumulate,
                      void *stream);
 
diff --git a/rot-mvgaze_amd/_lib.py b/rot-mvgaze_amd/_lib.py
--- a/rot-mvgaze_amd/_lib.py
+++ b/rot-mvgaze_amd/_lib.py
@@ -156,6 +156,11 @@
     "mvg_fuse_unbuild": (_I, [_P, _P, _P, _P, _P, _P, _P, _I, _I, _I, _I, _I, _I, _I, _P, _P]),
     "mvg_linear_fprop_split": (_I, [_I, _I, _I, _P, _P, _P, _P, _P, _I, _P, _I, _P, _P, _P, _P]),
     "mvg_linear_dgrad_split": (_I, [_I, _I, _I, _P, _P, _P, _P, _P, _P, _P, _P, _P]),
+    "mvg_linear_fprop_split_streamk": (_I, [_I, _I, _I, _P, _P, _P, _P, _P, _I, _P, _I, _P, _P, _P, _P]),
+    "mvg_linear_dgrad_split_streamk": (_I, [_I, _I, _I, _P, _P, _P, _P, _P, _P, _P, _P, _P]),
+    "mvg_linear_split_streamk_plan": (_I, [_I, _I, _I, _I, C.POINTER(C.c_int32), C.POINTER(C.c_int32)]),
+    "mvg_set_linear_streamk": (_I, [_I]),
+    "mvg_set_linear_streamk_grid": (_I, [_I]),
     "mvg_linear_wgrad_split": (_I, [_I, _I, _I, _P, _P, _P, _P, _P, _P, _I, _I, _P]),
     "mvg_split_colsum": (_I, [_P, _I, _I, _P, _P, _P, _P, _I, _P]),
     "mvg_cast_weights_bf16": (_I, [_D, _P, _I, _P, _P, _P]),
diff --git a/rot-mvgaze_amd/csrc/conv_split.hip b/rot-mvgaze_amd/csrc/conv_split.hip
--- a/rot-mvgaze_amd/csrc/conv_split.hip
+++ b/rot-mvgaze_amd/csrc/conv_split.hip
@@ -353,6 +353,59 @@
 #define MVG_SPLIT_RNG 1
 #include "conv_split_igemm.inc"
 #undef MVG_SPLIT_RNG
+template <int TM, int TN>
+struct SkAcc {
+  f32x4 v[TM][TN];
+  __device__ __forceinline__ f32x4 (&operator[](int i))[TN] { return v[i]; }
+};
+#define MVG_SPLIT_RNG 2
+#include "conv_split_igemm.inc"
+#undef MVG_SPLIT_RNG
+
+template <int BN, bool DGRAD>
+__global__ __launch_bounds__(256) void igemm_split16_fixup_kernel(IgemmParams p, int P) {
+  constexpr int BM = SP_BM, WGM = 2, WGN = 2;
+  constexpr int TM = BM / WGM / 16, TN = BN / WGN / 16;
+  __shared__ __attribute__((aligned(16))) unsigned char smem[bf16_epilogue_bytes<BM, BN, WGM, DGRAD>()];
+  const int tid = threadIdx.x;
+  const IgemmClass &c = p.cls[0];
+  const long long U = (long long)p.sk_tiles * c.KT;
+  const int cut = blockIdx.x;
+  const long long ucut = (long long)(cut + 1) * U / P;
+  const long long tile = ucut / c.KT;
+  const long long t0 = tile * c.KT, t1 = t0 + c.KT;
+  if (ucut == t0) return;
+  if ((long long)cut * U / P > t0) return;
+  SkAcc<TM, TN> acc;
+#pragma unroll
+  for (int i = 0; i < TM; ++i)
+#pragma unroll
+    for (int j = 0; j < TN; ++j)
+#pragma unroll
+      for (int e = 0; e < 4; ++e) acc[i][j][e] = 0.f;
+  for (int b = cut; b < P; ++b) {
+    const long long ub = (long long)b * U / P;
+    if (ub >= t1) break;
+    if ((long long)(b + 1) * U / P == ub) continue;
+    const float4 *src = reinterpret_cast<const float4 *>(p.slab) + ((long long)b * 2 + (ub > t0 ? 0 : 1)) * (BM * BN / 4);
+#pragma unroll
+    for (int i = 0; i < TM; ++i)
+#pragma unroll
+      for (int j = 0; j < TN; ++j) {
+        const float4 v = src[(i * TN + j) * 256 + tid];
+        acc[i][j][0] += v.x;
+        acc[i][j][1] += v.y;
+        acc[i][j][2] += v.z;
+        acc[i][j][3] += v.w;
+      }
+  }
+  const int wg = (int)tile;
+  const int ntile = wg % p.ntiles;
+  const int mt_all = wg / p.ntiles;
+  const int g = mt_all / c.mtiles_per_group;
+  const int mtile = mt_all - g * c.mtiles_per_group;
+  bf16_epilogue<BM, BN, WGM, DGRAD, true, WGM, true, DGRAD, true, WGN>(p, c, acc, reinterpret_cast<unsigned short *>(smem), tid, g, mtile, ntile);
+}
 
 template <int BM, int BN, bool INCR>
 __global__ __launch_bounds__(256, BN >= 256 ? 2 : 3) void wgrad_split_kernel(WgradParams p) {
@@ -664,8 +717,26 @@
   return pl;
 }
 
+static int g_lin_streamk = 1;
+static int g_lin_streamk_grid = 0;
+constexpr int SK_MIN_STEPS = 28;
+static int plan_split_streamk(const SplitPlan &pl, int ncls, int groups) {
+  if (g_lin_streamk == 0 || ncls != 1 || groups != 1 || pl.bm != SP_BM || pl.kt_max <= 1 || pl.tiles <= 0) return 0;
+  const long long units = pl.tiles * pl.kt_max;
+  const int cus = compute_cus();
+  if (g_lin_streamk == 2 || g_lin_streamk_grid > 0) {
+    const long long P = (long long)(g_lin_streamk_grid > 0 ? g_lin_streamk_grid : 1) * cus;
+    return (int)(P < units ? P : units);
+  }
+  if (!pl.pipelined || pl.tiles >= cus) return 0;
+  for (int sp = 2; pl.tiles * sp <= 2LL * cus && pl.kt_max / sp >= SK_MIN_STEPS; ++sp)
+    if (pl.kt_max % sp == 0 && pl.tiles * sp >= cus) return (int)(pl.tiles * sp);
+  return 0;
+}
+
 template <bool DGRAD>
-static int launch_igemm_split(IgemmParams &p, hipStream_t st, bool lin, int taps, long long rows, AForm af = A_DMA, bool ranged = false) {
+static int launch_igemm_split(IgemmParams &p, hipStream_t st, bool lin, int taps, long long rows, AForm af = A_DMA, bool ranged = false,
+                              bool streamk = false) {
   const SplitPlan pl = split_plan(p.ncols, taps, rows, p.groups, lin, p.cls, p.ncls);
   const int bm = pl.bm, bn = pl.bn;
   const bool pipelined = pl.pipelined;
@@ -709,6 +780,21 @@
       else hipLaunchKernelGGL((igemm_split16_ranged_kernel<64>), grid, block, 0, st, p);
     }
     return check_launch("conv_fprop_split_ranged");
+  }
+  if (lin && streamk) {
+    const int P = plan_split_streamk(pl, p.ncls, p.groups);
+    float *scratch = P > 0 ? stream_scratch(st, (size_t)P * 2 * SP_BM * bn) : nullptr;
+    if (scratch) {
+      p.slab = scratch;
+      p.sk_tiles = (int)pl.tiles;
+      if (bn == 128) hipLaunchKernelGGL((igemm_split16_streamk_kernel<128, DGRAD>), dim3((unsigned)P), block, 0, st, p);
+      else hipLaunchKernelGGL((igemm_split16_streamk_kernel<64, DGRAD>), dim3((unsigned)P), block, 0, st, p);
+      if (check_launch(DGRAD ? "linear_dgrad_split(stream-K)" : "linear_fprop_split(stream-K)")) return 1;
+      if (P < 2) return 0;
+      if (bn == 128) hipLaunchKernelGGL((igemm_split16_fixup_kernel<128, DGRAD>), dim3((unsigned)(P - 1)), block, 0, st, p, P);
+      else hipLaunchKernelGGL((igemm_split16_fixup_kernel<64, DGRAD>), dim3((unsigned)(P - 1)), block, 0, st, p, P);
+      return check_launch("linear split stream-K fix-up");
+    }
   }
   if (lin) {
     if (bn == 128 && pipelined) hipLaunchKernelGGL((igemm_split16_kernel<128, DGRAD, true, 2, 2>), grid, block, 0, st, p);
@@ -816,6 +902,7 @@
   float *out_absmax, *out_sinv;
   const float *bias_absmax;
   uint32_t *range_word;
+  int streamk;
 };
 
 struct SplitFwdApply {
@@ -867,7 +954,7 @@
   ProfScope ps(lin ? MVG_K_LINEAR_FPROP : MVG_K_CONV_FPROP, (hipStream_t)stream, flops, bytes);
   p.stats_partials = ceil_div(p.rows_per_group, SP_BM) * 2;
   return launch_igemm_split<false>(p, (hipStream_t)stream, aff && aff->lin, d->r * d->s, p.rows_per_group,
-                                   fap ? (fap->res_scale ? A_OUT_AFFINE : A_OUT_SP) : A_DMA, aff && aff->range_word);
+                                   fap ? (fap->res_scale ? A_OUT_AFFINE : A_OUT_SP) : A_DMA, aff && aff->range_word, aff && aff->streamk);
 }
 
 int mvg_conv_fprop_split(const mvg_conv_desc *d, const void *x_sp, const float *x_sinv, const void *w_sp, const float *w_sinv, float *y,
@@ -933,7 +1020,7 @@
 
 static int dgrad_split_impl(const mvg_conv_desc *d, const void *dy_sp, const float *dy_sinv, const void *w_crsk_sp, const float *w_sinv,
                             float *dx, const float *addend, void *stream, const SplitBnFuse *bnf, const void *relu_mask_sp = nullptr,
-                            bool lin_kernel = false, float *out_absmax = nullptr, const SplitBnApply *bna = nullptr) {
+                            bool lin_kernel = false, float *out_absmax = nullptr, const SplitBnApply *bna = nullptr, bool streamk = false) {
   if (validate_split(d)) return 2;
   IgemmParams p;
   memset(&p, 0, sizeof(p));
@@ -976,7 +1063,8 @@
   ProfScope ps(lin ? MVG_K_LINEAR_DGRAD : MVG_K_CONV_DGRAD, (hipStream_t)stream, flops, bytes);
   if (int e = dgrad_classes(p, d, bnf != nullptr, 4, dx, addend, (hipStream_t)stream)) return e;
   if (p.ncls == 0) return 0;
-  return launch_igemm_split<true>(p, (hipStream_t)stream, lin_kernel, d->r * d->s, (long long)d->n * d->h * d->w, bna ? A_DY : A_DMA);
+  return launch_igemm_split<true>(p, (hipStream_t)stream, lin_kernel, d->r * d->s, (long long)d->n * d->h * d->w, bna ? A_DY : A_DMA, false,
+                                  streamk);
 }
 
 int mvg_conv_dgrad_split(const mvg_conv_desc *d, const void *dy_sp, const float *dy_sinv, const void *w_crsk_sp, const float *w_sinv,
@@ -1205,6 +1293,48 @@
   return dgrad_split_impl(&d, dy_sp, dy_sinv, wt_sp, w_sinv, dx, addend, stream, nullptr, relu_mask_sp, true, out_absmax);
 }
 
+int mvg_linear_fprop_split_streamk(int rows, int fin, int fout, const void *x_sp, const float *x_sinv, const void *w_sp, const float *w_sinv,
+                                   const float *bias, int relu, void *out, int out_sp, float *out_sinv, const float *bias_absmax,
+                                   float *out_absmax, void *stream) {
+  MVG_REQUIRE(bias != nullptr && out != nullptr, "linear_fprop_split_streamk: bias and out are required");
+  MVG_REQUIRE(!out_sp || out_sinv, "linear_fprop_split_streamk: an sp result needs out_sinv (it is stored scaled)");
+  MVG_REQUIRE(!(out_sp && out_absmax), "linear_fprop_split_streamk: out_absmax is for fp32 results");
+  const mvg_conv_desc d = linear_desc(rows, fin, fout);
+  const SplitAffine a = {nullptr, bias, nullptr, 0, relu, out_sp, 1, out_absmax, out_sinv, bias_absmax, nullptr, 1};
+  return fprop_split_impl(&d, x_sp, x_sinv, w_sp, w_sinv, out, nullptr, stream, &a);
+}
+
+int mvg_linear_dgrad_split_streamk(int rows, int fin, int fout, const void *dy_sp, const float *dy_sinv, const void *wt_sp, const float *w_sinv,
+                                   float *dx, const float *addend, const void *relu_mask_sp, float *out_absmax, void *stream) {
+  const mvg_conv_desc d = linear_desc(rows, fin, fout);
+  return dgrad_split_impl(&d, dy_sp, dy_sinv, wt_sp, w_sinv, dx, addend, stream, nullptr, relu_mask_sp, true, out_absmax, nullptr, true);
+}
+
+int mvg_linear_split_streamk_plan(int rows, int fin, int fout, int dgrad, int32_t *bn, int32_t *grid) {
+  const mvg_conv_desc d = linear_desc(rows, fin, fout);
+  if (validate_split(&d)) return 2;
+  IgemmClass c;
+  memset(&c, 0, sizeof(c));
+  c.rows_per_group = rows;
+  c.ktotal = dgrad ? fout : fin;
+  const SplitPlan pl = split_plan(dgrad ? fin : fout, 1, rows, 1, true, &c, 1);
+  if (bn) *bn = pl.bn;
+  if (grid) *grid = plan_split_streamk(pl, 1, 1);
+  return 0;
+}
+
+int mvg_set_linear_streamk(int mode) {
+  MVG_REQUIRE(mode >= 0 && mode <= 2, "set_linear_streamk: 0 never, 1 by the plan, 2 wherever a tile has more than one K-step");
+  g_lin_streamk = mode;
+  return 0;
+}
+
+int mvg_set_linear_streamk_grid(int per_cu) {
+  MVG_REQUIRE(per_cu >= 0 && per_cu <= 2, "set_linear_streamk_grid: 0 (the plan's grid) or one / two persistent workgroups per CU");
+  g_lin_streamk_grid = per_cu;
+  return 0;
+}
+
 int mvg_linear_wgrad_split(int rows, int fin, int fout, const void *x_sp, const float *x_sinv, const void *dy_sp, const float *dy_sinv,
                            float *dw, float *workspace, int splits, int accumulate, void *stream) {
   const mvg_conv_desc d = linear_desc(rows, fin, fout);
diff --git a/rot-mvgaze_amd/csrc/conv_split_igemm.inc b/rot-mvgaze_amd/csrc/conv_split_igemm.inc
--- a/rot-mvgaze_amd/csrc/conv_split_igemm.inc
+++ b/rot-mvgaze_amd/csrc/conv_split_igemm.inc
@@ -1,8 +1,14 @@
 #ifndef MVG_SPLIT_RNG
-#error "conv_split_igemm.inc: define MVG_SPLIT_RNG (0 or 1) before including"
-#endif
-
-#if MVG_SPLIT_RNG
+#error "conv_split_igemm.inc: define MVG_SPLIT_RNG (0, 1 or 2) before including"
+#endif
+
+#if MVG_SPLIT_RNG == 2
+template <int BN, bool DGRAD>
+__global__ __launch_bounds__(256, 2) void igemm_split16_streamk_kernel(IgemmParams p) {
+  constexpr bool LIN = true;
+  constexpr int WGM = 2, STAGES = 2;
+  constexpr AForm AF = A_DMA;
+#elif MVG_SPLIT_RNG
 template <int BN, int WGM = 2, int STAGES = 1>
 __global__ __launch_bounds__(256, STAGES == 2 ? 2 : WGM == 4 ? 3 : 4) void igemm_split16_ranged_kernel(IgemmParams p) {
   constexpr bool DGRAD = false, LIN = false;
@@ -31,6 +37,29 @@
   constexpr int SMEM_B = BNK_OFF + (AF != A_DMA ? Former::TABLES : 0) * BNA_MAX_C * 4;
   __shared__ __attribute__((aligned(16))) unsigned char smem[SMEM_B];
 
+#if MVG_SPLIT_RNG == 2
+  const int nwg = gridDim.x;
+  const int wg_all = p.no_remap ? (int)blockIdx.x : xcd_remap(blockIdx.x, nwg);
+  const IgemmClass &c = p.cls[0];
+  const long long U = (long long)p.sk_tiles * c.KT;
+  long long u0 = (long long)wg_all * U / nwg;
+  const long long u1 = (long long)(wg_all + 1) * U / nwg;
+  while (u0 < u1) {
+  int tid = threadIdx.x;
+  asm volatile("" : "+v"(tid));
+  const int lane = tid & 63, wave = __builtin_amdgcn_readfirstlane(tid >> 6);
+  const int wm = wave / WGN, wn = wave % WGN;
+  const int wg = (int)(u0 / c.KT);
+  const int kt0 = (int)(u0 - (long long)wg * c.KT);
+  const int KT = (u1 - u0 < (long long)(c.KT - kt0)) ? kt0 + (int)(u1 - u0) : c.KT;
+  u0 += KT - kt0;
+  const int ntile = wg % p.ntiles;
+  const int mt_all = wg / p.ntiles;
+  const int g = mt_all / c.mtiles_per_group;
+  const int mtile = mt_all - g * c.mtiles_per_group;
+  const int ohw = c.out_h * c.out_w;
+#else
+  constexpr int kt0 = 0;
   const int tid = threadIdx.x;
   const int lane = tid & 63, wave = __builtin_amdgcn_readfirstlane(tid >> 6);
   const int wm = wave / WGN, wn = wave % WGN;
@@ -46,6 +75,7 @@
   const int mtile = mt_all - g * c.mtiles_per_group;
   const int KT = c.KT;
   const int ohw = c.out_h * c.out_w;
+#endif
 
   uint2 *rowinfo = reinterpret_cast<uint2 *>(smem + INFO_OFF);
   if (tid < BM) {
@@ -119,7 +149,11 @@
       __builtin_amdgcn_raw_ptr_buffer_load_lds(rs_b, (lds_vp)(smem + stage_off + (wave + NW * (A_PER + i)) * 1024), 16, (int)(b_base[i] + kb), 0, 0, 0);
   };
 
+#if MVG_SPLIT_RNG == 2
+  SkAcc<TM, TN> acc;
+#else
   f32x4 acc[TM][TN];
+#endif
 #pragma unroll
   for (int i = 0; i < TM; ++i)
 #pragma unroll
@@ -220,9 +254,9 @@
     }
   } else {
     constexpr int G = A_PER + B_PER;
-    if (KT > 0) issue(0, 0);
-    if (KT > 1) {
-      issue(1, STAGE_B);
+    if (KT > kt0) issue(kt0, 0);
+    if (KT > kt0 + 1) {
+      issue(kt0 + 1, STAGE_B);
       asm volatile("s_waitcnt vmcnt(%0)\n\ts_barrier" ::"n"(G) : "memory");
     } else {
       asm volatile("s_waitcnt vmcnt(0)\n\ts_barrier" ::: "memory");
@@ -239,13 +273,26 @@
       }
       products(ca, cb);
     };
-    for (int kt = 0; kt < KT; kt += 2) {
+    for (int kt = kt0; kt < KT; kt += 2) {
       step(kt, a0, b0, a1, b1);
       if (kt + 1 < KT) step(kt + 1, a1, b1, a0, b0);
     }
     __syncthreads();
   }
-#if MVG_SPLIT_RNG
+#if MVG_SPLIT_RNG == 2
+  if (kt0 > 0 || KT < c.KT) {
+    float4 *dst = reinterpret_cast<float4 *>(p.slab) + ((long long)wg_all * 2 + (kt0 > 0 ? 0 : 1)) * (BM * BN / 4);
+#pragma unroll
+    for (int i = 0; i < TM; ++i)
+#pragma unroll
+      for (int j = 0; j < TN; ++j) dst[(i * TN + j) * 256 + tid] = make_float4(acc[i][j][0], acc[i][j][1], acc[i][j][2], acc[i][j][3]);
+  } else {
+    bf16_epilogue<BM, BN, WGM, DGRAD, true, WGM, true, DGRAD, LIN, WGN>(p, c, acc, reinterpret_cast<unsigned short *>(smem), tid, g, mtile, ntile);
+    __syncthreads();
+  }
+  asm volatile("s_waitcnt vmcnt(0)" ::: "memory");
+  }
+#elif MVG_SPLIT_RNG
   bf16_epilogue<BM, BN, WGM, DGRAD, true, WGM, true, DGRAD, LIN, WGN, false, true>(p, c, acc, reinterpret_cast<unsigned short *>(smem), tid, g, mtile,
                                                                                      ntile);
 #else
diff --git a/rot-mvgaze_amd/heads.py b/rot-mvgaze_amd/heads.py
--- a/rot-mvgaze_amd/heads.py
+++ b/rot-mvgaze_amd/heads.py
@@ -408,13 +408,14 @@
             wf0, wf1, wh0 = fu._wsp[0], fu._wsp[1], hd._wsp[0]
             hid, hhid = fu.fout[0], hd.fout[0]
             h = sp(rows, hid, f"h{it}")
-            ops.linear_fprop_split(xf, wf0[0], fu.b[0].detach(), True, h, rows, kin, hid, bias_absmax=slot(f"bam{it}"))
-            ops.linear_fprop_split(h, wf1[0], fu.b[1].detach(), False, feats[it], rows, hid, ROT_DIM, out_absmax=slot(f"amF{it}"))
+            ops.linear_fprop_split(xf, wf0[0], fu.b[0].detach(), True, h, rows, kin, hid, bias_absmax=slot(f"bam{it}"), streamk=keep_tape)
+            ops.linear_fprop_split(h, wf1[0], fu.b[1].detach(), False, feats[it], rows, hid, ROT_DIM, out_absmax=slot(f"amF{it}"),
+                                   streamk=keep_tape)
             xh = sp(rows, kin, f"xh{it}")
             xf_next = sp(rows, kin, f"xf{it + 1}") if it + 1 < I else None
             ops.fuse_build_split(img2d, feats[it], rel_fuse, rt["img"], rt["partner"], rt["ident"], xf_next, xh, slot("am_img"),
                                  slot(f"amF{it}"), rows, cf, NV)
-            ops.linear_fprop_split(xh, wh0[0], hd.b[0].detach(), True, hh[it], rows, kin, hhid)
+            ops.linear_fprop_split(xh, wh0[0], hd.b[0].detach(), True, hh[it], rows, kin, hhid, streamk=keep_tape)
             ops.linear_skinny_fwd(hh[it], hd.w[1].detach(), hd.b[1].detach(), preds[it], rows, hhid, 2)
             if keep_tape:
                 saved.append((xf, h, xh, hh[it], wf0, wf1, wh0))
@@ -463,7 +464,7 @@
                 ops.split_colsum(dhh, rows, hhid, slot(f"am_dhh{it}"), g_hh, sink.view(hd.b[0]), ab0)
                 wgrad(xh, g_hh, hd.w[0], kin, hhid, a0)
                 dXh = torch.empty(rows, kin, dtype=torch.float32, device=dev)
-                ops.linear_dgrad_split(g_hh, wh0[1], dXh, rows, kin, hhid)
+                ops.linear_dgrad_split(g_hh, wh0[1], dXh, rows, kin, hhid, streamk=True)
             else:
                 self._zero_grads(hd, sink, wr)
             ext = d_feats[it].reshape(rows, ROT_DIM).contiguous() if d_feats is not None else None
@@ -490,14 +491,15 @@
             ops.split_colsum(dF, rows, ROT_DIM, am_dF, g_F, sink.view(fu.b[1]), ab1)
             wgrad(h, g_F, fu.w[1], hid, ROT_DIM, a1)
             dh = torch.empty(rows, hid, dtype=torch.float32, device=dev)
-            ops.linear_dgrad_split(g_F, wf1[1], dh, rows, hid, ROT_DIM, relu_mask_sp=h, out_absmax=slot(f"am_dh{it}"))
+            ops.linear_dgrad_split(g_F, wf1[1], dh, rows, hid, ROT_DIM, relu_mask_sp=h, out_absmax=slot(f"am_dh{it}"),
+                                   streamk=True)
             a0, ab0 = wr.acc(fu.w[0]), wr.acc(fu.b[0])
             assert a0 == ab0
             g_h = sp(rows, hid, f"g_h{it}")
             ops.split_colsum(dh, rows, hid, slot(f"am_dh{it}"), g_h, sink.view(fu.b[0]), ab0)
             wgrad(xf, g_h, fu.w[0], kin, hid, a0)
             dXn = torch.empty(rows, kin, dtype=torch.float32, device=dev)
-            ops.linear_dgrad_split(g_h, wf0[1], dXn, rows, kin, hid)
+            ops.linear_dgrad_split(g_h, wf0[1], dXn, rows, kin, hid, streamk=True)
             if not v.share_weights:
                 sink.publish(hd.parameters() + fu.parameters())
         if v.share_weights:
diff --git a/rot-mvgaze_amd/ops.py b/rot-mvgaze_amd/ops.py
--- a/rot-mvgaze_amd/ops.py
+++ b/rot-mvgaze_amd/ops.py
@@ -727,15 +727,31 @@
                                  batch, cf, nvec, _p(absmax), _s()), "fuse_unbuild")
 
 
-def linear_fprop_split(x_sp, w_sp, bias, relu, out, rows, fin, fout, bias_absmax=None, out_absmax=None):
-    check(lib().mvg_linear_fprop_split(rows, fin, fout, _p(x_sp), _sinv(x_sp), _p(w_sp), _sinv(w_sp), _p(bias), int(relu), _p(out),
-                                       int(is_sp(out)), _sinv(out) if is_sp(out) else None, _p(bias_absmax), _p(out_absmax), _s()),
+def linear_fprop_split(x_sp, w_sp, bias, relu, out, rows, fin, fout, bias_absmax=None, out_absmax=None, streamk=False):
+    fn = lib().mvg_linear_fprop_split_streamk if streamk else lib().mvg_linear_fprop_split
+    check(fn(rows, fin, fout, _p(x_sp), _sinv(x_sp), _p(w_sp), _sinv(w_sp), _p(bias), int(relu), _p(out),
+             int(is_sp(out)), _sinv(out) if is_sp(out) else None, _p(bias_absmax), _p(out_absmax), _s(streamk)),
           "linear_fprop_split")
 
 
-def linear_dgrad_split(dy_sp, wt_sp, dx, rows, fin, fout, addend=None, relu_mask_sp=None, out_absmax=None):
-    check(lib().mvg_linear_dgrad_split(rows, fin, fout, _p(dy_sp), _sinv(dy_sp), _p(wt_sp), _sinv(wt_sp), _p(dx), _p(addend),
-                                       _p(relu_mask_sp), _p(out_absmax), _s()), "linear_dgrad_split")
+def linear_dgrad_split(dy_sp, wt_sp, dx, rows, fin, fout, addend=None, relu_mask_sp=None, out_absmax=None, streamk=False):
+    fn = lib().mvg_linear_dgrad_split_streamk if streamk else lib().mvg_linear_dgrad_split
+    check(fn(rows, fin, fout, _p(dy_sp), _sinv(dy_sp), _p(wt_sp), _sinv(wt_sp), _p(dx), _p(addend),
+             _p(relu_mask_sp), _p(out_absmax), _s(streamk)), "linear_dgrad_split")
+
+
+def linear_split_streamk_plan(rows, fin, fout, dgrad=False):
+    bn, grid = C.c_int32(0), C.c_int32(0)
+    check(lib().mvg_linear_split_streamk_plan(rows, fin, fout, int(dgrad), C.byref(bn), C.byref(grid)), "linear_split_streamk_plan")
+    return bn.value, grid.value
+
+
+def set_linear_streamk(mode: int):
+    check(lib().mvg_set_linear_streamk(int(mode)), "set_linear_streamk")
+
+
+def set_linear_streamk_grid(per_cu: int):
+    check(lib().mvg_set_linear_streamk_grid(int(per_cu)), "set_linear_streamk_grid")
 
 
 def linear_wgrad_split(x_sp, dy_sp, dw, rows, fin, fout, accumulate=False):
```
